# ucb-bar/Accelerated-TinyMPC

Hardware: AMD Instinct MI355X
Metric: MPC solves/sec (batched quadrotor nx=12,nu=4,N=30) (higher is better)
Workload: dtype f32; 1 GPU; quadrotor_tracking batched 65536 instances per GPU, cold-start tiny_solve, early_exit (tol 1e-3, max_iter 100); nx=12, nu=4, N=30, instances_per_gpu=65536, instances_total=65536, parallelism=batch-shard x1, world_size_seen=1, backend=none (single process), kernel=tile16<12,4,30,exact>, max_iters=85

## Files before the change

accelerated-tinympc_amd/csrc/admm_tile16.hip:

```cpp
#include "rowlane_math.h"
#include <cstdlib>

namespace tinympc
{

typedef float f32x16 __attribute__((ext_vector_type(16)));
#ifndef TINY_T16_ABLATE
#define TINY_T16_ABLATE 0
#endif
#ifndef TINY_T16_CQ
#define TINY_T16_CQ 1
#endif
#ifndef TINY_T16_BADDR
#define TINY_T16_BADDR 1
#endif
#ifndef TINY_T16_PADTAB
#define TINY_T16_PADTAB 1
#endif
#ifndef TINY_T16_XPOSE
#define TINY_T16_XPOSE 1
#endif
#ifndef TINY_T16_SCHED
#define TINY_T16_SCHED 1
#endif
// ... 307 lines not shown
{
#pragma unroll
    for (int k = 0; k < 4; k++)
    {
        lo8[k] = __int_as_float(__builtin_amdgcn_update_dpp(__float_as_int(e[k]), __float_as_int(o[k]), 0x128, 0xf, 0xc, false));
        hi8[k] = __int_as_float(__builtin_amdgcn_update_dpp(__float_as_int(o[k]), __float_as_int(e[k]), 0x128, 0xf, 0x3, false));
    }
}

#if TINY_T16_STAMP && !defined(TINY_T16_PI_UNIT)
constexpr int T16_STAMP_TILES = 32;
__device__ unsigned long long *t16_stamp_buf;
__device__ int t16_stamp_slots;
__device__ __forceinline__ void t16_stamp(int wslot, int k, int field, unsigned long long v)
{
    unsigned long long *const buf = t16_stamp_buf;
    if (buf && wslot < t16_stamp_slots && k < T16_STAMP_TILES && (threadIdx.x & 63) == 0) buf[((size_t)wslot * T16_STAMP_TILES + k) * 4 + field] = v;
}
#define T16_STAMP(k, field, v) t16_stamp((int)blockIdx.x * TILE16_WAVES + (int)(threadIdx.x >> 6), (k), (field), (v))
#else
#define T16_STAMP(k, field, v) ((void)0)
#endif

__device__ __forceinline__ void t16_dma_row(unsigned on, const float *sbase, unsigned voff, unsigned lds_dst, float after)
{
    asm volatile("s_cmp_eq_u32 %0, 0\n\ts_cbranch_scc1 1f\n\ts_mov_b32 m0, %3\n\ts_nop 0\n\tglobal_load_lds_dwordx4 %1, %2\n1:"
                 : : "s"(on), "v"(voff), "s"(sbase), "s"(lds_dst), "v"(after) : "memory", "scc");
}
__device__ __forceinline__ void t16_dma_row2(unsigned on, const float *sbase, unsigned voff, unsigned lds_dst, float after0, float after1)
{
    asm volatile("s_cmp_eq_u32 %0, 0\n\ts_cbranch_scc1 1f\n\ts_mov_b32 m0, %3\n\ts_nop 0\n\tglobal_load_lds_dwordx4 %1, %2\n\t"
                 "s_add_u32 m0, m0, 0x3f0\n\ts_nop 0\n\tglobal_load_lds_dwordx4 %1, %2 offset:16\n1:"
                 : : "s"(on), "v"(voff), "s"(sbase), "s"(lds_dst), "v"(after0), "v"(after1) : "memory", "scc");
}
__device__ __forceinline__ void t16_dma_img2(unsigned on, const float *sbase, unsigned voff, unsigned lds_dst, float after0, float after1)
{
    asm volatile("s_cmp_eq_u32 %0, 0\n\ts_cbranch_scc1 1f\n\ts_mov_b32 m0, %3\n\ts_nop 0\n\tglobal_load_lds_dwordx4 %1, %2\n\t"
                 "global_load_lds_dwordx4 %1, %2 offset:1024\n1:"
                 : : "s"(on), "v"(voff), "s"(sbase), "s"(lds_dst), "v"(after0), "v"(after1) : "memory", "scc");
}
__device__ __forceinline__ void t16_wait_vm(int k)
{
    if (k == 0) asm volatile("s_waitcnt vmcnt(0)" ::: "memory");
    else if (k == 1) asm volatile("s_waitcnt vmcnt(1)" ::: "memory");
    else if (k == 2) asm volatile("s_waitcnt vmcnt(2)" ::: "memory");
    else if (k == 3) asm volatile("s_waitcnt vmcnt(3)" ::: "memory");
    else if (k == 4) asm volatile("s_waitcnt vmcnt(4)" ::: "memory");
    else if (k == 5) asm volatile("s_waitcnt vmcnt(5)" ::: "memory");
    else if (k == 6) asm volatile("s_waitcnt vmcnt(6)" ::: "memory");
    else if (k == 7) asm volatile("s_waitcnt vmcnt(7)" ::: "memory");
    else asm volatile("s_waitcnt vmcnt(8)" ::: "memory");
}
constexpr int t16_ring_b(bool XR) { return XR ? 3 : 4; }
constexpr int t16_ring_x(bool BR) { return BR ? 4 : 6; }
constexpr int T16_RING_B = 2048, T16_RING_X = 1024;

template <int N, bool EXACT, bool COLD, bool MPC = false, bool BR = false, bool XR = false>
__global__ __launch_bounds__(WAVE * TILE16_WAVES, 1) void admm_tile16_kernel(const RowParams P)
{
    static_assert(!(MPC && (BR || XR)), "the closed loop on chip is instantiated for batch-shared bounds and a shared / windowed reference");
    constexpr int NX = 12, NU = 4;
    const int lane = threadIdx.x & 63, wv = threadIdx.x >> 6, g = lane >> 4, c = lane & 15;
    const int ntiles = (P.batch + 15) >> 4;
    const float rho = P.rho;
    const f32x4 rho4 = {rho, rho, rho, rho};

    extern __shared__ __attribute__((aligned(16))) float4 lds4_base[];
    float4 *const lds4 = lds4_base;
    float4 *const sn0 = lds4 + wv * (N * WAVE) + lane;
    constexpr int DB = t16_ring_b(XR), DX = t16_ring_x(BR);
    const unsigned ringsB = (P.pi_flags & 1u) ? DB : 2, ringsX = (P.pi_flags & 2u) ? DX : 1;
    const unsigned bnd_f4 = BR ? TILE16_WAVES * ringsB * (T16_RING_B / 16) : 2 * N * 4;
    float4 *const blo = lds4 + TILE16_WAVES * N * WAVE, *const bhi = blo + N * 4, *const tab0 = blo + bnd_f4;
    float4 *const tab = tab0;
    const int tab_rows = P.xref_mode == 1 ? P.table_rows : N;
    const float *tab_src = P.xref_mode == 1 ? P.xref_table : P.xref;
    unsigned dmaB = 0, dmaX = 0;
    if constexpr (BR)
    {
        const unsigned ring = (unsigned)(size_t)(lds_float4 *)blo + wv * (ringsB * T16_RING_B);
        dmaB = __builtin_amdgcn_readfirstlane(ring);
    }
    else
    {
        for (int e = threadIdx.x; e < N * 16; e += WAVE * TILE16_WAVES)
        {
            const float2 lh = reinterpret_cast<const float2 *>(P.bounds)[e];
            const int i = e >> 4, r = e & 15;
            reinterpret_cast<float *>(&blo[i * 4 + (r & 3)])[r >> 2] = lh.x;
            reinterpret_cast<float *>(&bhi[i * 4 + (r & 3)])[r >> 2] = lh.y;
        }
    }
    if constexpr (XR)
    {
        const unsigned ring = (unsigned)(size_t)(lds_float4 *)tab0 + wv * (ringsX * T16_RING_X);
        dmaX = __builtin_amdgcn_readfirstlane(ring);
    }
    else
    {
        for (int e = threadIdx.x; e < (tab_rows + N - 1) * 16; e += WAVE * TILE16_WAVES)
        {
            const int er = (e >> 4) < tab_rows ? (e >> 4) : tab_rows - 1;
            float val = tab_src[er * 16 + (e & 15)];
            if (TINY_T16_CQ) val = -(val * ((e & 15) < NX ? P.mats[(2 * NX + 2 * NU) * 16 + (e & 15)] : 1.f));
            reinterpret_cast<float *>(&tab[(e >> 4) * 4 + (e & 3)])[(e & 15) >> 2] = val;
        }
    }
    if constexpr (!BR || !XR) __syncthreads();

    TileMath<EXACT> M;
    M.load(P.mats, g, c);
    f32x4 qv;
#pragma unroll
    for (int v = 0; v < 3; v++) qv[v] = P.mats[(2 * NX + 2 * NU) * 16 + 4 * v + g];
    qv[3] = 1.f;
    constexpr bool CQ = TINY_T16_CQ && !XR;
    auto cost_of = [&](const f32x4 &xr) { return CQ ? xr : -(xr * qv); };

    constexpr bool DQ = COLD && !MPC;
    int qinc = 1;
    if constexpr (DQ)
    {
        const unsigned tail_stride = (P.pi_flags >> 8) & 0xffu;
        if (tail_stride && (((unsigned)blockIdx.x * TILE16_WAVES + (unsigned)wv) % tail_stride) == 0u) qinc = 0x10000;
        qinc = __builtin_amdgcn_readfirstlane(qinc);
    }
#if TINY_T16_STAMP
    int stamp_k = 0;
#else
    constexpr int stamp_k = 0;
#endif
    for (;;)
    {
    int slot = 0;
    if (lane == 0) slot = atomicAdd(P.n_unsolved + 1, qinc);
    slot = __builtin_amdgcn_readfirstlane(slot);
    T16_STAMP(stamp_k, 0, __builtin_amdgcn_s_memrealtime());
    T16_STAMP(stamp_k, 3, ~0ull);
    if (DQ && ntiles <= 32768)
    {
        const int qh = slot & 0xffff, qt = (int)((unsigned)slot >> 16);
        if (qh + qt >= ntiles) break;
        slot = qinc == 1 ? qh : ntiles - 1 - qt;
    }
    else if (slot >= ntiles) break;
    int ozt;
    asm volatile("s_mov_b32 %0, 0" : "=s"(ozt));
    float4 *const sn = sn0 + ozt;
    float4 *const lds4 = lds4_base + ozt;
    int tile = slot;
    if (P.order) tile = P.order[slot];
    const bool tile_ok = tile >= 0 && tile < ntiles;
    T16_STAMP(stamp_k, 3, (unsigned long long)(unsigned)tile);
    const int inst = tile * 16 + c;
    const bool valid = tile_ok && inst < P.batch;
    const int inst_a = valid ? inst : P.batch - 1;

    float a[N][4];
    float dr[N], bo[N][4], pl[N][3];
    auto dual4 = [&](int i) { return f32x4{a[i][0], a[i][1], a[i][2], a[i][3]}; };
    const int ebase = (inst_a * N) * 16 + g;
    int wstart = 0;
    if (P.xref_mode == 1) wstart = P.xref_start[inst_a];
    const bool zdual = COLD || (P.duals_zero != 0);

    if constexpr (COLD)
    {
        const float4 z4 = make_float4(0.f, 0.f, 0.f, 0.f);
#pragma unroll
        for (int i = 0; i < N; i++)
        {
            a[i][0] = a[i][1] = a[i][2] = a[i][3] = 0.f;
#pragma unroll
            for (int v = 0; v < 4; v++) acc_init(bo[i][v], 0.f);
            sn[i * WAVE] = z4;
            acc_init(pl[i][0], 0.f); acc_init(pl[i][1], 0.f); acc_init(pl[i][2], 0.f);
            dr[i] = 0.f;
        }
    }
    else
    {
#pragma unroll
        for (int i = 0; i < N; i++)
        {
            float vzl[4], pdv[4];
#pragma unroll
            for (int v = 0; v < 4; v++)
            {
                const int o = ebase + i * 16 + 4 * v;
                vzl[v] = P.vz[o]; pdv[v] = P.pd[o];
                const float gyv = P.gy[o];
                a[i][v] = zdual ? 0.f : gyv;
                acc_init(bo[i][v], vzl[v]);
            }
            sn[i * WAVE] = make_float4(vzl[0], vzl[1], vzl[2], vzl[3]);
            acc_init(pl[i][0], pdv[0]); acc_init(pl[i][1], pdv[1]); acc_init(pl[i][2], pdv[2]);
            dr[i] = pdv[3];
        }
    }
    float x0[3];
#pragma unroll
    for (int v = 0; v < 3; v++) x0[v] = P.xu[ebase + 4 * v];

    const unsigned onB = BR ? (P.pi_flags & 1u) : 0u, onX = XR ? (P.pi_flags & 2u) : 0u;
    struct PiAddr { unsigned rdB, rdX, voffB, voffX; };
    auto pi_addr = [&](unsigned lane16) {
        const unsigned c16 = lane16 & 0xf0u, gg = lane16 >> 8, cc = c16 >> 4;
        const int ins = tile * 16 + (int)cc;
        const unsigned ia = (unsigned)((tile_ok && ins < P.batch) ? ins : P.batch - 1);
        PiAddr A;
        A.rdB = dmaB + 1024u * (gg >> 1) + c16 + 8u * (gg & 1u);
        A.rdX = dmaX + c16 + 4u * gg;
        A.voffB = ia * P.bounds_inst_stride * 8u + 32u * gg;
        A.voffX = ia * P.xref_inst_stride * 4u + 16u * gg;
        return A;
    };
    const float *const xsrc = P.xref;
    auto load_xref = [&](const float4 *tb, int ws, int i, int gsel = -1) {
        if constexpr (XR)
        {
            unsigned ll = lane;
            asm volatile("" : "+v"(ll));
            const unsigned cc = ll & 15u, gg = ll >> 4;
            if (onX)
            {
                const float *rp = xsrc + ((size_t)((tile_ok ? tile : 0) * N + i) * 64 + cc) * 4 + gg;
                return f32x4{rp[0], rp[64], rp[128], 0.f};
            }
            const int ins = tile * 16 + (int)cc;
            const float *rp = xsrc + (size_t)((tile_ok && ins < P.batch) ? ins : P.batch - 1) * P.xref_inst_stride + i * 16 + gg;
            return f32x4{rp[0], rp[4], rp[8], 0.f};
        }
        else
        {
        int row;
        if constexpr (TINY_T16_PADTAB && !(EXACT && COLD && !MPC && !BR && !XR)) row = (ws < tab_rows - 1 ? ws : tab_rows - 1) + i;
        else { row = ws + i; row = row < tab_rows ? row : tab_rows - 1; }
        const float4 t4 = tb[row * 4 + (gsel >= 0 ? gsel : g)];
        return f32x4{t4.x, t4.y, t4.z, t4.w};
        }
    };
    PiAddr A0 = {0u, 0u, 0u, 0u};
    if constexpr (BR || XR)
    {
        A0 = pi_addr(16u * lane);
        if constexpr (BR) { t16_dma_row2(onB ^ 1u, P.bounds, A0.voffB, dmaB, 0.f, 0.f); t16_dma_row2(onB ^ 1u, P.bounds, A0.voffB + (N - 1) * 128u, dmaB + T16_RING_B, 0.f, 0.f); }
        if constexpr (XR) t16_dma_row((onX >> 1) ^ 1u, xsrc, A0.voffX, dmaX, 0.f);
        asm volatile("s_waitcnt vmcnt(0)" ::: "memory");
    }
    auto load_xref_raw = [&](const float4 *tb, int ws, int i) {
        if constexpr (CQ)
        {
            int row = ws + i;
            row = row < tab_rows ? row : tab_rows - 1;
            const float *rp = tab_src + row * 16 + g;
            return f32x4{rp[0], rp[4], rp[8], 0.f};
        }
        else return load_xref(tb, ws, i);
    };
    float pterm[3];
    {
        const f32x4 xrN4 = load_xref_raw(tab, wstart, N - 1);
        const float xrN[3] = {xrN4[0], xrN4[1], xrN4[2]};
        M.terminal(xrN, pterm);
    }

    int st = TINY_STATUS_UNSOLVED_, itn = 1;
    float r_ps = 0.f, r_pi = 0.f, r_ds = 0.f, r_di = 0.f;
    if (valid && !COLD)
    {
        r_ps = P.res[4 * inst + 0]; r_pi = P.res[4 * inst + 1];
        r_ds = P.res[4 * inst + 2]; r_di = P.res[4 * inst + 3];
    }
    float pN[3] = {0.f, 0.f, 0.f};

    auto backward_sweep = [&](unsigned long long amask, const float4 *snI, const float4 *tabI, int wsI) {
        float p[3] = {pN[0], pN[1], pN[2]};
        auto load_lin = [&](int i, float4 &sl, f32x4 &xr) {
            sl = snI[i * WAVE];
            xr = load_xref(tabI, wsI, i);
        };
        auto make_lin = [&](int i, const float4 &sl, const f32x4 &xr) {
            const f32x4 sni = {sl.x, sl.y, sl.z, sl.w};
            return lin_cost4<EXACT>(cost_of(xr), rho4, sni - dual4(i));
        };
        float4 sl0; f32x4 xr0;
        load_lin(N - 2, sl0, xr0);
        f32x4 lin = make_lin(N - 2, sl0, xr0);
#pragma unroll
        for (int i = N - 2; i >= 0; i--)
        {
            float4 sl_n = make_float4(0.f, 0.f, 0.f, 0.f); f32x4 xr_n = {0.f, 0.f, 0.f, 0.f};
            if (EXACT && i > 0) load_lin(i - 1, sl_n, xr_n);
            typename TileMath<EXACT>::InFlight F;
            M.riccati_issue(p, lin, F);
            if (!EXACT && i > 0) load_lin(i - 1, sl_n, xr_n);
#if TINY_T16_SCHED
            if constexpr (EXACT) __builtin_amdgcn_sched_barrier(0);
#endif
            f32x4 lin_n = lin;
            if (i > 0) lin_n = make_lin(i - 1, sl_n, xr_n);
#if TINY_T16_SCHED
            if constexpr (EXACT) __builtin_amdgcn_sched_barrier(0);
#endif
            float pn[3], dd;
            M.riccati_finish(F, lin, pn, dd);
            masked_backward_update(amask, pl[i], dr[i], pn, dd);
            p[0] = pn[0]; p[1] = pn[1]; p[2] = pn[2];
// ... 68 lines not shown
            const f32x4 dp = sv - t, dd_ = old - t;
            pri_x = fmaxf(fmaxf(fmaxf(pri_x, fabsf(dp[0])), fabsf(dp[1])), fabsf(dp[2]));
            dua_x = fmaxf(fmaxf(fmaxf(dua_x, fabsf(dd_[0])), fabsf(dd_[1])), fabsf(dd_[2]));
            pri_u = fmaxf(pri_u, fabsf(dp[3]));
            dua_u = fmaxf(dua_u, fabsf(dd_[3]));
            if (i == N - 1)
            {
                const f32x4 an = tp - t;
#pragma unroll
                for (int v = 0; v < 3; v++)
                {
                    const float pn_ = lin_cost<EXACT>(pterm[v], rho, t[v] - an[v]);
                    pN[v] = active ? pn_ : pN[v];
                }
            }
            masked_forward_update(amask, a[i], tp, bo[i], old, sn_addr + i * (WAVE * 16), t);
        };
        f32x4 sv_p = {0.f, 0.f, 0.f, 0.f};
        float4 lo_p = make_float4(0.f, 0.f, 0.f, 0.f), hi_p = lo_p, ol_p = lo_p;
#pragma unroll
        for (int i = 0; i < N; i++)
        {
            float4 lo, hi;
            if constexpr (BR)
            {
                if (i + DB - 1 < N) dma_b(i + DB - 1, lo_p.x, hi_p.w);
                t16_wait_vm(2 * ((N - 1 - i) < (DB - 1) ? (N - 1 - i) : (DB - 1)));
                ring_bounds(i, lo, hi);
            }
            else if constexpr (TINY_T16_BADDR && (COLD || !XR)) { lo = bloG[i * 4]; hi = bhiG[i * 4]; }
            else { lo = bloI[i * 4 + g]; hi = bhiI[i * 4 + g]; }
            const float4 ol = snI[i * WAVE];
            typename TileMath<EXACT>::InFlight F;
            if (i < N - 1) M.lqr_issue(s, F);
#if TINY_T16_SCHED
            if constexpr (EXACT) __builtin_amdgcn_sched_barrier(0);
#endif
            if (i > 0) elementwise(i - 1, sv_p, lo_p, hi_p, ol_p);
            float un = 0.f, xn[3] = {0.f, 0.f, 0.f};
            if (i < N - 1) M.lqr_finish(F, dr[i], un, xn);
            sv_p = f32x4{s[0], s[1], s[2], un};
            lo_p = lo; hi_p = hi; ol_p = ol;
            s[0] = xn[0]; s[1] = xn[1]; s[2] = xn[2];
        }
        elementwise(N - 1, sv_p, lo_p, hi_p, ol_p);
        pri_x = tile_inst_max(pri_x); dua_x = tile_inst_max(dua_x);
        pri_u = tile_inst_max(pri_u); dua_u = tile_inst_max(dua_u);
        bool conv = false;
        if (active)
        {
            itn = it + 1;
            if ((it + 1) % P.check_termination == 0)
            {
                r_ps = pri_x; r_ds = dua_x * rho; r_pi = pri_u; r_di = dua_u * rho;
                conv = (r_ps < P.abs_pri_tol) && (r_pi < P.abs_pri_tol) && (r_ds < P.abs_dua_tol) && (r_di < P.abs_dua_tol);
            }
            if (conv) st = TINY_STATUS_SOLVED_;
        }
        active = active && !conv;
        if (!__any(active)) break;
        if (it == P.max_iter - 1) break;
        {
            float p[3] = {pN[0], pN[1], pN[2]};
            const unsigned long long amask = __ballot(active);
            auto load_lin = [&](int i, float4 &sl, f32x4 &xr) {
                sl = snI[i * WAVE];
                if constexpr (XR) xr = ring_xref(i);
                else xr = load_xref(tabI, wsI, i, TINY_T16_BADDR ? (int)gI : -1);
            };
            auto make_lin = [&](int i, const float4 &sl, const f32x4 &xr) {
                const f32x4 sni = {sl.x, sl.y, sl.z, sl.w};
                return lin_cost4<EXACT>(cost_of(xr), rho4, sni - dual4(i));
            };
            float4 sl0; f32x4 xr0;
            if constexpr (XR) t16_wait_vm(0);
            load_lin(N - 2, sl0, xr0);
            f32x4 lin = make_lin(N - 2, sl0, xr0);
#pragma unroll
            for (int i = N - 2; i >= 0; i--)
            {
                float4 sl_n = make_float4(0.f, 0.f, 0.f, 0.f); f32x4 xr_n = {0.f, 0.f, 0.f, 0.f};
                if constexpr (XR)
                {
                    if (i >= DX) dma_x(i - DX, lin[0]);
                    if (i > 0)
                    {
                        const int hi_j = (i - 2) < (N - 2 - DX) ? (i - 2) : (N - 2 - DX), lo_j = (i - DX) > 0 ? (i - DX) : 0;
                        t16_wait_vm(hi_j >= lo_j ? hi_j - lo_j + 1 : 0);
                    }
                }
                if (EXACT && i > 0) load_lin(i - 1, sl_n, xr_n);
                typename TileMath<EXACT>::InFlight F;
                M.riccati_issue(p, lin, F);
                if (!EXACT && i > 0) load_lin(i - 1, sl_n, xr_n);
#if TINY_T16_SCHED
                if constexpr (EXACT) __builtin_amdgcn_sched_barrier(0);
#endif
                f32x4 lin_n = lin;
                if (i > 0) lin_n = make_lin(i - 1, sl_n, xr_n);
#if TINY_T16_SCHED
                if constexpr (EXACT) __builtin_amdgcn_sched_barrier(0);
#endif
                float pn[3], dd;
                M.riccati_finish(F, lin, pn, dd);
                masked_backward_update(amask, pl[i], dr[i], pn, dd);
                p[0] = pn[0]; p[1] = pn[1]; p[2] = pn[2];
                lin = lin_n;
            }
        }
    }
    if (!MPC || ms + 1 >= P.mpc_steps) break;
    if constexpr (MPC)
    {
        int oz;
        asm volatile("s_mov_b32 %0, 0" : "=s"(oz));
        float4 *const snA = sn + oz;
        const unsigned sn_addr = (unsigned)(size_t)(lds_float4 *)snA;
        const bool solved = st == TINY_STATUS_SOLVED_;
        float un, xn_[3];
        M.lqr(x0, dr[0], un, xn_);
        if (P.u0_traj && valid) P.u0_traj[((long long)ms * P.batch + inst) * NU + g] = un;
        {
            const f32x16 p0 = TINY_MFMA1(M.A1[0], x0[0], M.negz), p1 = TINY_MFMA1(M.A1[1], x0[1], M.negz), p2 = TINY_MFMA1(M.A1[2], x0[2], M.negz);
            const f32x16 pb = TINY_MFMA1(M.A2, un, M.negz);
            f32x4 t[12], t2[4];
            gather12v(t, p0, p1, p2);
            gather4v(t2, pb);
            f32x4 z = {0.f, 0.f, 0.f, 0.f};
            asm volatile("" : "+v"(z));
            f32x4 acc = z + t[0];
#pragma unroll
            for (int k = 1; k < 12; k++) acc = acc + t[k];
            const f32x4 x1 = acc + reduce4<PLAN_SEQ>(t2);
            x0[0] = x1[0]; x0[1] = x1[1]; x0[2] = x1[2];
        }
        const unsigned long long umask = __ballot(valid && !solved);
        if (umask != 0ull) backward_sweep(umask, snA, tab + oz, wstart + oz);
        const unsigned long long smask = __ballot(valid && solved);
#pragma unroll
        for (int i = 0; i < N; i++) masked_restore_slack(smask, bo[i], sn_addr + i * (WAVE * 16));
        if (P.xref_mode == 1)
        {
            wstart += P.window_advance;
            const f32x4 xrN4 = load_xref_raw(tab + oz, wstart, N - 1);
            const float xrN[3] = {xrN4[0], xrN4[1], xrN4[2]};
            M.terminal(xrN, pterm);
        }
#pragma unroll
        for (int i = 0; i < N; i++) a[i][0] = a[i][1] = a[i][2] = a[i][3] = 0.f;
    }
    }
    T16_STAMP(stamp_k, 1, __builtin_amdgcn_s_memrealtime());

    if (P.max_iter <= 0)
    {
        if (valid && g == 0)
        {
            P.status[inst] = TINY_STATUS_UNSOLVED_;
            P.iter[inst] = 1;
            atomicAdd(P.n_unsolved, 1);
        }
        T16_STAMP(stamp_k, 2, __builtin_amdgcn_s_memrealtime());
#if TINY_T16_STAMP
        ++stamp_k;
#endif
        continue;
    }

    {
        const bool solved = st == TINY_STATUS_SOLVED_;
        const int c2 = lane >> 2, q2 = lane & 3;
        const int inst2 = tile * 16 + c2;
        const bool valid2 = tile_ok && inst2 < P.batch;
        const int obase2 = ((valid2 ? inst2 : 0) * N) * 16 + 4 * q2;
        typedef float float_ma __attribute__((may_alias));
        typedef f32x4 f32x4_ma __attribute__((may_alias));
        float_ma *const stage_w = reinterpret_cast<float_ma *>(lds4 + wv * (N * WAVE));
        const int rd_off = (c2 * 4 + q2);
        const int obase4 = ebase + 3 * g;
        constexpr bool XPOSE = TINY_T16_XPOSE && !(EXACT && !COLD && !MPC);
        auto put = [&](float *dst, int i, const f32x4 &val) {
            if constexpr (XPOSE)
            {
                const f32x4 o = t16_transpose4(val);
                if (valid) *reinterpret_cast<f32x4 *>(dst + obase4 + i * 16) = o;
                return;
            }
            float_ma *slot = stage_w + i * (WAVE * 4);
            reinterpret_cast<f32x4_ma *>(slot)[lane] = val;
            asm volatile("" ::: "memory");
            f32x4 o;
            o[0] = slot[rd_off]; o[1] = slot[rd_off + 64]; o[2] = slot[rd_off + 128]; o[3] = slot[rd_off + 192];
            asm volatile("" ::: "memory");
            if (valid2) *reinterpret_cast<f32x4 *>(dst + obase2 + i * 16) = o;
        };
        float s[3] = {x0[0], x0[1], x0[2]};
        if constexpr (XPOSE && TINY_T16_LINES && COLD && !MPC && !BR && !XR)
        {
            auto slack_of = [&](int i) { return reinterpret_cast<const f32x4_ma *>(stage_w + i * (WAVE * 4))[lane]; };
            auto lin_of = [&](int i, const f32x4 &sni) {
                const f32x4 xr = load_xref(tab, wstart, i);
                f32x4 lin = lin_cost4<EXACT>(cost_of(xr), rho4, sni - dual4(i));
                if (i == N - 1) lin[3] = 0.f;
                return lin;
            };
            auto pd_of = [&](int i) { return i == N - 1 ? f32x4{pN[0], pN[1], pN[2], 0.f} : f32x4{acc_get(pl[i][0]), acc_get(pl[i][1]), acc_get(pl[i][2]), dr[i]}; };
            auto vz_of = [&](int i, const f32x4 &sni) {
                f32x4 vzv;
    #pragma unroll
                for (int v = 0; v < 4; v++)
                {
                    const float bov = acc_get(bo[i][v]);
                    vzv[v] = solved ? bov : sni[v];
                }
                return vzv;
            };
            const int instL = tile * 16 + (c & 7);
            const bool validL = tile_ok && instL < P.batch, validH = tile_ok && instL + 8 < P.batch;
            const int obaseL = (validL ? instL : 0) * (N * 16) + ((c >> 3) << 4) + 4 * g, offH = 8 * N * 16;
            auto put2 = [&](float *dst, int i, const f32x4 &ve, const f32x4 &vo) {
                f32x4 lo8, hi8;
                t16_pair_lines(t16_transpose4(ve), t16_transpose4(vo), lo8, hi8);
                if (validL) *reinterpret_cast<f32x4 *>(dst + obaseL + i * 16) = lo8;
                if (validH) *reinterpret_cast<f32x4 *>(dst + obaseL + offH + i * 16) = hi8;
            };
#pragma unroll
            for (int i = 0; i + 1 < N; i += 2)
            {
                const f32x4 sne = slack_of(i), sno = slack_of(i + 1);
                put2(P.gy, i, dual4(i), dual4(i + 1));
                put2(P.vzn, i, sne, sno);
                put2(P.vz, i, vz_of(i, sne), vz_of(i + 1, sno));
                put2(P.pd, i, pd_of(i), pd_of(i + 1));
                put2(P.qr, i, lin_of(i, sne), lin_of(i + 1, sno));
                float ue = 0.f, xe[3];
                M.lqr(s, dr[i], ue, xe);
                const f32x4 sve = {s[0], s[1], s[2], ue};
                float uo = 0.f, xo[3] = {0.f, 0.f, 0.f};
                if (i + 1 < N - 1) M.lqr(xe, dr[i + 1], uo, xo);
                put2(P.xu, i, sve, f32x4{xe[0], xe[1], xe[2], uo});
                s[0] = xo[0]; s[1] = xo[1]; s[2] = xo[2];
            }
            if constexpr (N % 2 == 1)
            {
                const f32x4 sni = slack_of(N - 1);
                put(P.xu, N - 1, f32x4{s[0], s[1], s[2], 0.f});
                put(P.qr, N - 1, lin_of(N - 1, sni));
                put(P.pd, N - 1, pd_of(N - 1));
                put(P.vz, N - 1, vz_of(N - 1, sni));
                put(P.vzn, N - 1, sni);
                put(P.gy, N - 1, dual4(N - 1));
            }
        }
        else
        {
#pragma unroll
        for (int i = 0; i < N; i++)
        {
            float un = 0.f, xn[3] = {0.f, 0.f, 0.f};
            if (i < N - 1) M.lqr(s, dr[i], un, xn);
            const f32x4 sv = {s[0], s[1], s[2], un};
            const f32x4 sni = reinterpret_cast<const f32x4_ma *>(stage_w + i * (WAVE * 4))[lane];
            const f32x4 xr = load_xref(tab, wstart, i);
            f32x4 lin = lin_cost4<EXACT>(cost_of(xr), rho4, sni - dual4(i));
            if (i == N - 1) lin[3] = 0.f;
            f32x4 pdv = {acc_get(pl[i][0]), acc_get(pl[i][1]), acc_get(pl[i][2]), dr[i]};
            if (i == N - 1) pdv = f32x4{pN[0], pN[1], pN[2], 0.f};
            f32x4 vzv;
#pragma unroll
            for (int v = 0; v < 4; v++)
            {
                const float bov = acc_get(bo[i][v]);
                vzv[v] = solved ? bov : sni[v];
            }
            put(P.xu, i, sv);
            put(P.qr, i, lin);
            put(P.pd, i, pdv);
            put(P.vz, i, vzv);
            put(P.vzn, i, sni);
            put(P.gy, i, dual4(i));
            if constexpr (!XPOSE) reinterpret_cast<f32x4_ma *>(stage_w + i * (WAVE * 4))[lane] = sni;
            s[0] = xn[0]; s[1] = xn[1]; s[2] = xn[2];
        }
        }
        const unsigned long long umask = __ballot(valid && !solved);
        if (umask != 0ull)
        {
            const bool unsolved2 = valid2 && ((umask >> c2) & 1ull);
            float p[3] = {pN[0], pN[1], pN[2]};
#pragma unroll
            for (int i = N - 2; i >= 0; i--)
            {
                const f32x4 sni = reinterpret_cast<const f32x4_ma *>(stage_w + i * (WAVE * 4))[lane];
                const f32x4 xr = load_xref(tab, wstart, i);
                const f32x4 lin = lin_cost4<EXACT>(cost_of(xr), rho4, sni - dual4(i));
                float pn[3], dd;
                M.riccati(p, lin, pn, dd);
                if constexpr (XPOSE)
                {
                    const f32x4 o = t16_transpose4(f32x4{pn[0], pn[1], pn[2], dd});
                    if (valid && !solved) *reinterpret_cast<f32x4 *>(P.pd + obase4 + i * 16) = o;
                }
                else
                {
                float_ma *slot = stage_w + i * (WAVE * 4);
                reinterpret_cast<f32x4_ma *>(slot)[lane] = f32x4{pn[0], pn[1], pn[2], dd};
                asm volatile("" ::: "memory");
                f32x4 o;
                o[0] = slot[rd_off]; o[1] = slot[rd_off + 64]; o[2] = slot[rd_off + 128]; o[3] = slot[rd_off + 192];
                asm volatile("" ::: "memory");
                if (unsolved2) *reinterpret_cast<f32x4 *>(P.pd + obase2 + i * 16) = o;
                }
                p[0] = pn[0]; p[1] = pn[1]; p[2] = pn[2];
            }
        }
        if (valid && g == 0)
        {
            P.res[4 * inst + 0] = r_ps; P.res[4 * inst + 1] = r_pi;
            P.res[4 * inst + 2] = r_ds; P.res[4 * inst + 3] = r_di;
            P.status[inst] = st;
            P.iter[inst] = itn;
            if (!solved) atomicAdd(P.n_unsolved, 1);
        }
        if (MPC && valid)
        {
#pragma unroll
            for (int v = 0; v < 3; v++) P.x0buf[inst * NX + 4 * v + g] = x0[v];
            if (g == 0 && P.xref_mode == 1) P.xref_start[inst] = wstart;
        }
    }
    T16_STAMP(stamp_k, 2, __builtin_amdgcn_s_memrealtime());
#if TINY_T16_STAMP
    ++stamp_k;
#endif
    }
}

#ifdef TINY_T16_ONLY30
#define TINY_FOR_EACH_TILE16(X) X(30)
#else
#define TINY_FOR_EACH_TILE16(X) X(30) X(25) X(20) X(10)
#endif

static inline unsigned t16_tail_stride(const RowParams &P, int ntiles, int nblocks, int asked)
{
    static const int env = [] { const char *e = getenv("TINYMPC_T16_TAIL"); return e ? atoi(e) : -1; }();
    const int forced = asked >= 0 ? asked : env;
    if (ntiles > 32768) return 0u;
    if (forced >= 0) return (P.cold_start && P.mpc_steps <= 1) ? (unsigned)(forced > 255 ? 255 : forced) : 0u;
    if (!P.order || P.mpc_steps > 1 || !P.cold_start) return 0u;
    const int slots = nblocks * TILE16_WAVES;
    if (ntiles < 3 * slots) return 0u;
    return (ntiles >= 4 * slots && ntiles < 8 * slots) ? 4u : 8u;
}

#ifdef TINY_T16_PI_UNIT
size_t tile16_pi_lds_bytes(int N, bool bounds_ring, bool xref_ring, unsigned pi_flags, int table_rows)
{
    const size_t bnd = bounds_ring ? (size_t)TILE16_WAVES * ((pi_flags & 1u) ? t16_ring_b(xref_ring) : 2) * T16_RING_B : (size_t)2 * N * 4 * sizeof(float4);
    const size_t ref = xref_ring ? (size_t)TILE16_WAVES * ((pi_flags & 2u) ? t16_ring_x(bounds_ring) : 1) * T16_RING_X : (size_t)(table_rows + N - 1) * 4 * sizeof(float4);
    return (size_t)TILE16_WAVES * N * WAVE * sizeof(float4) + bnd + ref;
}

hipError_t launch_admm_tile16_pi(int N, bool exact, bool bounds_ring, bool xref_ring, const RowParams &P, hipStream_t stream, int n_cu, int tail)
{
    const int ntiles = (P.batch + 15) / 16;
    if (n_cu <= 0) n_cu = 256;
    const int want = (ntiles + TILE16_WAVES - 1) / TILE16_WAVES, nblocks = want < n_cu ? want : n_cu;
    if (P.mpc_steps > 1 || (!bounds_ring && !xref_ring)) return hipErrorInvalidValue;
    if (P.xref_mode == 1 && P.table_rows < 1) return hipErrorInvalidValue;
    if (!bounds_ring && P.bounds_inst_stride != 0) return hipErrorInvalidValue;
    if (!xref_ring && P.xref_mode != 1 && P.xref_inst_stride != 0) return hipErrorInvalidValue;
    if (xref_ring && P.xref_mode == 1) return hipErrorInvalidValue;
    const size_t lds = tile16_pi_lds_bytes(N, bounds_ring, xref_ring, P.pi_flags, P.xref_mode == 1 ? P.table_rows : N);
    if (lds > 160 * 1024) return hipErrorInvalidValue;
    RowParams Q = P;
    Q.pi_flags = (Q.pi_flags & 0xffu) | (t16_tail_stride(P, ntiles, nblocks, tail) << 8);
#define TINY_TILE16_PI_LAUNCH3(NN, EX, BRR, XRR)                                                                           \
    {                                                                                                                      \
        auto kern = P.cold_start ? admm_tile16_kernel<NN, EX, true, false, BRR, XRR> : admm_tile16_kernel<NN, EX, false, false, BRR, XRR>; \
        hipError_t e = hipFuncSetAttribute((const void *)kern, hipFuncAttributeMaxDynamicSharedMemorySize, (int)lds);      \
        if (e != hipSuccess) return e;                                                                                     \
        hipLaunchKernelGGL(kern, dim3(nblocks), dim3(WAVE * TILE16_WAVES), lds, stream, Q);                                \
        return hipGetLastError();                                                                                          \
    }
#define TINY_TILE16_PI_LAUNCH(NN, EX)                                             \
    {                                                                             \
        if (bounds_ring && xref_ring) TINY_TILE16_PI_LAUNCH3(NN, EX, true, true)  \
        else if (bounds_ring) TINY_TILE16_PI_LAUNCH3(NN, EX, true, false)         \
        else TINY_TILE16_PI_LAUNCH3(NN, EX, false, true)                          \
    }
#define TINY_TILE16_PI_DISPATCH(NN)                  \
    if (N == NN)                                     \
    {                                                \
        if (exact) TINY_TILE16_PI_LAUNCH(NN, true)   \
        else TINY_TILE16_PI_LAUNCH(NN, false)        \
    }
    TINY_FOR_EACH_TILE16(TINY_TILE16_PI_DISPATCH)
    return hipErrorInvalidValue;
}
#else
bool tile16_supported(int nx, int nu, int N)
{
    if (nx != 12 || nu != 4) return false;
#define TINY_TILE16_CHECK(NN) \
    if (N == NN) return true;
    TINY_FOR_EACH_TILE16(TINY_TILE16_CHECK)
    return false;
}

int tile16_max_table_rows() { return TILE16_MAX_TABLE_ROWS; }

#if TINY_T16_STAMP
static int t16_stamp_nslots = 0;
extern "C" int tiny_t16_stamp_begin()
{
    static unsigned long long *buf = nullptr;
    int dev = 0, ncu = 0;
    if (hipGetDevice(&dev) != hipSuccess || hipDeviceGetAttribute(&ncu, hipDeviceAttributeMultiprocessorCount, dev) != hipSuccess || ncu <= 0) return 1;
    const int nslots = ncu * TILE16_WAVES;
    const size_t bytes = (size_t)nslots * T16_STAMP_TILES * 4 * sizeof(unsigned long long);
    if (buf) (void)hipFree(buf);
    buf = nullptr;
    if (hipMalloc(&buf, bytes) != hipSuccess || hipMemset(buf, 0, bytes) != hipSuccess) return 1;
    if (hipMemcpyToSymbol(HIP_SYMBOL(t16_stamp_slots), &nslots, sizeof(nslots)) != hipSuccess) return 1;
    if (hipMemcpyToSymbol(HIP_SYMBOL(t16_stamp_buf), &buf, sizeof(buf)) != hipSuccess || hipDeviceSynchronize() != hipSuccess) return 1;
    t16_stamp_nslots = nslots;
    return 0;
}
extern "C" int tiny_t16_stamp_slots() { return t16_stamp_nslots; }
extern "C" int tiny_t16_stamp_read(unsigned long long *host, int nslots)
{
    if (nslots > t16_stamp_nslots) return 1;
    unsigned long long *buf = nullptr;
    if (hipMemcpyFromSymbol(&buf, HIP_SYMBOL(t16_stamp_buf), sizeof(buf)) != hipSuccess || !buf) return 1;
    return hipMemcpy(host, buf, (size_t)nslots * T16_STAMP_TILES * 4 * sizeof(unsigned long long), hipMemcpyDeviceToHost) != hipSuccess;
}
extern "C" int tiny_t16_stamp_tiles() { return T16_STAMP_TILES; }
#endif

hipError_t launch_admm_tile16(int N, bool exact, const RowParams &P, hipStream_t stream, int n_cu, int tail)
{
    const int ntiles = (P.batch + 15) / 16;
    if (n_cu <= 0) n_cu = 256;
    const int want = (ntiles + TILE16_WAVES - 1) / TILE16_WAVES, nblocks = want < n_cu ? want : n_cu;
    const int rows = P.xref_mode == 1 ? P.table_rows : N;
    if (rows > TILE16_MAX_TABLE_ROWS) return hipErrorInvalidValue;
    const size_t lds = (size_t)(TILE16_WAVES * N * WAVE + 2 * N * 4 + (rows + N - 1) * 4) * sizeof(float4);
    RowParams Q = P;
    Q.pi_flags = (Q.pi_flags & 0xffu) | (t16_tail_stride(P, ntiles, nblocks, tail) << 8);
#define TINY_TILE16_LAUNCH(NN, EX)                                                                                         \
    {                                                                                                                      \
        auto kern = P.mpc_steps > 1 ? (P.cold_start ? admm_tile16_kernel<NN, EX, true, true> : admm_tile16_kernel<NN, EX, false, true>) \
                                    : (P.cold_start ? admm_tile16_kernel<NN, EX, true> : admm_tile16_kernel<NN, EX, false>); \
        hipError_t e = hipFuncSetAttribute((const void *)kern, hipFuncAttributeMaxDynamicSharedMemorySize, (int)lds);      \
        if (e != hipSuccess) return e;                                                                                     \
        hipLaunchKernelGGL(kern, dim3(nblocks), dim3(WAVE * TILE16_WAVES), lds, stream, Q);                                \
        return hipGetLastError();                                                                                          \
    }
#define TINY_TILE16_DISPATCH(NN)                  \
    if (N == NN)                                  \
    {                                             \
        if (exact) TINY_TILE16_LAUNCH(NN, true)   \
        else TINY_TILE16_LAUNCH(NN, false)        \
    }
    TINY_FOR_EACH_TILE16(TINY_TILE16_DISPATCH)
    return hipErrorInvalidValue;
}
#endif

}
```

accelerated-tinympc_amd/csrc/dispatch_order.hip:

```cpp
#include "rowlane_math.h"

namespace tinympc
{

constexpr int kPredictorSteps = 4;

template <int NX, int NU, bool H16, bool TILES = false>
__global__ __launch_bounds__(TILES ? 4 * WAVE : WAVE) void dispatch_key_kernel(const RowParams P, float *__restrict__ key)
{
    const int lane = threadIdx.x & (WAVE - 1), r16 = lane & 15;
    const int grp = TILES ? (int)blockIdx.x * 4 + (int)(threadIdx.x >> 6) : (int)blockIdx.x;
    const int inst = grp * 4 + (lane >> 4);
    const bool valid = inst < P.batch;
    const int inst_a = valid ? inst : P.batch - 1;
    const bool is_x = r16 < NX, is_u = (r16 >= NX) && (r16 < NX + NU);
    const int N = P.N;
    const int rowbase = (inst_a * N) * 16 + r16;
    const bool cold = P.cold_start != 0, zdual = cold || (P.duals_zero != 0);
    RowGains<NX, NU> G;
    G.load(P.mats, r16);
    float s = ldw<H16>(P.xu, rowbase), pri = 0.f;
    const int steps = N < kPredictorSteps ? N : kPredictorSteps;
    for (int i = 0; i < steps; i++)
    {
        const int o = rowbase + i * 16;
        float sv, xn = 0.f;
        if (i < N - 1) lqr_step<NX, NU, false, H16>(G, is_x, is_u, s, cold ? 0.f : ldw<H16>(P.pd, o), sv, xn);
        else sv = is_x ? s : 0.f;
        const float2 lh = ld_bounds<H16>(P.bounds, inst_a * (int)P.bounds_inst_stride + i * 16 + r16);
        const float a = zdual ? 0.f : ldw<H16>(P.gy, o);
        pri = fmaxf(pri, fabsf(sv - __builtin_amdgcn_fmed3f(sv + a, lh.x, lh.y)));
        s = xn;
    }
    pri = (valid && (is_x || is_u)) ? pri : 0.f;
#pragma unroll
    for (int m = 32; m >= 1; m >>= 1) pri = fmaxf(pri, __shfl_xor(pri, m));
    if constexpr (TILES)
    {
        __shared__ float wk[4];
        if (lane == 0) wk[threadIdx.x >> 6] = pri;
        __syncthreads();
        if (threadIdx.x == 0) key[blockIdx.x] = fmaxf(fmaxf(wk[0], wk[1]), fmaxf(wk[2], wk[3]));
    }
    else if (lane == 0) key[blockIdx.x] = pri;
}

constexpr int NBUCKET = 2048;
template <class BucketOf>
__device__ inline void bucket_sort_descending(BucketOf bucket_of, int *__restrict__ order, int n, int *__restrict__ counters)
{
    __shared__ int cnt[NBUCKET], sa[NBUCKET], sb[NBUCKET];
    const int t = threadIdx.x;
    if (t == 0 && counters) counters[0] = counters[1] = 0;
    for (int b = t; b < NBUCKET; b += 1024) cnt[b] = 0;
    __syncthreads();
    for (int g = t; g < n; g += 1024) atomicAdd(&cnt[bucket_of(g)], 1);
    __syncthreads();
    for (int r = t; r < NBUCKET; r += 1024) sa[r] = cnt[NBUCKET - 1 - r];
    __syncthreads();
    int *src = sa, *dst = sb;
    for (int d = 1; d < NBUCKET; d <<= 1)
    {
        for (int r = t; r < NBUCKET; r += 1024) dst[r] = src[r] + (r >= d ? src[r - d] : 0);
        __syncthreads();
        int *tmp = src; src = dst; dst = tmp;
    }
    for (int b = t; b < NBUCKET; b += 1024)
    {
        const int r = NBUCKET - 1 - b;
        dst[b] = src[r] - cnt[b];
    }
    __syncthreads();
    for (int g = t; g < n; g += 1024) order[atomicAdd(&dst[bucket_of(g)], 1)] = g;
}

__global__ __launch_bounds__(1024) void dispatch_order_kernel(const float *__restrict__ key, int *__restrict__ order, int n, int *__restrict__ counters)
{
    bucket_sort_descending([key](int g) { return (int)((__builtin_bit_cast(unsigned, key[g]) & 0x7fffffffu) >> 20); }, order, n, counters);
}

__global__ __launch_bounds__(1024) void dispatch_order_history_kernel(const int *__restrict__ iter, int unit, int batch, int use_sum, int *__restrict__ order, int n,
                                                                      int *__restrict__ counters)
{
    bucket_sort_descending(
        [=](int g) {
            int m = 0;
            for (int k = 0; k < unit; k++)
            {
                const int i = g * unit + k;
                if (i < batch) m = use_sum ? m + max(iter[i], 0) : max(m, iter[i]);
            }
            return min(max(m, 0), NBUCKET - 1);
        },
        order, n, counters);
}

hipError_t launch_dispatch_order_history(const int *iter, int batch, int unit, int *order, int *counters, hipStream_t stream, int use_sum)
{
    const int n = (batch + unit - 1) / unit;
    hipLaunchKernelGGL(dispatch_order_history_kernel, dim3(1), dim3(1024), 0, stream, iter, unit, batch, use_sum, order, n, counters);
    return hipGetLastError();
}

hipError_t launch_dispatch_order(int nx, int nu, bool h16, const RowParams &P, float *key, int *order, hipStream_t stream, int tile)
{
    const int ngroups = (P.batch + 3) / 4;
    const int ntiles = (P.batch + 15) / 16;
#define TINY_KEY_DISPATCH(NX, NU)                                                                                      \
    if (nx == NX && nu == NU)                                                                                          \
    {                                                                                                                  \
        if (tile)                                                                                                      \
        {                                                                                                              \
            if (h16) return hipErrorInvalidValue;                                                                      \
            hipLaunchKernelGGL((dispatch_key_kernel<NX, NU, false, true>), dim3(ntiles), dim3(4 * WAVE), 0, stream, P, key); \
            hipLaunchKernelGGL(dispatch_order_kernel, dim3(1), dim3(1024), 0, stream, key, order, ntiles, P.n_unsolved); \
            return hipGetLastError();                                                                                  \
        }                                                                                                              \
        if (h16) hipLaunchKernelGGL((dispatch_key_kernel<NX, NU, true>), dim3(ngroups), dim3(WAVE), 0, stream, P, key); \
        else hipLaunchKernelGGL((dispatch_key_kernel<NX, NU, false>), dim3(ngroups), dim3(WAVE), 0, stream, P, key);   \
        hipLaunchKernelGGL(dispatch_order_kernel, dim3(1), dim3(1024), 0, stream, key, order, ngroups, P.n_unsolved);  \
        return hipGetLastError();                                                                                      \
    }
    TINY_FOR_EACH_ROWDIMS(TINY_KEY_DISPATCH)
    return hipErrorInvalidValue;
}

}
```

accelerated-tinympc_amd/csrc/tinympc_batch.hip:

```cpp
#include "../../include/tinympc_batch.h"
#include "eigen_orders.h"
#include "tinympc_internal.h"

#include <cmath>
#include <cstdarg>
#include <cstdio>
#include <cstring>
#include <limits>
#include <map>
#include <mutex>
#include <optional>
#include <string>
#include <vector>

using namespace tinympc;

namespace
{

thread_local std::string g_err;

int fail(int code, const char *fmt, ...)
{
    char buf[512];
// ... 268 lines not shown
    const long long total = (long long)batch * (1 + pm_gen_floats(nx, nu));
    for (long long e = (long long)blockIdx.x * blockDim.x + threadIdx.x; e < total; e += (long long)gridDim.x * blockDim.x)
    {
        long long o = e;
        int k = 0;
        while (o >= (long long)batch * sz[k]) o -= (long long)batch * sz[k++];
        double v = src[k][o];
        if (k == 7) v = v + rho[o / nx];
        dst[e] = (float)v;
    }
}

__global__ void bounds_table_kernel(const float *__restrict__ xmin, const float *__restrict__ xmax, const float *__restrict__ umin,
                                    const float *__restrict__ umax, int sh_x, int sh_u, float *__restrict__ dst, Geo g, int nb,
                                    int en_state, int en_input, int h16)
{
    const long long total = (long long)nb * g.N * g.rw;
    const float inf = __builtin_inff();
    for (long long e = (long long)blockIdx.x * blockDim.x + threadIdx.x; e < total; e += (long long)gridDim.x * blockDim.x)
    {
        const int r = (int)(e % g.rw);
        const long long t = e / g.rw;
        const int i = (int)(t % g.N), b = (int)(t / g.N);
        float lo = -inf, hi = inf;
        if (r < g.nx && en_state)
        {
            const long long o = ((long long)(sh_x ? 0 : b) * g.N + i) * g.nx + r;
            lo = xmin ? xmin[o] : 0.f; hi = xmax ? xmax[o] : 0.f;
        }
        else if (r >= g.nx && r < g.nx + g.nu && i < g.N - 1 && en_input)
        {
            const long long o = ((long long)(sh_u ? 0 : b) * (g.N - 1) + i) * g.nu + (r - g.nx);
            lo = umin ? umin[o] : 0.f; hi = umax ? umax[o] : 0.f;
        }
        lo = lo < hi ? lo : hi;
        if (h16)
        {
            reinterpret_cast<_Float16 *>(dst)[2 * e] = (_Float16)lo;
            reinterpret_cast<_Float16 *>(dst)[2 * e + 1] = (_Float16)hi;
        }
        else { dst[2 * e] = lo; dst[2 * e + 1] = hi; }
    }
}

__global__ void tile16_image_kernel(const float4 *__restrict__ src, float4 *__restrict__ dst, int nb, int N, int pieces, long long inst_stride_f4)
{
    const long long total = (long long)((nb + 15) / 16) * N * pieces * 64;
    for (long long e = (long long)blockIdx.x * blockDim.x + threadIdx.x; e < total; e += (long long)gridDim.x * blockDim.x)
    {
        const int lane = (int)(e & 63), piece = (int)((e >> 6) % pieces);
        const long long t = e / (64 * pieces);
        const int step = (int)(t % N), g = lane >> 4, c = lane & 15;
        long long inst = (t / N) * 16 + c;
        inst = inst < nb ? inst : nb - 1;
        dst[e] = src[inst * inst_stride_f4 + (long long)step * 4 * pieces + pieces * g + piece];
    }
}

__global__ void rows_vary_kernel(const float2 *__restrict__ bounds, const float *__restrict__ xref, int nb, int N, int nx, int nu, int *__restrict__ vary)
{
    const long long total = (long long)nb * 16;
    for (long long e = (long long)blockIdx.x * blockDim.x + threadIdx.x; e < total; e += (long long)gridDim.x * blockDim.x)
    {
        const int r = (int)(e & 15);
        const long long b = e >> 4;
        if (bounds && r < nx + nu)
        {
            const int steps = r < nx ? N : N - 1;
            const unsigned long long *p = reinterpret_cast<const unsigned long long *>(bounds) + (b * N) * 16 + r;
            bool differ = false;
            for (int i = 1; i < steps; i++) differ |= p[(size_t)i * 16] != p[0];
            if (differ) vary[0] = 1;
        }
        if (xref && r < nx)
        {
            const unsigned *p = reinterpret_cast<const unsigned *>(xref) + (b * N) * 16 + r;
            bool differ = false;
            for (int i = 1; i < N; i++) differ |= p[(size_t)i * 16] != p[0];
            if (differ) vary[1] = 1;
        }
    }
}

int grid_for(long long total, int block = 256)
{
    long long gsz = (total + block - 1) / block;
    if (gsz > 8192) gsz = 8192;
    if (gsz < 1) gsz = 1;
    return (int)gsz;
}

const int kPairOf[TINY_ARR_COUNT] = {0, 0, 1, 1, 2, 2, 3, 4, 3, 4, 5, 5};
bool is_xfam(int id)
{
    return id == TINY_ARR_X || id == TINY_ARR_Q || id == TINY_ARR_P || id == TINY_ARR_V || id == TINY_ARR_VNEW ||
           id == TINY_ARR_G;
}

struct InputArr
{
    float *dev = nullptr;
    bool shared = true, set = false;
    std::vector<float> host;
};

}

struct TinyBatch
{
    int nx = 0, nu = 0, N = 0, batch = 0, device = 0;
    int NXC = 0, NUC = 0, ntiles = 0, bpad4 = 0;
    int rw = 16;
    bool row_dims_ok = false, tile_dims_ok = false, rowmath_ok = false, rowloop_ok = false, wave_ok = false, quad_ok = false;
    bool tile16_ok = false;
    bool waveres_ok = false;
    bool tile48_ok = false;
    bool generic_ok = false;
    float *gen_mats = nullptr;
    int *conv_dev = nullptr;
    hipStream_t stream = nullptr;
    hipStream_t own_stream = nullptr;
    hipGraphExec_t graph_exec = nullptr;
    std::string graph_sig;
    bool have_cache = false, have_dyn = false, have_settings = false, gains_dirty = true;
    float rho = 0.f;
    std::vector<float> Kinf, Pinf, Quu_inv, AmBKt, Adyn, Bdyn, Q;
    float abs_pri_tol = 0.f, abs_dua_tol = 0.f;
    int max_iter = 0, check_termination = 1, en_state_bound = 0, en_input_bound = 0;
    int layout = LAYOUT_TILE;
    float *arr[TINY_ARR_COUNT] = {};
    float *pair[6] = {};
    size_t xfam_floats = 0, ufam_floats = 0, pair_floats = 0;
    InputArr in_xref, in_bnd[4];
    bool en_uref = false, en_d2p = false, have_rcost = false;
    std::vector<float> Rcost, coeff_d2p;
    InputArr in_uref;
    float *r_uref = nullptr;
    const int *order_dev = nullptr;
    int dispatch_mode = -1;
    float *u0_stage = nullptr;
    float *key_buf = nullptr;
    int *order_buf = nullptr;
    bool derived_dirty[2] = {true, true};
    float *t_xref = nullptr, *t_bnd[4] = {};
    float *r_xref = nullptr, *r_bounds = nullptr;
    float *r_bounds_img = nullptr, *r_xref_img = nullptr;
    size_t r_bounds_img_n = 0, r_xref_img_n = 0;
    int *rows_vary_dev = nullptr;
    unsigned rows_vary = 3u;
    size_t r_xref_n = 0, r_bounds_n = 0, r_uref_n = 0;
    int graph_captures = 0;
    int n_cu = 256;
    int tile_queue = -1;
    float *tab_tile = nullptr, *tab_row = nullptr;
    float *tab_row_h = nullptr;
    int table_rows = 0;
    int *xref_start = nullptr;
    int xref_mode = 0;
    float *res = nullptr;
    int *status = nullptr, *iter = nullptr, *n_unsolved = nullptr;
    float *opnd = nullptr, *qvec = nullptr;
    float *mats_exact = nullptr, *mats_fast = nullptr;
    float *dA = nullptr, *dB = nullptr;
    float *x0buf = nullptr;
    float *staging = nullptr;
    size_t staging_floats = 0;
    bool duals_zero_pending = false;
    bool cold_pending = false;
    bool x0_zero_pending = false;
    int variant = VAR_AUTO;
    std::optional<Kernel> row_family_forced;
    int last_dispatch = 0;
    bool iter_history = false;
    bool pm = false;
    float *pm_src = nullptr, *pm_rho = nullptr, *pm_row[2] = {};
    bool pm_row_dirty[2] = {true, true};
    bool h16 = false;
    bool dual32 = false;
    bool dual32_pref = false;
    bool dual32_forced = false;
    bool timing = false;
    hipEvent_t ev0 = nullptr, ev1 = nullptr;
    bool ev_valid = false;
    std::string name_buf[2];
};

namespace
{

struct KernelTraits
{
    const char *name;
    bool name_has_N;
    bool name_has_storage;
    int layout;
    bool fp32_duals;
    int order_unit_solve;
    int order_unit_run;
    bool onchip_mpc;
    int row_kernel_number;
    bool TinyBatch::*has;
};
constexpr KernelTraits kKernelTraits[] = {
     {"rowlane", true, true, LAYOUT_ROW, true, 4, 4, true, 1, &TinyBatch::row_dims_ok},
     {"rowloop", false, true, LAYOUT_ROW, false, 4, 0, false, 2, &TinyBatch::rowloop_ok},
     {"rowstream", false, true, LAYOUT_ROW, false, 0, 0, false, 3, &TinyBatch::rowmath_ok},
     {"wavestream", false, false, LAYOUT_ROW, false, 0, 0, false, 6, &TinyBatch::wave_ok},
     {"quadlane", true, true, LAYOUT_ROW, true, 0, 0, true, 4, &TinyBatch::quad_ok},
     {"tile16", true, false, LAYOUT_ROW, false, 16, 16, true, 5, &TinyBatch::tile16_ok},
     {"waveres", false, false, LAYOUT_ROW, false, 0, 0, false, 7, &TinyBatch::waveres_ok},
     {"tile48", true, false, LAYOUT_ROW, false, 0, 0, false, 8, &TinyBatch::tile48_ok},
     {"stream", false, false, LAYOUT_TILE, false, 0, 0, false, 0, &TinyBatch::tile_dims_ok},
     {"generic", false, false, LAYOUT_TILE, false, 0, 0, false, 0, &TinyBatch::generic_ok},
};
constexpr const KernelTraits &traits(Kernel k) { return kKernelTraits[(int)k]; }

Geo geo(const TinyBatch *tb) { return Geo{tb->nx, tb->nu, tb->N, tb->NXC, tb->NUC, tb->rw}; }

void invalidate_graph(TinyBatch *tb)
{
    if (tb->graph_exec)
    {
        (void)hipSetDevice(tb->device);
        (void)hipStreamSynchronize(tb->stream);
        (void)hipGraphExecDestroy(tb->graph_exec);
        tb->graph_exec = nullptr;
    }
    tb->graph_sig.clear();
}

int set_device(TinyBatch *tb)
{
    HIP_TRY(hipSetDevice(tb->device));
    return 0;
}

int dev_alloc_zero(float **p, size_t nfloats)
{
    HIP_TRY(guarded_malloc((void **)p, nfloats * sizeof(float)));
    HIP_TRY(hipMemset(*p, 0, nfloats * sizeof(float)));
    HIP_TRY(hipStreamSynchronize(nullptr));
    return 0;
}

int sized_buffer(float **p, size_t *have, size_t nfloats)
{
    if (*p && *have == nfloats) return 0;
    if (*p) { (void)guarded_free(*p); *p = nullptr; }
    *have = 0;
    TRY(dev_alloc_zero(p, nfloats));
    *have = nfloats;
    return 0;
}

float *work_ptr(TinyBatch *tb, int id) { return tb->layout == LAYOUT_ROW ? tb->pair[kPairOf[id]] : tb->arr[id]; }
int h16_of(const TinyBatch *tb, int layout) { return (tb->h16 && layout == LAYOUT_ROW) ? 1 : 0; }
int h16_at(const TinyBatch *tb, int layout, const float *arr) { return (h16_of(tb, layout) && !(tb->dual32 && arr == tb->pair[5])) ? 1 : 0; }

int alloc_layout(TinyBatch *tb, int layout)
{
    if (layout == LAYOUT_ROW)
    {
        for (int p = 0; p < 6; p++)
            if (!tb->pair[p]) TRY(dev_alloc_zero(&tb->pair[p], (tb->h16 && !(tb->dual32 && p == 5)) ? (tb->pair_floats + 1) / 2 : tb->pair_floats));
    }
    else
    {
        for (int id = 0; id < TINY_ARR_COUNT; id++)
            if (!tb->arr[id]) TRY(dev_alloc_zero(&tb->arr[id], is_xfam(id) ? tb->xfam_floats : tb->ufam_floats));
    }
    return 0;
}

void free_layout(TinyBatch *tb, int layout)
{
    if (layout == LAYOUT_ROW)
        for (int p = 0; p < 6; p++) { (void)guarded_free(tb->pair[p]); tb->pair[p] = nullptr; }
    else
        for (int id = 0; id < TINY_ARR_COUNT; id++) { (void)guarded_free(tb->arr[id]); tb->arr[id] = nullptr; }
}

int launch_pack(TinyBatch *tb, const float *src, float *dst, int layout, int fam, int nb, bool shared, int step0, int nsteps, float *mirror = nullptr)
{
    const long long total = (long long)nb * nsteps * (fam ? tb->nu : tb->nx);
    hipLaunchKernelGGL(pack_kernel, dim3(grid_for(total)), dim3(256), 0, tb->stream, src, dst, layout, geo(tb), fam, nb,
                       shared ? 1 : 0, step0, nsteps, h16_at(tb, layout, dst), mirror);
    HIP_TRY(hipGetLastError());
    return 0;
}
int launch_unpack(TinyBatch *tb, const float *src, float *dst, int layout, int fam, int nb, int step0, int nsteps)
{
    const long long total = (long long)nb * nsteps * (fam ? tb->nu : tb->nx);
    hipLaunchKernelGGL(unpack_kernel, dim3(grid_for(total)), dim3(256), 0, tb->stream, src, dst, layout, geo(tb), fam, nb,
                       step0, nsteps, h16_at(tb, layout, src));
    HIP_TRY(hipGetLastError());
    return 0;
}
int launch_zero(TinyBatch *tb, float *dst, int layout, int fam, int step0, int nsteps)
{
    const long long total = (long long)tb->batch * nsteps * (fam ? tb->nu : tb->nx);
    hipLaunchKernelGGL(zero_kernel, dim3(grid_for(total)), dim3(256), 0, tb->stream, dst, layout, geo(tb), fam, tb->batch,
                       step0, nsteps, h16_at(tb, layout, dst));
    HIP_TRY(hipGetLastError());
    return 0;
}

// ... 417 lines not shown
};

Kernel row_kernel_for(const TinyBatch *tb, bool closed_loop)
{
    const std::optional<Kernel> forced = tb->row_family_forced;
    if (tb->wave_ok)
    {
        if (forced == Kernel::Wavestream) return Kernel::Wavestream;
        if (tb->tile48_ok && !tb->h16 && (forced == Kernel::Tile48 || (!forced && tile48_pays(tb->batch, tb->n_cu)))) return Kernel::Tile48;
        return tb->waveres_ok ? Kernel::Waveres : Kernel::Wavestream;
    }
    const bool optional_terms = tb->en_uref || tb->en_d2p;
    if (optional_terms && tb->row_dims_ok && !tb->h16 && bounds_all_shared(tb) && !closed_loop && (!forced || forced == Kernel::Rowlane))
        return Kernel::Rowlane;
    if (!bounds_all_shared(tb))
    {
        if (optional_terms) return Kernel::Rowstream;
        if (tile16_applies(tb, closed_loop) && (forced == Kernel::Tile16 || (!forced && tile16_pi_auto(tb)))) return Kernel::Tile16;
        const std::optional<Kernel> ff = forced == Kernel::Tile16 ? std::nullopt : forced;
        if (tb->row_dims_ok && !tb->h16 && (!ff || ff == Kernel::Rowlane)) return Kernel::Rowlane;
        if (tb->rowloop_ok && (!ff || ff == Kernel::Rowloop)) return Kernel::Rowloop;
        return Kernel::Rowstream;
    }
    if (optional_terms) return Kernel::Rowstream;
    if (forced == Kernel::Tile16)
        return tile16_applies(tb, closed_loop) ? Kernel::Tile16 : (tb->row_dims_ok ? Kernel::Rowlane : (tb->rowloop_ok ? Kernel::Rowloop : Kernel::Rowstream));
    if (forced) return *forced;
    if (tb->quad_ok) return Kernel::Quadlane;
    if (tile16_applies(tb, closed_loop) && !tb->order_dev && (closed_loop ? tile16_closed_loop_size(tb) : tile16_auto_size(tb))) return Kernel::Tile16;
    if (tb->row_dims_ok) return Kernel::Rowlane;
    if (tb->rowloop_ok) return Kernel::Rowloop;
    return Kernel::Rowstream;
}

int plan_of(const TinyBatch *tb, int v, Kernel row, KernelPlan *out)
{
    out->kernel = v == VAR_STREAM ? Kernel::Stream : (v == VAR_GENERIC ? Kernel::Generic : row);
    out->exact = v == VAR_ROW_EXACT || v == VAR_GENERIC;
    out->pm = tb->pm;
    out->pi = out->kernel == Kernel::Tile16 && tile16_per_instance(tb);
    if (out->pi) out->pi_tables = tile16_pi_plan(tb);
    return 0;
}

int resolve_plan(const TinyBatch *tb, bool closed_loop, KernelPlan *out)
{
    int v = tb->variant;
    if (tb->pm)
    {
        if (tb->h16)
            return fail(TINY_BATCH_EUNSUPPORTED, "per-instance models (tiny_batch_set_models) are implemented for fp32 storage only: tiny_batch_set_storage(tb, 32) or tiny_batch_clear_models()");
        if (tb->en_uref || tb->en_d2p)
            return fail(TINY_BATCH_EUNSUPPORTED, "the optional Uref / coeff_d2p terms are not implemented with per-instance models (tiny_batch_set_optional_terms(tb, 0, 0) or tiny_batch_clear_models())");
        if (v == VAR_STREAM)
            return fail(TINY_BATCH_EUNSUPPORTED, "the streaming MFMA kernel (variant 1) holds one gain matrix for the whole launch and cannot serve per-instance models");
        if (v == VAR_AUTO)
        {
            if (!tb->row_dims_ok && !tb->generic_ok)
                return fail(TINY_BATCH_EUNSUPPORTED, "per-instance models need the unrolled 16-lane kernel (an instantiated nx, nu, N) or the run-time-dimension exact kernel "
                                                     "(nx, nu each <= 4 or a multiple of 4); nx=%d nu=%d N=%d has neither", tb->nx, tb->nu, tb->N);
            v = tb->row_dims_ok ? VAR_ROW_EXACT : VAR_GENERIC;
        }
        if (v == VAR_ROW_EXACT || v == VAR_ROW_FAST)
        {
            if (!tb->row_dims_ok)
                return fail(TINY_BATCH_EUNSUPPORTED, "with per-instance models the row variants run on the unrolled 16-lane kernel only, which has no instantiation for nx=%d nu=%d N=%d "
                                                     "(variant 4, the run-time-dimension exact kernel, serves it)", tb->nx, tb->nu, tb->N);
            if (tb->row_family_forced && tb->row_family_forced != Kernel::Rowlane)
                return fail(TINY_BATCH_EUNSUPPORTED, "the forced row kernel (tiny_batch_set_row_kernel) keeps one gain table for the whole launch and cannot serve per-instance models "
                                                     "(tile16: its MFMA A operand is one gain matrix for all 16 columns); only the 16-lane kernel (1) or auto (0) can");
        }
        if (v == VAR_GENERIC && !tb->generic_ok)
            return fail(TINY_BATCH_EUNSUPPORTED, "the run-time-dimension exact kernel (variant 4) needs nx, nu each <= 4 or a multiple of 4 (nx=%d nu=%d)", tb->nx, tb->nu);
        return plan_of(tb, v, Kernel::Rowlane, out);
    }
    const bool row_ok = tb->row_dims_ok || tb->rowmath_ok || tb->wave_ok;
    const Kernel row = row_kernel_for(tb, closed_loop);
    if (v == VAR_ROW_FAST && tb->wave_ok && row != Kernel::Waveres && row != Kernel::Tile48)
        return fail(TINY_BATCH_EUNSUPPORTED, "fma arithmetic for 16 < nx + nu <= 64 needs the state-on-chip wave kernel (N <= 50); beyond that it is the streaming MFMA kernel (variant 1)");
    if (v == VAR_AUTO)
    {
        if (!row_ok && !tb->generic_ok)
            return fail(TINY_BATCH_EUNSUPPORTED, "nx=%d nu=%d has no exact-arithmetic kernel (the reference's own summation order depends on column alignment "
                                                 "unless nx and nu are each <= 4 or a multiple of 4); tiny_batch_select_kernel(tb, 1) opts into fma arithmetic "
                                                 "on the MFMA streaming kernel", tb->nx, tb->nu);
        v = row_ok ? VAR_ROW_EXACT : VAR_GENERIC;
    }
    if (v == VAR_GENERIC && (!tb->generic_ok || tb->h16 || tb->en_uref || tb->en_d2p))
        return fail(TINY_BATCH_EUNSUPPORTED, "the run-time-dimension exact kernel (variant 4) needs nx, nu each <= 4 or a multiple of 4 (nx <= 64, nu <= 32), "
                                             "fp32 storage and no optional terms (nx=%d nu=%d)", tb->nx, tb->nu);
    const bool row_variant = v == VAR_ROW_EXACT || v == VAR_ROW_FAST;
    if ((tb->en_uref || tb->en_d2p) && (!tb->rowmath_ok || !row_variant))
        return fail(TINY_BATCH_EUNSUPPORTED, "the optional Uref / coeff_d2p terms (tiny_batch_set_optional_terms) are implemented by the row "
                                             "kernels for nx + nu <= 16 only (nx=%d nu=%d, variant %d)", tb->nx, tb->nu, v);
    if (row_variant && !row_ok)
        return fail(TINY_BATCH_EUNSUPPORTED, "no row kernel instantiation for nx=%d nu=%d (needs nx + nu <= 16)", tb->nx, tb->nu);
    if (v == VAR_STREAM && !tb->tile_dims_ok)
        return fail(TINY_BATCH_EUNSUPPORTED, "no streaming kernel instantiation for nx=%d nu=%d", tb->nx, tb->nu);
    if (v == VAR_STREAM && tb->h16)
        return fail(TINY_BATCH_EUNSUPPORTED, "fp16 storage is implemented by the row kernels only (nx + nu <= 16)");
    return plan_of(tb, v, row, out);
}

std::string kernel_name(const TinyBatch *tb, const KernelPlan &pl)
{
    const KernelTraits &t = traits(pl.kernel);
    char nm[96];
    if (pl.kernel == Kernel::Stream)
    {
        snprintf(nm, sizeof nm, "stream<%d,%d>", tb->NXC, tb->NUC);
        return nm;
    }
    int n = snprintf(nm, sizeof nm, "%s<%d,%d", t.name, tb->nx, tb->nu);
    if (t.name_has_N) n += snprintf(nm + n, sizeof nm - n, ",%d", tb->N);
    const bool d32 = tb->dual32_forced ? tb->dual32 : (tb->dual32_pref && t.fp32_duals);
    const char *suffix = pl.pm ? ",pm" : pl.pi ? ",pi" : (t.name_has_storage && tb->h16) ? (d32 ? ",h16d" : ",h16") : "";
    snprintf(nm + n, sizeof nm - n, ",%s%s>", pl.exact ? "exact" : "fast", suffix);
    return nm;
}

const char *plan_name(TinyBatch *tb, bool closed_loop)
{
    std::string &name = tb->name_buf[closed_loop ? 1 : 0];
    const std::string keep = g_err;
    KernelPlan pl;
    name = resolve_plan(tb, closed_loop, &pl) ? "unsupported" : kernel_name(tb, pl);
    g_err = keep;
    return name.c_str();
}

void fill_row_params(TinyBatch *tb, RowParams &P, bool exact)
{
    P.nx = tb->nx; P.nu = tb->nu; P.N = tb->N; P.batch = tb->batch;
    P.rho = tb->rho; P.abs_pri_tol = tb->abs_pri_tol; P.abs_dua_tol = tb->abs_dua_tol;
    P.max_iter = tb->max_iter; P.check_termination = tb->check_termination;
    P.duals_zero = tb->duals_zero_pending ? 1 : 0;
    P.cold_start = tb->cold_pending ? 1 : 0;
    P.xref_mode = tb->xref_mode;
    P.xu = tb->pair[0]; P.qr = tb->pair[1]; P.pd = tb->pair[2]; P.vz = tb->pair[3]; P.vzn = tb->pair[4]; P.gy = tb->pair[5];
    P.xref = tb->r_xref;
    P.xref_inst_stride = (tb->in_xref.set && !tb->in_xref.shared) ? (unsigned)(tb->N * tb->rw) : 0u;
    P.pi_flags = 0u;
    P.xref_table = tb->h16 ? tb->tab_row_h : tb->tab_row; P.xref_start = tb->xref_start; P.table_rows = tb->table_rows;
    P.bounds = tb->r_bounds;
    P.bounds_inst_stride = bounds_all_shared(tb) ? 0u : (unsigned)(tb->N * tb->rw);
    P.mats = exact ? tb->mats_exact : tb->mats_fast;
    P.uref = tb->en_uref ? tb->r_uref : nullptr;
    P.uref_inst_stride = (tb->in_uref.set && !tb->in_uref.shared) ? (unsigned)(tb->N * tb->rw) : 0u;
    P.en_d2p = tb->en_d2p ? 1 : 0;
    P.order = tb->order_dev;
    P.res = tb->res; P.status = tb->status; P.iter = tb->iter; P.n_unsolved = tb->n_unsolved;
    P.mpc_steps = 1; P.window_advance = 0; P.u0_traj = nullptr; P.x0buf = tb->x0buf;
    P.dual32 = (tb->h16 && tb->dual32) ? 1 : 0;
}

int check_optional_terms(const TinyBatch *tb)
{
    if (tb->en_uref && (!tb->have_rcost || !tb->in_uref.set))
        return fail(TINY_BATCH_ENOTREADY, "the Uref term is enabled: tiny_batch_set_input_cost and tiny_batch_set_uref must be called first");
    if (tb->en_d2p && tb->coeff_d2p.empty())
        return fail(TINY_BATCH_ENOTREADY, "the coeff_d2p term is enabled: tiny_batch_set_coeff_d2p must be called first");
    return 0;
}

int run_step(TinyBatch *tb, int fn, int *converged_host, int *n_true)
{
    if (tb->pm)
        return fail(TINY_BATCH_EUNSUPPORTED, "the six single-function step kernels read one shared model: not available with per-instance models (tiny_batch_clear_models())");
    if (!tb->have_cache || !tb->have_dyn || !tb->have_settings)
        return fail(TINY_BATCH_ENOTREADY, "set_cache, set_dynamics and set_settings must be called first");
    if (!tb->rowmath_ok)
        return fail(TINY_BATCH_EUNSUPPORTED, "the single-function kernels need nx + nu <= 16 and an entry in TINY_FOR_EACH_ROWDIMS (nx=%d nu=%d)", tb->nx, tb->nu);
    if (tb->dual32_forced) return fail(TINY_BATCH_EUNSUPPORTED, "the single-function kernels do not implement fp16 storage with fp32 duals (tiny_batch_set_storage_ex(tb, 16, 32))");
    TRY(check_optional_terms(tb));
    TRY(set_device(tb));
    if (tb->gains_dirty) TRY(pack_gains(tb));
    TRY(ensure_layout(tb, LAYOUT_ROW));
    TRY(settle_dual_width(tb, false));
    TRY(prepare_inputs(tb, LAYOUT_ROW));
    TRY(flush_pending(tb));
    if (!tb->conv_dev) TRY(dev_alloc_zero((float **)&tb->conv_dev, tb->batch));
    RowParams P;
    fill_row_params(tb, P, tb->variant != VAR_ROW_FAST);
    HIP_TRY(hipMemsetAsync(tb->n_unsolved, 0, 2 * sizeof(int), tb->stream));
    hipError_t e = launch_admm_step(tb->nx, tb->nu, tb->variant != VAR_ROW_FAST, tb->h16, fn, P, tb->conv_dev, tb->stream);
    if (e != hipSuccess) return fail(TINY_BATCH_EHIP, "kernel launch failed: %s", hipGetErrorString(e));
    if (fn == STEP_TERMINATION_CONDITION)
    {
        int n_false = 0;
        HIP_TRY(hipMemcpyAsync(&n_false, tb->n_unsolved, sizeof(int), hipMemcpyDeviceToHost, tb->stream));
        if (converged_host)
            HIP_TRY(hipMemcpyAsync(converged_host, tb->conv_dev, (size_t)tb->batch * sizeof(int), hipMemcpyDeviceToHost, tb->stream));
        HIP_TRY(hipStreamSynchronize(tb->stream));
        if (n_true) *n_true = tb->batch - n_false;
    }
    return 0;
}

int pack_models(TinyBatch *tb, const KernelPlan &pl)
{
    if (pl.kernel != Kernel::Rowlane) return 0;
    const int f = pl.exact ? 0 : 1;
    if (!tb->pm_row_dirty[f]) return 0;
    const long long n = (long long)tb->batch * pm_row_floats(tb->nx, tb->nu);
    if (!tb->pm_row[f]) HIP_TRY(guarded_malloc((void **)&tb->pm_row[f], (size_t)n * sizeof(float)));
    hipLaunchKernelGGL(models_pack_row_kernel, dim3(grid_for(n)), dim3(256), 0, tb->stream, tb->pm_src, tb->pm_row[f], tb->batch, tb->nx, tb->nu, f);
    HIP_TRY(hipGetLastError());
    tb->pm_row_dirty[f] = false;
    return 0;
}

ModelParams model_params(const TinyBatch *tb, const KernelPlan &pl)
{
    ModelParams M;
    M.rho = tb->pm_rho;
    if (pl.kernel == Kernel::Generic) { M.mats = tb->pm_src; M.mats_stride = (unsigned)pm_gen_floats(tb->nx, tb->nu); }
    else { M.mats = tb->pm_row[pl.exact ? 0 : 1]; M.mats_stride = (unsigned)pm_row_floats(tb->nx, tb->nu); }
    return M;
}

int prepare_solve(TinyBatch *tb, bool closed_loop, KernelPlan *plan)
{
    if (!(tb->pm || (tb->have_cache && tb->have_dyn)) || !tb->have_settings)
        return fail(TINY_BATCH_ENOTREADY, "tiny_batch_solve: set_cache, set_dynamics (or set_models) and set_settings must be called first");
    for (int k = 0; k < 4; k += 2)
    {
        const InputArr &lo = tb->in_bnd[k], &hi = tb->in_bnd[k + 1];
        const bool lo_inst = lo.set && !lo.shared, hi_inst = hi.set && !hi.shared;
        if (lo_inst != hi_inst && (lo.set || hi.set))
            return fail(TINY_BATCH_EINVAL, "min and max bounds must both be shared or both be per-instance");
    }
    TRY(check_optional_terms(tb));
    TRY(set_device(tb));
    KernelPlan pl;
    TRY(resolve_plan(tb, closed_loop, &pl));
    if (tb->pm) TRY(pack_models(tb, pl));
    else if (tb->gains_dirty) TRY(pack_gains(tb));
    if (!tb->order_buf && tb->bpad4 / 4 >= kDispatchMinGroups)
    {
        TRY(dev_alloc_zero(&tb->key_buf, (size_t)tb->bpad4 / 4 + (size_t)tb->bpad4 / 16 + 16));
        TRY(dev_alloc_zero((float **)&tb->order_buf, (size_t)tb->bpad4 / 4));
    }
    const int layout = traits(pl.kernel).layout;
    const bool inputs_rebuilt = tb->derived_dirty[layout];
    TRY(ensure_layout(tb, layout));
    TRY(settle_dual_width(tb, traits(pl.kernel).fp32_duals));
    TRY(prepare_inputs(tb, layout));
    TRY(flush_x0_zero(tb));
    if (tb->max_iter <= 0) TRY(flush_pending(tb));
    if (inputs_rebuilt) return resolve_plan(tb, closed_loop, plan);
    *plan = pl;
    return 0;
}

void fill_solve_params(const TinyBatch *tb, SolveParams &P)
{
    P.nx = tb->nx; P.nu = tb->nu; P.N = tb->N; P.batch = tb->batch; P.ntiles = tb->ntiles;
    P.rho = tb->rho; P.abs_pri_tol = tb->abs_pri_tol; P.abs_dua_tol = tb->abs_dua_tol;
    P.max_iter = tb->max_iter; P.check_termination = tb->check_termination;
    P.en_state_bound = tb->en_state_bound; P.en_input_bound = tb->en_input_bound;
    P.duals_zero = tb->duals_zero_pending ? 1 : 0;
    P.cold_start = tb->cold_pending ? 1 : 0;
    P.xref_mode = tb->xref_mode;
    P.x = tb->arr[TINY_ARR_X]; P.q = tb->arr[TINY_ARR_Q]; P.p = tb->arr[TINY_ARR_P];
    P.v = tb->arr[TINY_ARR_V]; P.vnew = tb->arr[TINY_ARR_VNEW]; P.g = tb->arr[TINY_ARR_G];
    P.u = tb->arr[TINY_ARR_U]; P.r = tb->arr[TINY_ARR_R]; P.d = tb->arr[TINY_ARR_D];
    P.z = tb->arr[TINY_ARR_Z]; P.znew = tb->arr[TINY_ARR_ZNEW]; P.y = tb->arr[TINY_ARR_Y];
    P.xmin = tb->t_bnd[0]; P.xmax = tb->t_bnd[1]; P.umin = tb->t_bnd[2]; P.umax = tb->t_bnd[3]; P.xref = tb->t_xref;
    const long long xt = (long long)tb->N * WAVE * tb->NXC, ut = (long long)(tb->N - 1) * WAVE * tb->NUC;
    P.xb_tile_stride = (tb->in_bnd[0].set && !tb->in_bnd[0].shared) ? xt : 0;
    P.ub_tile_stride = (tb->in_bnd[2].set && !tb->in_bnd[2].shared) ? ut : 0;
    P.xref_tile_stride = (tb->in_xref.set && !tb->in_xref.shared) ? xt : 0;
    P.xref_table = tb->tab_tile; P.xref_start = tb->xref_start; P.table_rows = tb->table_rows;
    P.res = tb->res; P.status = tb->status; P.iter = tb->iter; P.n_unsolved = tb->n_unsolved;
    P.opnd = tb->opnd; P.qvec = tb->qvec;
}

int enqueue_dispatch_order(TinyBatch *tb, const KernelPlan &pl, int run_steps, bool from_reset, RowParams &P)
{
    const bool run = run_steps > 1;
    const int unit = run ? traits(pl.kernel).order_unit_run : traits(pl.kernel).order_unit_solve;
    const bool eligible = unit && !tb->order_dev && tb->bpad4 / 4 >= kDispatchMinGroups && tb->order_buf;
    const bool history = eligible && dispatch_effective(tb) == 2 && (run || tb->max_iter > 1);
    const bool want_predicted = run ? (tb->dispatch_mode == 1 || (tb->dispatch_mode == -1 && from_reset)) : dispatch_effective(tb) == 1;
    const bool predicted = eligible && want_predicted && !history && !pl.pm && !tb->dual32 && tb->max_iter > 1;
    if (traits(pl.kernel).order_unit_solve == 16) P.order = nullptr;
    hipError_t e = hipSuccess;
    if (history) e = launch_dispatch_order_history(tb->iter, tb->batch, unit, tb->order_buf, tb->n_unsolved, tb->stream, run && unit == 16);
    else if (predicted)
    {
        RowParams K;
        fill_row_params(tb, K, false);
        e = launch_dispatch_order(tb->nx, tb->nu, tb->h16, K, tb->key_buf, tb->order_buf, tb->stream, unit == 16);
    }
    else HIP_TRY(hipMemsetAsync(tb->n_unsolved, 0, 2 * sizeof(int), tb->stream));
    if (e != hipSuccess) return fail(TINY_BATCH_EHIP, "kernel launch failed: %s", hipGetErrorString(e));
    if (history || predicted) P.order = tb->order_buf;
    return history ? 3 : predicted ? 1 : (P.order ? 2 : 0);
}

hipError_t launch_kernel(const TinyBatch *tb, const KernelPlan &pl, RowParams &P)
{
    const int nx = tb->nx, nu = tb->nu, N = tb->N;
    switch (pl.kernel)
    {
    case Kernel::Rowlane:
        return pl.pm ? launch_admm_rowlane_pm(nx, nu, N, pl.exact, P, model_params(tb, pl), tb->stream) : launch_admm_rowlane(nx, nu, N, pl.exact, tb->h16, P, tb->stream);
    case Kernel::Rowloop: return launch_admm_rowloop(nx, nu, pl.exact, tb->h16, P, tb->stream);
    case Kernel::Rowstream: return launch_admm_rowstream(nx, nu, pl.exact, tb->h16, P, tb->stream);
    case Kernel::Wavestream: return launch_admm_wavestream(nx, nu, P, tb->stream);
    case Kernel::Quadlane: return launch_admm_quadlane(N, pl.exact, tb->h16, P, tb->stream);
    case Kernel::Waveres: return launch_admm_waveres(nx, nu, pl.exact, P, tb->stream);
    case Kernel::Tile48: return launch_admm_tile48(N, pl.exact, P, tb->stream);
    case Kernel::Tile16:
    {
        if (!pl.pi) return launch_admm_tile16(N, pl.exact, P, tb->stream, tb->n_cu, tb->tile_queue);
        const Tile16Pi &t = pl.pi_tables;
        P.pi_flags = t.flags;
        if (t.bounds_ring && (t.flags & 1u))
        {
            if (!tb->r_bounds_img) return hipErrorInvalidValue;
            P.bounds = tb->r_bounds_img;
        }
        if (t.xref_ring && (t.flags & 2u))
        {
            if (!tb->r_xref_img) return hipErrorInvalidValue;
            P.xref = tb->r_xref_img;
        }
        return launch_admm_tile16_pi(N, pl.exact, t.bounds_ring, t.xref_ring, P, tb->stream, tb->n_cu, tb->tile_queue);
    }
    case Kernel::Stream:
    case Kernel::Generic:
    {
        SolveParams S;
        fill_solve_params(tb, S);
        if (pl.kernel == Kernel::Stream) return launch_admm_stream(tb->NXC, tb->NUC, S, tb->stream);
        return pl.pm ? launch_admm_generic_pm(S, model_params(tb, pl), tb->NXC, tb->NUC, tb->stream) : launch_admm_generic(S, tb->gen_mats, tb->NXC, tb->NUC, tb->stream);
    }
    }
    return hipErrorInvalidValue;
}

int enqueue_solve(TinyBatch *tb, const KernelPlan &pl, bool record_events)
{
    const KernelTraits &t = traits(pl.kernel);
    RowParams P;
    if (t.layout == LAYOUT_ROW)
    {
        fill_row_params(tb, P, pl.exact);
        const int applied = enqueue_dispatch_order(tb, pl, 1, false, P);
        if (applied < 0) return applied;
        tb->last_dispatch = applied;
    }
    else HIP_TRY(hipMemsetAsync(tb->n_unsolved, 0, 2 * sizeof(int), tb->stream));
    if (record_events) HIP_TRY(hipEventRecord(tb->ev0, tb->stream));
    if (t.layout == LAYOUT_ROW && P.dual32 && !t.fp32_duals)
        return fail(TINY_BATCH_EUNSUPPORTED, "fp16 storage with fp32 duals runs on the register-resident 16-lane and quad kernels only "
                                             "(batch-shared bounds, no optional terms, no forced row kernel)");
    const hipError_t e = launch_kernel(tb, pl, P);
    if (e != hipSuccess) return fail(TINY_BATCH_EHIP, "kernel launch failed: %s", hipGetErrorString(e));
    if (record_events)
    {
        HIP_TRY(hipEventRecord(tb->ev1, tb->stream));
        tb->ev_valid = true;
    }
    if (tb->max_iter > 0) tb->duals_zero_pending = tb->cold_pending = false;
    if (tb->max_iter > 0) tb->iter_history = true;
    return 0;
}

int enqueue_plant_step(TinyBatch *tb, int window_advance)
{
    if (tb->pm)
    {
        hipLaunchKernelGGL(plant_step_pm_kernel, dim3((tb->batch + 127) / 128), dim3(128), 0, tb->stream, tb->x0buf, work_ptr(tb, TINY_ARR_X), work_ptr(tb, TINY_ARR_U),
                           tb->pm_src, tb->xref_mode == 1 ? tb->xref_start : nullptr, window_advance, tb->batch, tb->layout, geo(tb), h16_of(tb, tb->layout));
        HIP_TRY(hipGetLastError());
        return 0;
    }
    hipLaunchKernelGGL(plant_step_kernel, dim3((tb->batch + 127) / 128), dim3(128), 0, tb->stream, tb->x0buf,
                       work_ptr(tb, TINY_ARR_X), work_ptr(tb, TINY_ARR_U), tb->dA, tb->dB,
                       tb->xref_mode == 1 ? tb->xref_start : nullptr, window_advance, tb->batch, tb->layout, geo(tb),
                       h16_of(tb, tb->layout));
    HIP_TRY(hipGetLastError());
    return 0;
}

int set_bound(TinyBatch *tb, const float *src, int shared, int which)
{
    CHECK_TB(tb);
    CHECK_PTR(src);
    TRY(set_device(tb));
    const bool xf = which < 2;
    return store_input(tb, tb->in_bnd[which], src, shared != 0, xf ? tb->N : tb->N - 1, xf ? tb->nx : tb->nu);
}

bool stream_dims_supported(int nxc, int nuc, int *pxc, int *puc)
{
    int best = 1 << 30;
    bool found = false;
#define TINY_CHECK_DIMS(NXC, NUC)                                        \
    if (nxc <= NXC && nuc <= NUC && (NXC + NUC) * 64 + NXC < best)       \
    {                                                                    \
        best = (NXC + NUC) * 64 + NXC; *pxc = NXC; *puc = NUC; found = true; \
    }
    TINY_FOR_EACH_DIMS(TINY_CHECK_DIMS)
    return found;
}

}

extern "C"
{

const char *tiny_batch_last_error(void) { return g_err.c_str(); }

int tiny_batch_create(TinyBatch **out, int nx, int nu, int N, int batch, int device)
{
    CHECK_PTR(out);
    *out = nullptr;
    if (nx < 1 || nu < 1 || N < 2 || batch < 1)
        return fail(TINY_BATCH_EINVAL, "tiny_batch_create: need nx>=1, nu>=1, N>=2, batch>=1 (got %d,%d,%d,%d)", nx, nu, N, batch);
    int nxc = (nx + 3) / 4, nuc = (nu + 3) / 4;
    const bool tile_ok = stream_dims_supported(nxc, nuc, &nxc, &nuc),
               row_ok = rowlane_supported(nx, nu, N) && ((long long)(batch + 3) * N * 16 < (1ll << 30));
    const bool wave_ok = !rowdims_supported(nx, nu) && wavedims_supported(nx, nu) && ((long long)(batch + 3) * N * 64 < (1ll << 30));
    if (!tile_ok && !row_ok && !rowdims_supported(nx, nu) && !wave_ok)
        return fail(TINY_BATCH_EUNSUPPORTED,
                    "no kernel for nx=%d nu=%d N=%d: exact arithmetic needs a compiled class (TINY_FOR_EACH_ROWDIMS / _WAVEDIMS), fma arithmetic nx <= 64 and nu <= 32",
                    nx, nu, N);
    int ndev = 0;
    HIP_TRY(hipGetDeviceCount(&ndev));
    if (device < 0 || device >= ndev) return fail(TINY_BATCH_EINVAL, "device %d out of range (have %d)", device, ndev);
    TinyBatch *tb = new TinyBatch();
    tb->nx = nx; tb->nu = nu; tb->N = N; tb->batch = batch; tb->device = device;
    tb->NXC = nxc; tb->NUC = nuc; tb->ntiles = (batch + TILE - 1) / TILE; tb->bpad4 = (batch + 3) / 4 * 4;
    tb->tile_dims_ok = tile_ok; tb->row_dims_ok = row_ok;
    tb->rowmath_ok = rowdims_supported(nx, nu) && ((long long)(batch + 3) * N * 16 < (1ll << 30));
    tb->rowloop_ok = tb->rowmath_ok && rowloop_supported(nx, nu, N);
    tb->wave_ok = wave_ok;
    tb->quad_ok = tb->rowmath_ok && quadlane_supported(nx, nu, N);
    tb->tile16_ok = tb->rowmath_ok && tile16_supported(nx, nu, N);
    tb->waveres_ok = wave_ok && waveres_supported(nx, nu, N);
    tb->tile48_ok = wave_ok && tile48_supported(nx, nu, N);
    tb->generic_ok = tile_ok && generic_exact_supported(nx, nu);
    tb->rw = wave_ok ? 64 : 16;
    tb->xfam_floats = (size_t)tb->ntiles * N * WAVE * nxc;
    tb->ufam_floats = (size_t)tb->ntiles * (N - 1) * WAVE * nuc;
    tb->pair_floats = (size_t)tb->bpad4 * N * tb->rw;
    tb->layout = (row_ok || wave_ok || !tile_ok) ? LAYOUT_ROW : LAYOUT_TILE;
    auto cleanup = [&](int rc) { tiny_batch_destroy(tb); return rc; };
    if (hipSetDevice(device) != hipSuccess) return cleanup(fail(TINY_BATCH_EHIP, "hipSetDevice(%d) failed", device));
    {
        int ncu = 0;
        if (hipDeviceGetAttribute(&ncu, hipDeviceAttributeMultiprocessorCount, device) == hipSuccess && ncu > 0) tb->n_cu = ncu;
    }
    if (int rc = alloc_layout(tb, tb->layout)) return cleanup(rc);
    if (int rc = dev_alloc_zero(&tb->res, (size_t)batch * 4)) return cleanup(rc);
    if (int rc = dev_alloc_zero((float **)&tb->status, batch)) return cleanup(rc);
    if (int rc = dev_alloc_zero((float **)&tb->iter, batch)) return cleanup(rc);
    if (int rc = dev_alloc_zero((float **)&tb->n_unsolved, 2)) return cleanup(rc);
    if (int rc = dev_alloc_zero((float **)&tb->xref_start, batch)) return cleanup(rc);
    if (int rc = dev_alloc_zero(&tb->x0buf, (size_t)batch * nx)) return cleanup(rc);
    tb->staging_floats = (size_t)batch * N * (nx > nu ? nx : nu);
    if (int rc = dev_alloc_zero(&tb->staging, tb->staging_floats)) return cleanup(rc);
    if (hipEventCreate(&tb->ev0) != hipSuccess || hipEventCreate(&tb->ev1) != hipSuccess)
        return cleanup(fail(TINY_BATCH_EHIP, "hipEventCreate failed"));
    tb->cold_pending = true;
    *out = tb;
    return TINY_BATCH_OK;
}

void tiny_batch_destroy(TinyBatch *tb)
{
    if (!tb) return;
    (void)hipSetDevice(tb->device);
    free_layout(tb, LAYOUT_TILE);
    free_layout(tb, LAYOUT_ROW);
    (void)guarded_free(tb->in_xref.dev);
    (void)guarded_free(tb->in_uref.dev); (void)guarded_free(tb->r_uref);
    (void)guarded_free(tb->key_buf); (void)guarded_free(tb->order_buf); (void)guarded_free(tb->u0_stage);
    for (int k = 0; k < 4; k++) { (void)guarded_free(tb->in_bnd[k].dev); (void)guarded_free(tb->t_bnd[k]); }
    (void)guarded_free(tb->t_xref); (void)guarded_free(tb->r_xref); (void)guarded_free(tb->r_bounds); (void)guarded_free((float *)tb->rows_vary_dev);
    (void)guarded_free(tb->r_bounds_img); (void)guarded_free(tb->r_xref_img);
    (void)guarded_free(tb->tab_tile); (void)guarded_free(tb->tab_row); (void)guarded_free(tb->tab_row_h); (void)guarded_free(tb->xref_start);
    (void)guarded_free(tb->res); (void)guarded_free(tb->status); (void)guarded_free(tb->iter); (void)guarded_free(tb->n_unsolved);
    (void)guarded_free(tb->opnd); (void)guarded_free(tb->qvec); (void)guarded_free(tb->gen_mats); (void)guarded_free(tb->mats_exact); (void)guarded_free(tb->mats_fast);
    (void)guarded_free(tb->pm_src); (void)guarded_free(tb->pm_rho); (void)guarded_free(tb->pm_row[0]); (void)guarded_free(tb->pm_row[1]);
    (void)guarded_free(tb->dA); (void)guarded_free(tb->dB); (void)guarded_free(tb->x0buf); (void)guarded_free(tb->staging); (void)guarded_free(tb->conv_dev);
    if (tb->graph_exec) (void)hipGraphExecDestroy(tb->graph_exec);
    if (tb->own_stream) (void)hipStreamDestroy(tb->own_stream);
    if (tb->ev0) (void)hipEventDestroy(tb->ev0);
    if (tb->ev1) (void)hipEventDestroy(tb->ev1);
    delete tb;
}

int tiny_batch_set_stream(TinyBatch *tb, void *hip_stream)
{
    CHECK_TB(tb);
    invalidate_graph(tb);
    tb->stream = (hipStream_t)hip_stream;
    return 0;
}

int tiny_batch_synchronize(TinyBatch *tb)
{
    CHECK_TB(tb);
    TRY(set_device(tb));
    HIP_TRY(hipStreamSynchronize(tb->stream));
    return 0;
}

int tiny_batch_set_cache(TinyBatch *tb, float rho, const float *Kinf, const float *Pinf, const float *Quu_inv,
                         const float *AmBKt)
{
    CHECK_TB(tb); CHECK_PTR(Kinf); CHECK_PTR(Pinf); CHECK_PTR(Quu_inv); CHECK_PTR(AmBKt);
    const int nx = tb->nx, nu = tb->nu;
    tb->rho = rho;
    tb->Kinf.assign(Kinf, Kinf + (size_t)nu * nx);
    tb->Pinf.assign(Pinf, Pinf + (size_t)nx * nx);
    tb->Quu_inv.assign(Quu_inv, Quu_inv + (size_t)nu * nu);
    tb->AmBKt.assign(AmBKt, AmBKt + (size_t)nx * nx);
    tb->have_cache = true;
    tb->gains_dirty = true;
    invalidate_graph(tb);
    return 0;
}

int tiny_batch_set_dynamics(TinyBatch *tb, const float *Adyn, const float *Bdyn, const float *Q)
{
    CHECK_TB(tb); CHECK_PTR(Adyn); CHECK_PTR(Bdyn); CHECK_PTR(Q);
    const int nx = tb->nx, nu = tb->nu;
    tb->Adyn.assign(Adyn, Adyn + (size_t)nx * nx);
    tb->Bdyn.assign(Bdyn, Bdyn + (size_t)nx * nu);
    tb->Q.assign(Q, Q + nx);
    tb->have_dyn = true;
    tb->gains_dirty = true;
    invalidate_graph(tb);
    return 0;
}

int tiny_batch_set_models_device(TinyBatch *tb, const float *d_rho, const float *d_Kinf, const float *d_Pinf, const float *d_Quu_inv,
                                 const float *d_AmBKt, const float *d_Adyn, const float *d_Bdyn, const float *d_Q)
{
    CHECK_TB(tb); CHECK_PTR(d_rho); CHECK_PTR(d_Kinf); CHECK_PTR(d_Pinf); CHECK_PTR(d_Quu_inv); CHECK_PTR(d_AmBKt); CHECK_PTR(d_Adyn); CHECK_PTR(d_Bdyn); CHECK_PTR(d_Q);
    TRY(set_device(tb));
    invalidate_graph(tb);
    const long long n = (long long)tb->batch * pm_gen_floats(tb->nx, tb->nu);
    if (!tb->pm_src) HIP_TRY(guarded_malloc((void **)&tb->pm_src, (size_t)n * sizeof(float)));
    if (!tb->pm_rho) HIP_TRY(guarded_malloc((void **)&tb->pm_rho, (size_t)tb->batch * sizeof(float)));
    hipLaunchKernelGGL(models_gather_kernel, dim3(grid_for(n)), dim3(256), 0, tb->stream, d_rho, d_Kinf, d_Pinf, d_Quu_inv, d_AmBKt, d_Adyn, d_Bdyn, d_Q,
                       tb->pm_src, tb->pm_rho, tb->batch, tb->nx, tb->nu);
    HIP_TRY(hipGetLastError());
    tb->pm = true;
    tb->pm_row_dirty[0] = tb->pm_row_dirty[1] = true;
    return 0;
}

namespace
{
int set_models_packed(TinyBatch *tb, const float *d)
{
    const size_t B = tb->batch, nx = tb->nx, nu = tb->nu;
    const float *p = d;
    const float *rho = p; p += B;
    const float *K = p; p += B * nu * nx;
    const float *Pf = p; p += B * nx * nx;
    const float *Qi = p; p += B * nu * nu;
    const float *Am = p; p += B * nx * nx;
    const float *A = p; p += B * nx * nx;
    const float *Bm = p; p += B * nx * nu;
    return tiny_batch_set_models_device(tb, rho, K, Pf, Qi, Am, A, Bm, p);
}
}

int tiny_batch_set_models(TinyBatch *tb, const float *rho, const float *Kinf, const float *Pinf, const float *Quu_inv, const float *AmBKt,
                          const float *Adyn, const float *Bdyn, const float *Q)
{
    CHECK_TB(tb); CHECK_PTR(rho); CHECK_PTR(Kinf); CHECK_PTR(Pinf); CHECK_PTR(Quu_inv); CHECK_PTR(AmBKt); CHECK_PTR(Adyn); CHECK_PTR(Bdyn); CHECK_PTR(Q);
    TRY(set_device(tb));
    const size_t B = tb->batch, nx = tb->nx, nu = tb->nu;
    const float *src[8] = {rho, Kinf, Pinf, Quu_inv, AmBKt, Adyn, Bdyn, Q};
    const size_t sz[8] = {B, B * nu * nx, B * nx * nx, B * nu * nu, B * nx * nx, B * nx * nx, B * nx * nu, B * nx};
    size_t total = 0;
    for (size_t z : sz) total += z;
    float *d = nullptr;
    HIP_TRY(guarded_malloc((void **)&d, total * sizeof(float)));
    int rc = 0;
    size_t o = 0;
    for (int k = 0; k < 8 && rc == 0; k++)
    {
        if (hipMemcpyAsync(d + o, src[k], sz[k] * sizeof(float), hipMemcpyHostToDevice, tb->stream) != hipSuccess) rc = fail(TINY_BATCH_EHIP, "hipMemcpyAsync failed");
        o += sz[k];
    }
    if (rc == 0) rc = set_models_packed(tb, d);
    if (hipStreamSynchronize(tb->stream) != hipSuccess && rc == 0) rc = fail(TINY_BATCH_EHIP, "hipStreamSynchronize failed");
    (void)guarded_free(d);
    return rc;
}

int tiny_batch_clear_models(TinyBatch *tb)
{
    CHECK_TB(tb);
    if (!tb->pm) return 0;
    TRY(set_device(tb));
    invalidate_graph(tb);
    HIP_TRY(hipStreamSynchronize(tb->stream));
    for (float **p : {&tb->pm_src, &tb->pm_rho, &tb->pm_row[0], &tb->pm_row[1]})
    {
        (void)guarded_free(*p);
        *p = nullptr;
    }
    tb->pm_row_dirty[0] = tb->pm_row_dirty[1] = true;
    tb->pm = false;
    return 0;
}

int tiny_batch_models_per_instance(TinyBatch *tb)
{
    CHECK_TB(tb);
    return tb->pm ? 1 : 0;
}

int tiny_batch_riccati_device(int nx, int nu, int count, const double *d_A, const double *d_B, const double *d_Q, const double *d_R, const double *d_rho,
                              double *d_Kinf, double *d_Pinf, double *d_Quu_inv, double *d_AmBKt, double *d_coeff_d2p, int *d_iters, void *hip_stream)
{
    if (nx < 1 || nx > 64 || nu < 1 || nu > 32) return fail(TINY_BATCH_EINVAL, "tiny_batch_riccati_device: need 1 <= nx <= 64 and 1 <= nu <= 32 (got %d, %d)", nx, nu);
    if (count < 1) return fail(TINY_BATCH_EINVAL, "tiny_batch_riccati_device: count must be >= 1 (got %d)", count);
    CHECK_PTR(d_A); CHECK_PTR(d_B); CHECK_PTR(d_Q); CHECK_PTR(d_R); CHECK_PTR(d_rho); CHECK_PTR(d_Kinf); CHECK_PTR(d_Pinf); CHECK_PTR(d_Quu_inv);
    CHECK_PTR(d_AmBKt); CHECK_PTR(d_iters);
    hipStream_t st = (hipStream_t)hip_stream;
    const size_t per = (size_t)riccati_batch_doubles(nx, nu) * sizeof(double);
    long long chunk = (long long)((1ull << 30) / per) / 64 * 64;
    if (chunk < 64) chunk = 64;
    if (chunk > (long long)(count + 63) / 64 * 64) chunk = (long long)(count + 63) / 64 * 64;
    double *scratch = nullptr;
    int *nfail = nullptr;
    HIP_TRY(guarded_malloc((void **)&scratch, (size_t)chunk * per));
    int rc = 0;
    if (guarded_malloc((void **)&nfail, sizeof(int)) != hipSuccess || hipMemsetAsync(nfail, 0, sizeof(int), st) != hipSuccess)
        rc = fail(TINY_BATCH_EHIP, "tiny_batch_riccati_device: allocation failed");
    for (long long s0 = 0; s0 < count && rc == 0; s0 += chunk)
    {
        hipError_t e = launch_riccati_batch(nx, nu, (int)s0, (int)chunk, count, d_A, d_B, d_Q, d_R, d_rho, d_Kinf, d_Pinf, d_Quu_inv, d_AmBKt, d_coeff_d2p, d_iters,
                                            scratch, nfail, st);
        if (e != hipSuccess) rc = fail(TINY_BATCH_EHIP, "kernel launch failed: %s", hipGetErrorString(e));
    }
    int h = 0;
    if (rc == 0 && hipMemcpyAsync(&h, nfail, sizeof(int), hipMemcpyDeviceToHost, st) != hipSuccess) rc = fail(TINY_BATCH_EHIP, "hipMemcpyAsync failed");
    if (hipStreamSynchronize(st) != hipSuccess && rc == 0) rc = fail(TINY_BATCH_EHIP, "hipStreamSynchronize failed");
    (void)guarded_free(scratch);
    (void)guarded_free(nfail);
    return rc ? rc : h;
}

int tiny_batch_set_systems(TinyBatch *tb, const double *A, const double *B, const double *Q, const double *R, const double *rho, int *iters)
{
    CHECK_TB(tb); CHECK_PTR(A); CHECK_PTR(B); CHECK_PTR(Q); CHECK_PTR(R); CHECK_PTR(rho);
    TRY(set_device(tb));
    const size_t Bn = tb->batch, nx = tb->nx, nu = tb->nu;
    const size_t in_sz[5] = {Bn * nx * nx, Bn * nx * nu, Bn * nx, Bn * nu, Bn};
    const size_t out_sz[4] = {Bn * nu * nx, Bn * nx * nx, Bn * nu * nu, Bn * nx * nx};
    const double *in[5] = {A, B, Q, R, rho};
    size_t nd = 0;
    for (size_t z : in_sz) nd += z;
    for (size_t z : out_sz) nd += z;
    const size_t nf = Bn * (1 + pm_gen_floats(tb->nx, tb->nu));
    double *d = nullptr;
    float *f = nullptr;
    int *it = nullptr;
    int rc = 0;
    if (guarded_malloc((void **)&d, nd * sizeof(double)) != hipSuccess || guarded_malloc((void **)&f, nf * sizeof(float)) != hipSuccess ||
        guarded_malloc((void **)&it, Bn * sizeof(int)) != hipSuccess)
        rc = fail(TINY_BATCH_EHIP, "tiny_batch_set_systems: allocation failed");
    double *dp[9];
    size_t o = 0;
    for (int k = 0; k < 5; k++) { dp[k] = d + o; o += in_sz[k]; }
    for (int k = 0; k < 4; k++) { dp[5 + k] = d + o; o += out_sz[k]; }
    for (int k = 0; k < 5 && rc == 0; k++)
        if (hipMemcpyAsync(dp[k], in[k], in_sz[k] * sizeof(double), hipMemcpyHostToDevice, tb->stream) != hipSuccess) rc = fail(TINY_BATCH_EHIP, "hipMemcpyAsync failed");
    int nfail = 0;
    if (rc == 0)
    {
        nfail = tiny_batch_riccati_device(tb->nx, tb->nu, tb->batch, dp[0], dp[1], dp[2], dp[3], dp[4], dp[5], dp[6], dp[7], dp[8], nullptr, it, tb->stream);
        if (nfail < 0) rc = nfail;
    }
    if (rc == 0 && iters && hipMemcpy(iters, it, Bn * sizeof(int), hipMemcpyDeviceToHost) != hipSuccess) rc = fail(TINY_BATCH_EHIP, "hipMemcpy failed");
    if (rc == 0 && nfail > 0) rc = fail(TINY_BATCH_EINVAL, "tiny_batch_set_systems: the Riccati recursion is singular for %d of %zu systems (iters = -1); models unchanged", nfail, Bn);
    if (rc == 0)
    {
        hipLaunchKernelGGL(systems_to_models_kernel, dim3(grid_for((long long)nf)), dim3(256), 0, tb->stream, dp[4], dp[5], dp[6], dp[7], dp[8], dp[0], dp[1], dp[2], f,
                           tb->batch, tb->nx, tb->nu);
        if (hipGetLastError() != hipSuccess) rc = fail(TINY_BATCH_EHIP, "kernel launch failed");
    }
    if (rc == 0) rc = set_models_packed(tb, f);
    if (hipStreamSynchronize(tb->stream) != hipSuccess && rc == 0) rc = fail(TINY_BATCH_EHIP, "hipStreamSynchronize failed");
    (void)guarded_free(d); (void)guarded_free(f); (void)guarded_free(it);
    return rc;
}

int tiny_batch_set_optional_terms(TinyBatch *tb, int en_uref, int en_coeff_d2p)
{
    CHECK_TB(tb);
    tb->en_uref = en_uref != 0;
    tb->en_d2p = en_coeff_d2p != 0;
    invalidate_graph(tb);
    return 0;
}

int tiny_batch_set_input_cost(TinyBatch *tb, const float *R)
{
    CHECK_TB(tb); CHECK_PTR(R);
    tb->Rcost.assign(R, R + tb->nu);
    tb->have_rcost = true;
    tb->gains_dirty = true;
    invalidate_graph(tb);
    return 0;
}

int tiny_batch_set_coeff_d2p(TinyBatch *tb, const float *coeff_d2p)
{
    CHECK_TB(tb); CHECK_PTR(coeff_d2p);
    tb->coeff_d2p.assign(coeff_d2p, coeff_d2p + (size_t)tb->nx * tb->nu);
    tb->gains_dirty = true;
    invalidate_graph(tb);
    return 0;
}

int tiny_batch_set_uref(TinyBatch *tb, const float *uref, int shared)
{
    CHECK_TB(tb); CHECK_PTR(uref);
    TRY(set_device(tb));
    TRY(store_input(tb, tb->in_uref, uref, shared != 0, tb->N - 1, tb->nu));
    return 0;
}

int tiny_batch_set_dispatch(TinyBatch *tb, int mode)
{
    CHECK_TB(tb);
    if (mode < -1 || mode > 2) return fail(TINY_BATCH_EINVAL, "tiny_batch_set_dispatch: mode must be 0 (index order), 1 (longest first, predicted), 2 (longest first by the previous solve's iteration counts) or -1 (automatic)");
    tb->dispatch_mode = mode;
    invalidate_graph(tb);
    return 0;
}

int tiny_batch_set_tile_queue(TinyBatch *tb, int stride)
{
    CHECK_TB(tb);
    if (stride < -1 || stride > 255) return fail(TINY_BATCH_EINVAL, "tiny_batch_set_tile_queue: stride must be -1 (automatic), 0 (one counter) or 1 .. 255");
    tb->tile_queue = stride;
    invalidate_graph(tb);
    return TINY_BATCH_OK;
}

int tiny_batch_dispatch_applied(TinyBatch *tb)
{
    CHECK_TB(tb);
    return tb->last_dispatch;
}

int tiny_batch_set_dispatch_order_device(TinyBatch *tb, const int *d_order)
{
    CHECK_TB(tb);
    tb->order_dev = d_order;
    invalidate_graph(tb);
    return 0;
}

int tiny_batch_set_settings(TinyBatch *tb, float abs_pri_tol, float abs_dua_tol, int max_iter, int check_termination,
                            int en_state_bound, int en_input_bound)
{
    CHECK_TB(tb);
    if (check_termination < 1)
        return fail(TINY_BATCH_EINVAL, "check_termination must be >= 1 (the reference computes iter %% check_termination, admm.cpp:93)");
    if (tb->en_state_bound != en_state_bound || tb->en_input_bound != en_input_bound) tb->derived_dirty[LAYOUT_ROW] = true;
    tb->abs_pri_tol = abs_pri_tol; tb->abs_dua_tol = abs_dua_tol;
    tb->max_iter = max_iter; tb->check_termination = check_termination;
    tb->en_state_bound = en_state_bound; tb->en_input_bound = en_input_bound;
    tb->have_settings = true;
    return 0;
}

int tiny_batch_set_x0(TinyBatch *tb, const float *x0)
{
    CHECK_TB(tb); CHECK_PTR(x0);
    TRY(set_device(tb));
    tb->x0_zero_pending = false;
    HIP_TRY(hipMemcpyAsync(tb->x0buf, x0, (size_t)tb->batch * tb->nx * sizeof(float), hipMemcpyHostToDevice, tb->stream));
    return upload_work(tb, x0, TINY_ARR_X, 0, 1);
}

int tiny_batch_set_x0_device(TinyBatch *tb, const float *d_x0)
{
    CHECK_TB(tb); CHECK_PTR(d_x0);
    TRY(set_device(tb));
    tb->x0_zero_pending = false;
    return launch_pack(tb, d_x0, work_ptr(tb, TINY_ARR_X), tb->layout, 0, tb->batch, false, 0, 1, tb->x0buf);
}

int tiny_batch_set_xref(TinyBatch *tb, const float *xref, int shared)
{
    CHECK_TB(tb); CHECK_PTR(xref);
    TRY(set_device(tb));
    TRY(store_input(tb, tb->in_xref, xref, shared != 0, tb->N, tb->nx));
    tb->xref_mode = 0;
    return 0;
}

int tiny_batch_set_xref_window(TinyBatch *tb, const float *table, int rows, const int *start)
{
    CHECK_TB(tb); CHECK_PTR(table); CHECK_PTR(start);
    if (rows < tb->N) return fail(TINY_BATCH_EINVAL, "trajectory table has %d rows, need at least N=%d", rows, tb->N);
    for (int b = 0; b < tb->batch; b++)
        if (start[b] < 0 || start[b] + tb->N > rows)
            return fail(TINY_BATCH_EINVAL, "window start[%d]=%d out of range for %d rows, N=%d", b, start[b], rows, tb->N);
    TRY(set_device(tb));
    std::vector<float> tt((size_t)rows * 4 * tb->NXC, 0.f), tr((size_t)rows * tb->rw, 0.f);
    for (int r = 0; r < rows; r++)
        for (int row = 0; row < tb->nx; row++)
        {
            const float v = table[(size_t)r * tb->nx + row];
            tt[((size_t)r * 4 + (row & 3)) * tb->NXC + (row >> 2)] = v;
            if (row < tb->rw) tr[(size_t)r * tb->rw + row] = v;
        }
    if (tb->table_rows != rows)
    {
        (void)guarded_free(tb->tab_tile); (void)guarded_free(tb->tab_row); (void)guarded_free(tb->tab_row_h);
        tb->tab_tile = tb->tab_row = tb->tab_row_h = nullptr;
    }
    TRY(upload_vec(tb, &tb->tab_tile, tt));
    TRY(upload_vec(tb, &tb->tab_row, tr));
    {
        std::vector<_Float16> th(tr.size());
        for (size_t e = 0; e < tr.size(); e++) th[e] = (_Float16)tr[e];
        std::vector<float> packed(tr.size() / 2);
        std::memcpy(packed.data(), th.data(), packed.size() * sizeof(float));
        TRY(upload_vec(tb, &tb->tab_row_h, packed));
    }
    HIP_TRY(hipMemcpyAsync(tb->xref_start, start, (size_t)tb->batch * sizeof(int), hipMemcpyHostToDevice, tb->stream));
    HIP_TRY(hipStreamSynchronize(tb->stream));
    tb->table_rows = rows;
    tb->xref_mode = 1;
    invalidate_graph(tb);
    return 0;
}

int tiny_batch_set_xmin(TinyBatch *tb, const float *s, int shared) { return set_bound(tb, s, shared, 0); }
int tiny_batch_set_xmax(TinyBatch *tb, const float *s, int shared) { return set_bound(tb, s, shared, 1); }
int tiny_batch_set_umin(TinyBatch *tb, const float *s, int shared) { return set_bound(tb, s, shared, 2); }
int tiny_batch_set_umax(TinyBatch *tb, const float *s, int shared) { return set_bound(tb, s, shared, 3); }

int tiny_batch_reset_dual_variables(TinyBatch *tb)
{
    CHECK_TB(tb);
    tb->duals_zero_pending = true;
    return 0;
}

int tiny_batch_solve_async(TinyBatch *tb)
{
    CHECK_TB(tb);
    KernelPlan pl;
    TRY(prepare_solve(tb, false, &pl));
    return enqueue_solve(tb, pl, tb->timing);
}

int tiny_batch_wait(TinyBatch *tb, int *n_unsolved)
{
    CHECK_TB(tb);
    TRY(set_device(tb));
    int n = 0;
    HIP_TRY(hipMemcpyAsync(&n, tb->n_unsolved, sizeof(int), hipMemcpyDeviceToHost, tb->stream));
    HIP_TRY(hipStreamSynchronize(tb->stream));
    if (n_unsolved) *n_unsolved = n;
    return 0;
}

int tiny_batch_solve(TinyBatch *tb)
{
    TRY(tiny_batch_solve_async(tb));
    int n = 0;
    TRY(tiny_batch_wait(tb, &n));
    return n > 0 ? 1 : 0;
}

int tiny_batch_group_solve(TinyBatch **tbs, int n, int *n_unsolved)
{
    CHECK_PTR(tbs);
    if (n < 1) return fail(TINY_BATCH_EINVAL, "tiny_batch_group_solve: need at least one handle");
    for (int i = 0; i < n; i++)
    {
        CHECK_TB(tbs[i]);
        for (int j = 0; j < i; j++)
            if (tbs[j] == tbs[i]) return fail(TINY_BATCH_EINVAL, "tiny_batch_group_solve: handle %d appears twice", i);
    }
    for (int i = 0; i < n; i++)
    {
        TinyBatch *tb = tbs[i];
        if (!tb->stream)
        {
            TRY(set_device(tb));
            HIP_TRY(hipStreamSynchronize(nullptr));
            if (!tb->own_stream) HIP_TRY(hipStreamCreateWithFlags(&tb->own_stream, hipStreamNonBlocking));
            tb->stream = tb->own_stream;
        }
        TRY(tiny_batch_solve_async(tb));
    }
    int total = 0;
    for (int i = 0; i < n; i++)
    {
        int u = 0;
        TRY(tiny_batch_wait(tbs[i], &u));
        total += u;
    }
    if (n_unsolved) *n_unsolved = total;
    return total > 0 ? 1 : 0;
}

int tiny_batch_group_gather_u0(TinyBatch **tbs, int n, int dst_device, float *d_dst)
{
    CHECK_PTR(tbs); CHECK_PTR(d_dst);
    if (n < 1) return fail(TINY_BATCH_EINVAL, "tiny_batch_group_gather_u0: need at least one handle");
    for (int i = 0; i < n; i++)
    {
        CHECK_TB(tbs[i]);
        if (tbs[i]->nu != tbs[0]->nu) return fail(TINY_BATCH_EINVAL, "tiny_batch_group_gather_u0: handle %d has nu=%d, handle 0 nu=%d", i, tbs[i]->nu, tbs[0]->nu);
    }
    size_t off = 0;
    for (int i = 0; i < n; i++)
    {
        TinyBatch *tb = tbs[i];
        const size_t cnt = (size_t)tb->batch * tb->nu;
        TRY(set_device(tb));
        if (tb->device == dst_device)
            TRY(launch_unpack(tb, work_ptr(tb, TINY_ARR_U), d_dst + off, tb->layout, 1, tb->batch, 0, 1));
        else
        {
            if (!tb->u0_stage) TRY(dev_alloc_zero(&tb->u0_stage, cnt));
            TRY(launch_unpack(tb, work_ptr(tb, TINY_ARR_U), tb->u0_stage, tb->layout, 1, tb->batch, 0, 1));
            HIP_TRY(hipMemcpyPeerAsync(d_dst + off, dst_device, tb->u0_stage, tb->device, cnt * sizeof(float), tb->stream));
        }
        off += cnt;
    }
    for (int i = 0; i < n; i++)
    {
        TRY(set_device(tbs[i]));
        HIP_TRY(hipStreamSynchronize(tbs[i]->stream));
    }
    return 0;
}

int tiny_batch_group_get_u0(TinyBatch **tbs, int n, float *u0_host)
{
    CHECK_PTR(tbs); CHECK_PTR(u0_host);
    if (n < 1) return fail(TINY_BATCH_EINVAL, "tiny_batch_group_get_u0: need at least one handle");
    size_t total = 0;
    for (int i = 0; i < n; i++) { CHECK_TB(tbs[i]); total += (size_t)tbs[i]->batch * tbs[i]->nu; }
    TRY(set_device(tbs[0]));
    float *d = nullptr;
    HIP_TRY(guarded_malloc((void **)&d, total * sizeof(float)));
    int rc = tiny_batch_group_gather_u0(tbs, n, tbs[0]->device, d);
    if (rc == 0)
    {
        (void)hipSetDevice(tbs[0]->device);
        hipError_t e = hipMemcpy(u0_host, d, total * sizeof(float), hipMemcpyDeviceToHost);
        if (e != hipSuccess) rc = fail(TINY_BATCH_EHIP, "tiny_batch_group_get_u0: %s", hipGetErrorString(e));
    }
    (void)hipSetDevice(tbs[0]->device);
    (void)guarded_free(d);
    return rc;
}

int tiny_batch_forward_pass(TinyBatch *tb) { CHECK_TB(tb); return run_step(tb, STEP_FORWARD_PASS, nullptr, nullptr); }
int tiny_batch_update_slack(TinyBatch *tb) { CHECK_TB(tb); return run_step(tb, STEP_UPDATE_SLACK, nullptr, nullptr); }
int tiny_batch_update_dual(TinyBatch *tb) { CHECK_TB(tb); return run_step(tb, STEP_UPDATE_DUAL, nullptr, nullptr); }
int tiny_batch_update_linear_cost(TinyBatch *tb) { CHECK_TB(tb); return run_step(tb, STEP_UPDATE_LINEAR_COST, nullptr, nullptr); }
int tiny_batch_backward_pass_grad(TinyBatch *tb) { CHECK_TB(tb); return run_step(tb, STEP_BACKWARD_PASS_GRAD, nullptr, nullptr); }
int tiny_batch_termination_condition(TinyBatch *tb, int *converged)
{
    CHECK_TB(tb);
    int n_true = 0;
    TRY(run_step(tb, STEP_TERMINATION_CONDITION, converged, &n_true));
    return n_true;
}

int tiny_batch_get_x(TinyBatch *tb, float *x) { return tiny_batch_get_array(tb, TINY_ARR_X, x); }
int tiny_batch_get_u(TinyBatch *tb, float *u) { return tiny_batch_get_array(tb, TINY_ARR_U, u); }

int tiny_batch_get_status(TinyBatch *tb, int *iter, int *status, float *residuals)
{
    CHECK_TB(tb);
    TRY(set_device(tb));
    TRY(flush_pending(tb));
    if (iter) HIP_TRY(hipMemcpyAsync(iter, tb->iter, (size_t)tb->batch * sizeof(int), hipMemcpyDeviceToHost, tb->stream));
    if (status) HIP_TRY(hipMemcpyAsync(status, tb->status, (size_t)tb->batch * sizeof(int), hipMemcpyDeviceToHost, tb->stream));
    if (residuals) HIP_TRY(hipMemcpyAsync(residuals, tb->res, (size_t)tb->batch * 4 * sizeof(float), hipMemcpyDeviceToHost, tb->stream));
    HIP_TRY(hipStreamSynchronize(tb->stream));
    return 0;
}

int tiny_batch_set_status(TinyBatch *tb, const int *iter, const int *status, const float *residuals)
{
    CHECK_TB(tb);
    TRY(set_device(tb));
    TRY(flush_pending(tb));
    if (iter) { HIP_TRY(hipMemcpyAsync(tb->iter, iter, (size_t)tb->batch * sizeof(int), hipMemcpyHostToDevice, tb->stream)); tb->iter_history = false; }
    if (status) HIP_TRY(hipMemcpyAsync(tb->status, status, (size_t)tb->batch * sizeof(int), hipMemcpyHostToDevice, tb->stream));
    if (residuals) HIP_TRY(hipMemcpyAsync(tb->res, residuals, (size_t)tb->batch * 4 * sizeof(float), hipMemcpyHostToDevice, tb->stream));
    HIP_TRY(hipStreamSynchronize(tb->stream));
    return 0;
}

int tiny_batch_set_array(TinyBatch *tb, int id, const float *src)
{
    CHECK_TB(tb); CHECK_PTR(src);
    if (id < 0 || id >= TINY_ARR_COUNT) return fail(TINY_BATCH_EINVAL, "bad array id %d", id);
    TRY(set_device(tb));
    TRY(flush_pending(tb));
    TRY(upload_work(tb, src, id, 0, is_xfam(id) ? tb->N : tb->N - 1));
    if (id == TINY_ARR_X)
        TRY(launch_unpack(tb, work_ptr(tb, TINY_ARR_X), tb->x0buf, tb->layout, 0, tb->batch, 0, 1));
    return 0;
}

int tiny_batch_get_array(TinyBatch *tb, int id, float *dst)
{
    CHECK_TB(tb); CHECK_PTR(dst);
    if (id < 0 || id >= TINY_ARR_COUNT) return fail(TINY_BATCH_EINVAL, "bad array id %d", id);
    TRY(set_device(tb));
    TRY(flush_pending(tb));
    return download_work(tb, id, dst, 0, is_xfam(id) ? tb->N : tb->N - 1);
}

int tiny_batch_reset_workspace(TinyBatch *tb)
{
    CHECK_TB(tb);
    TRY(set_device(tb));
    tb->x0_zero_pending = true;
    tb->cold_pending = true;
    tb->duals_zero_pending = false;
    tb->iter_history = false;
    return 0;
}

int tiny_batch_set_array_device(TinyBatch *tb, int id, const float *d_src)
{
    CHECK_TB(tb); CHECK_PTR(d_src);
    if (id < 0 || id >= TINY_ARR_COUNT) return fail(TINY_BATCH_EINVAL, "bad array id %d", id);
    TRY(set_device(tb));
    TRY(flush_pending(tb));
    const int fam = is_xfam(id) ? 0 : 1;
    TRY(launch_pack(tb, d_src, work_ptr(tb, id), tb->layout, fam, tb->batch, false, 0, fam ? tb->N - 1 : tb->N));
    if (id == TINY_ARR_X) TRY(launch_unpack(tb, work_ptr(tb, TINY_ARR_X), tb->x0buf, tb->layout, 0, tb->batch, 0, 1));
    return 0;
}

int tiny_batch_get_array_device(TinyBatch *tb, int id, float *d_dst)
{
    CHECK_TB(tb); CHECK_PTR(d_dst);
    if (id < 0 || id >= TINY_ARR_COUNT) return fail(TINY_BATCH_EINVAL, "bad array id %d", id);
    TRY(set_device(tb));
    TRY(flush_pending(tb));
    const int fam = is_xfam(id) ? 0 : 1;
    return launch_unpack(tb, work_ptr(tb, id), d_dst, tb->layout, fam, tb->batch, 0, fam ? tb->N - 1 : tb->N);
}

int tiny_batch_set_xref_device(TinyBatch *tb, const float *d_xref, int shared)
{
    CHECK_TB(tb); CHECK_PTR(d_xref);
    TRY(set_device(tb));
    TRY(store_input(tb, tb->in_xref, d_xref, shared != 0, tb->N, tb->nx, hipMemcpyDeviceToDevice));
    tb->xref_mode = 0;
    return 0;
}

int tiny_batch_get_u0_device(TinyBatch *tb, float *d_u0)
{
    CHECK_TB(tb); CHECK_PTR(d_u0);
    TRY(set_device(tb));
    return launch_unpack(tb, work_ptr(tb, TINY_ARR_U), d_u0, tb->layout, 1, tb->batch, 0, 1);
}

int tiny_batch_mpc_step_async(TinyBatch *tb, int window_advance)
{
    CHECK_TB(tb);
    if (tb->nx > 64) return fail(TINY_BATCH_EUNSUPPORTED, "mpc_step supports nx <= 64");
    if (window_advance < 0) return fail(TINY_BATCH_EINVAL, "tiny_batch_mpc_step_async: window_advance must be >= 0 (got %d): the window gather clamps at the last table row only", window_advance);
    tb->duals_zero_pending = true;
    TRY(tiny_batch_solve_async(tb));
    return enqueue_plant_step(tb, window_advance);
}

int tiny_batch_mpc_run_traj_async(TinyBatch *tb, int steps, int window_advance, float *d_u0_traj)
{
    CHECK_TB(tb);
    if (steps < 1) return fail(TINY_BATCH_EINVAL, "tiny_batch_mpc_run_async: steps must be >= 1");
    if (window_advance < 0) return fail(TINY_BATCH_EINVAL, "tiny_batch_mpc_run_async: window_advance must be >= 0 (got %d): the window gather clamps at the last table row only", window_advance);
    if (tb->nx > 64) return fail(TINY_BATCH_EUNSUPPORTED, "mpc_run supports nx <= 64");
    if (tb->max_iter <= 0) return fail(TINY_BATCH_EINVAL, "tiny_batch_mpc_run_async needs max_iter > 0");
    TRY(set_device(tb));
    const bool from_reset = tb->cold_pending;
    TRY(flush_pending(tb));
    tb->duals_zero_pending = true;
    KernelPlan pl;
    TRY(prepare_solve(tb, steps > 1, &pl));
    const size_t u0n = (size_t)tb->batch * tb->nu;
    if (traits(pl.kernel).onchip_mpc && !tb->h16 && steps > 1 && bounds_all_shared(tb))
    {
        RowParams P;
        fill_row_params(tb, P, pl.exact);
        P.mpc_steps = steps; P.window_advance = window_advance; P.u0_traj = d_u0_traj;
        const int applied = enqueue_dispatch_order(tb, pl, steps, from_reset, P);
        if (applied < 0) return applied;
        tb->last_dispatch = applied;
        const hipError_t e = launch_kernel(tb, pl, P);
        if (e != hipSuccess) return fail(TINY_BATCH_EHIP, "kernel launch failed: %s", hipGetErrorString(e));
        if (d_u0_traj) TRY(launch_unpack(tb, work_ptr(tb, TINY_ARR_U), d_u0_traj + (size_t)(steps - 1) * u0n, tb->layout, 1, tb->batch, 0, 1));
        TRY(enqueue_plant_step(tb, window_advance));
        tb->duals_zero_pending = tb->cold_pending = false;
        tb->iter_history = true;
        tb->ev_valid = false;
        return 0;
    }
    if (!tb->stream)
    {
        HIP_TRY(hipStreamSynchronize(nullptr));
        if (!tb->own_stream) HIP_TRY(hipStreamCreateWithFlags(&tb->own_stream, hipStreamNonBlocking));
        tb->stream = tb->own_stream;
    }
    char sig[560];
    snprintf(sig, sizeof sig, "%p|%p|%p|%d|%d|%d|%s|%d|%d|%g|%g|%d|%d|%p|%p|%p|%d|%p|%p|%p|%p|%d%d|%a|%d%d%d|%d%d|%d|%p|%p|%p", (void *)tb->pm_src, (void *)tb->pm_row[0],
             (void *)tb->pm_row[1], steps, window_advance, tb->variant, kernel_name(tb, pl).c_str(), tb->max_iter,
             tb->check_termination, (double)tb->abs_pri_tol, (double)tb->abs_dua_tol, tb->xref_mode, tb->table_rows, (void *)tb->pair[0],
             (void *)tb->arr[0], (void *)tb->r_bounds, (int)tb->h16, (void *)tb->stream, (void *)d_u0_traj, (void *)tb->r_xref,
             (void *)tb->r_uref, (int)tb->en_uref, (int)tb->en_d2p, (double)tb->rho, (int)bounds_all_shared(tb),
             (int)(tb->in_xref.set && tb->in_xref.shared), (int)(tb->in_uref.set && tb->in_uref.shared), tb->en_state_bound, tb->en_input_bound,
             tb->dispatch_mode, (void *)tb->order_dev, (void *)tb->mats_exact, (void *)tb->xref_start);
    if (!tb->graph_exec || tb->graph_sig != sig)
    {
        if (tb->graph_exec) { (void)hipGraphExecDestroy(tb->graph_exec); tb->graph_exec = nullptr; }
        hipGraph_t graph = nullptr;
        HIP_TRY(hipStreamBeginCapture(tb->stream, hipStreamCaptureModeThreadLocal));
        int rc = 0;
        for (int k = 0; k < steps && rc == 0; k++)
        {
            tb->duals_zero_pending = true;
            rc = enqueue_solve(tb, pl, false);
            if (rc == 0 && d_u0_traj) rc = launch_unpack(tb, work_ptr(tb, TINY_ARR_U), d_u0_traj + (size_t)k * u0n, tb->layout, 1, tb->batch, 0, 1);
            if (rc == 0) rc = enqueue_plant_step(tb, window_advance);
        }
        hipError_t ec = hipStreamEndCapture(tb->stream, &graph);
        if (rc) { if (graph) (void)hipGraphDestroy(graph); return rc; }
        HIP_TRY(ec);
        hipError_t ei = hipGraphInstantiate(&tb->graph_exec, graph, nullptr, nullptr, 0);
        (void)hipGraphDestroy(graph);
        HIP_TRY(ei);
        tb->graph_sig = sig;
        tb->graph_captures++;
    }
    HIP_TRY(hipGraphLaunch(tb->graph_exec, tb->stream));
    tb->duals_zero_pending = tb->cold_pending = false;
    tb->ev_valid = false;
    return 0;
}

int tiny_batch_mpc_run_async(TinyBatch *tb, int steps, int window_advance)
{
    return tiny_batch_mpc_run_traj_async(tb, steps, window_advance, nullptr);
}

int tiny_batch_mpc_run_traj(TinyBatch *tb, int steps, int window_advance, float *u0_traj_host)
{
    CHECK_TB(tb); CHECK_PTR(u0_traj_host);
    if (steps < 1) return fail(TINY_BATCH_EINVAL, "tiny_batch_mpc_run_traj: steps must be >= 1");
    TRY(set_device(tb));
    const size_t n = (size_t)steps * tb->batch * tb->nu;
    float *d = nullptr;
    HIP_TRY(guarded_malloc((void **)&d, n * sizeof(float)));
    int rc = tiny_batch_mpc_run_traj_async(tb, steps, window_advance, d);
    if (rc == 0)
    {
        hipError_t e = hipStreamSynchronize(tb->stream);
        if (e == hipSuccess) e = hipMemcpy(u0_traj_host, d, n * sizeof(float), hipMemcpyDeviceToHost);
        if (e != hipSuccess) rc = fail(TINY_BATCH_EHIP, "tiny_batch_mpc_run_traj: %s", hipGetErrorString(e));
    }
    (void)guarded_free(d);
    return rc;
}

int tiny_batch_get_x0(TinyBatch *tb, float *x0)
{
    CHECK_TB(tb); CHECK_PTR(x0);
    TRY(set_device(tb));
    TRY(flush_x0_zero(tb));
    HIP_TRY(hipMemcpyAsync(x0, tb->x0buf, (size_t)tb->batch * tb->nx * sizeof(float), hipMemcpyDeviceToHost, tb->stream));
    HIP_TRY(hipStreamSynchronize(tb->stream));
    return 0;
}

int tiny_batch_enable_timing(TinyBatch *tb, int on)
{
    CHECK_TB(tb);
    tb->timing = on != 0;
    tb->ev_valid = false;
    return 0;
}

int tiny_batch_last_solve_ms(TinyBatch *tb, float *ms)
{
    CHECK_TB(tb); CHECK_PTR(ms);
    if (!tb->ev_valid) return fail(TINY_BATCH_ENOTREADY, "no timed solve recorded (call tiny_batch_enable_timing first)");
    TRY(set_device(tb));
    HIP_TRY(hipEventSynchronize(tb->ev1));
    HIP_TRY(hipEventElapsedTime(ms, tb->ev0, tb->ev1));
    return 0;
}

const char *tiny_batch_kernel_name(TinyBatch *tb)
{
    if (!tb) return "";
    if (tb->tile16_ok && !tb->h16 && tb->derived_dirty[LAYOUT_ROW] && tile16_per_instance(tb))
    {
        const std::string keep = g_err;
        KernelPlan pl;
        (void)prepare_solve(tb, false, &pl);
        g_err = keep;
    }
    return plan_name(tb, false);
}

int tiny_batch_debug_graph_captures(TinyBatch *tb)
{
    CHECK_TB(tb);
    return tb->graph_captures;
}

int tiny_batch_debug_guards(int on)
{
    std::lock_guard<std::mutex> lk(g_guard_mu);
    g_guards_on = on != 0;
    return 0;
}

long long tiny_batch_debug_check(void)
{
    std::lock_guard<std::mutex> lk(g_guard_mu);
    if (g_guarded.empty()) return 0;
    unsigned long long *bad = nullptr, host = 0;
    if (hipMalloc((void **)&bad, sizeof *bad) != hipSuccess || hipMemset(bad, 0, sizeof *bad) != hipSuccess) return fail(TINY_BATCH_EHIP, "tiny_batch_debug_check: allocation failed");
    if (hipDeviceSynchronize() != hipSuccess) { (void)hipFree(bad); return fail(TINY_BATCH_EHIP, "tiny_batch_debug_check: a kernel faulted: %s", hipGetErrorString(hipGetLastError())); }
    for (const auto &kv : g_guarded)
    {
        char *u = (char *)kv.first;
        hipLaunchKernelGGL(guard_count_kernel, dim3(1), dim3(256), 0, nullptr, (const unsigned *)(u - kGuard * sizeof(float)), kGuard, bad);
        hipLaunchKernelGGL(guard_count_kernel, dim3(1), dim3(256), 0, nullptr, (const unsigned *)(u + kv.second), kGuard, bad);
    }
    hipError_t e = hipMemcpy(&host, bad, sizeof host, hipMemcpyDeviceToHost);
    (void)hipFree(bad);
    if (e != hipSuccess) return fail(TINY_BATCH_EHIP, "tiny_batch_debug_check: %s", hipGetErrorString(e));
    return (long long)host;
}

int tiny_batch_debug_poke(TinyBatch *tb, int which)
{
    CHECK_TB(tb);
    TRY(set_device(tb));
    float *arr = tb->layout == LAYOUT_ROW ? tb->pair[0] : tb->arr[0];
// ... 101 lines not shown
```

accelerated-tinympc_amd/csrc/tinympc_internal.h:

```cpp
#pragma once
#include <hip/hip_runtime.h>
#include <stddef.h>
#include <stdint.h>

namespace tinympc
{

constexpr int TILE = 16;
constexpr int WAVE = 64;
constexpr int TINY_STATUS_SOLVED_ = 1;
constexpr int TINY_STATUS_UNSOLVED_ = 11;

#define TINY_FOR_EACH_DIMS(X) X(3, 1) X(1, 1) X(8, 4) X(2, 1) X(16, 8)

template <int NXC_, int NUC_>
struct Dims
{
    static constexpr int NXC = NXC_;
    static constexpr int NUC = NUC_;
    static constexpr int NCH = NXC_ + NUC_;
    static constexpr int NT = (NCH + 3) / 4;
    static constexpr int NTX = (NXC_ + 3) / 4;
    static constexpr int TU0 = NXC_ / 4;
    static constexpr int NTU = NT - TU0;
    static constexpr int N_A1 = NT * NXC_;
    static constexpr int N_A2 = NTX * NUC_;
    static constexpr int N_A3 = NT * NXC_;
    static constexpr int N_A4 = NTX * NUC_;
    static constexpr int N_A5 = NTU * NUC_;
    static constexpr int N_AP = NTX * NXC_;
    static constexpr int N_OPND = N_A1 + N_A2 + N_A3 + N_A4 + N_A5 + N_AP;
};

struct SolveParams
{
    int nx, nu, N, batch, ntiles;
    float rho, abs_pri_tol, abs_dua_tol;
    int max_iter, check_termination, en_state_bound, en_input_bound;
    int duals_zero;
    int cold_start;
    int xref_mode;
    float *x, *q, *p, *v, *vnew, *g;
    float *u, *r, *d, *z, *znew, *y;
    const float *xmin, *xmax, *umin, *umax, *xref;
    long long xb_tile_stride, ub_tile_stride, xref_tile_stride;
    const float *xref_table;
    const int *xref_start;
    int table_rows;
    float *res;
    int *status;
    int *iter;
    int *n_unsolved;
    const float *opnd;
    const float *qvec;
};

#define TINY_FOR_EACH_ROWLANE(X) X(12, 4, 30) X(12, 4, 25) X(12, 4, 20) X(12, 4, 10) X(4, 1, 10) X(8, 3, 7) X(12, 4, 40) X(12, 4, 50)

struct RowParams
{
    int nx, nu, N, batch;
    float rho, abs_pri_tol, abs_dua_tol;
    int max_iter, check_termination;
    int duals_zero, cold_start;
    int xref_mode;
    float *xu, *qr, *pd, *vz, *vzn, *gy;
    const float *xref;
    unsigned xref_inst_stride;
    unsigned pi_flags;
    const float *xref_table;
    int *xref_start;
    int table_rows;
    const float *bounds;
    unsigned bounds_inst_stride;
    const float *mats;
    const float *uref;
    unsigned uref_inst_stride;
    int en_d2p;
    const int *order;
    float *res;
    int *status, *iter, *n_unsolved;
    int mpc_steps, window_advance;
    float *u0_traj;
    float *x0buf;
    int dual32;
};

struct ModelParams
{
    const float *mats = nullptr;
    unsigned mats_stride = 0;
    const float *rho = nullptr;
};
__host__ __device__ inline int pm_row_floats(int nx, int nu) { return (3 * nx + 2 * nu + 1) * 16; }
__host__ __device__ inline int pm_gen_floats(int nx, int nu) { return nu * nx + nx * nx + nu * nu + nx * nx + nx * nx + nx * nu + nx; }

__host__ __device__ inline int riccati_batch_doubles(int nx, int nu) { return 4 * nx * nx + 3 * nu * nx + nu * (nx > nu ? nx : nu) + 2 * nu * nu; }
hipError_t launch_riccati_batch(int nx, int nu, int s0, int n, int count, const double *A, const double *B, const double *Q, const double *R, const double *rho,
                                double *Kinf, double *Pinf, double *Quu_inv, double *AmBKt, double *coeff_d2p, int *iters, double *scratch, int *nfail,
                                hipStream_t stream);

#define TINY_FOR_EACH_ROWDIMS(X) X(12, 4) X(4, 1) X(8, 3) X(8, 4) X(12, 2) X(4, 2) X(4, 4) X(2, 2)
#define TINY_FOR_EXACT_H16(exact, h16, X, NX, NU)  \
    do                                             \
    {                                              \
        if ((exact) && !(h16)) X(NX, NU, true, false); \
        else if (exact) X(NX, NU, true, true);     \
        else if (!(h16)) X(NX, NU, false, false);  \
        else X(NX, NU, false, true);               \
    } while (0)
enum { STEP_FORWARD_PASS = 0, STEP_UPDATE_SLACK, STEP_UPDATE_DUAL, STEP_UPDATE_LINEAR_COST, STEP_TERMINATION_CONDITION,
       STEP_BACKWARD_PASS_GRAD };

typedef float f32x4 __attribute__((ext_vector_type(4)));

bool rowlane_supported(int nx, int nu, int N);
hipError_t launch_admm_rowlane(int nx, int nu, int N, bool exact, bool h16, const RowParams &P, hipStream_t stream);
hipError_t launch_admm_rowlane_pm(int nx, int nu, int N, bool exact, const RowParams &P, const ModelParams &M, hipStream_t stream);
bool rowdims_supported(int nx, int nu);
hipError_t launch_admm_rowstream(int nx, int nu, bool exact, bool h16, const RowParams &P, hipStream_t stream);
hipError_t launch_admm_step(int nx, int nu, bool exact, bool h16, int fn, const RowParams &P, int *conv_out, hipStream_t stream);

bool rowloop_supported(int nx, int nu, int N);
hipError_t launch_admm_rowloop(int nx, int nu, bool exact, bool h16, const RowParams &P, hipStream_t stream);

bool quadlane_supported(int nx, int nu, int N);
hipError_t launch_admm_quadlane(int N, bool exact, bool h16, const RowParams &P, hipStream_t stream);

bool tile16_supported(int nx, int nu, int N);
hipError_t launch_admm_tile16(int N, bool exact, const RowParams &P, hipStream_t stream, int n_cu, int tail = -1);
hipError_t launch_admm_tile16_pi(int N, bool exact, bool bounds_ring, bool xref_ring, const RowParams &P, hipStream_t stream, int n_cu, int tail = -1);
size_t tile16_pi_lds_bytes(int N, bool bounds_ring, bool xref_ring, unsigned pi_flags, int table_rows);
int tile16_max_table_rows();

#define TINY_FOR_EACH_WAVEDIMS(X) X(32, 16) X(16, 8) X(16, 4) X(20, 8) X(24, 4)
bool wavedims_supported(int nx, int nu);
hipError_t launch_admm_wavestream(int nx, int nu, const RowParams &P, hipStream_t stream);
bool waveres_supported(int nx, int nu, int N);
hipError_t launch_admm_waveres(int nx, int nu, bool exact, const RowParams &P, hipStream_t stream);
bool tile48_supported(int nx, int nu, int N);
hipError_t launch_admm_tile48(int N, bool exact, const RowParams &P, hipStream_t stream);

hipError_t launch_admm_stream(int nxc, int nuc, const SolveParams &P, hipStream_t stream);
bool generic_exact_supported(int nx, int nu);
hipError_t launch_admm_generic(const SolveParams &P, const float *gains, int nxc, int nuc, hipStream_t stream);
hipError_t launch_admm_generic_pm(const SolveParams &P, const ModelParams &M, int nxc, int nuc, hipStream_t stream);

hipError_t launch_dispatch_order(int nx, int nu, bool h16, const RowParams &P, float *key, int *order, hipStream_t stream, int tile = 0);
hipError_t launch_dispatch_order_history(const int *iter, int batch, int unit, int *order, int *counters, hipStream_t stream, int use_sum = 0);

}
```

accelerated-tinympc_amd/solver.py:

```python
from __future__ import annotations

import ctypes as C
from pathlib import Path

import numpy as np

import os

from . import build as _build

PKG = Path(__file__).resolve().parent
LIB_PATH = PKG / "lib" / "libtinympc_hip.so"

ARRAY_IDS = {"x": 0, "u": 1, "q": 2, "r": 3, "p": 4, "d": 5, "v": 6, "vnew": 7, "z": 8, "znew": 9, "g": 10, "y": 11}
X_FAMILY = ("x", "q", "p", "v", "vnew", "g")
TINY_SOLVED, TINY_UNSOLVED = 1, 11

_lib = None


class TinyBatchError(RuntimeError):
    pass


def load_library(build_if_missing: bool = False) -> C.CDLL:
    global _lib
    if _lib is not None:
        return _lib
    if not LIB_PATH.exists():
        if build_if_missing:
            _build.build()
        else:
            raise TinyBatchError(f"{LIB_PATH} is missing: run `python accelerated-tinympc_amd/build.py` "
                                 "(hipcc --offload-arch=gfx950); there is no CPU fallback")
    override = os.environ.get("TINYMPC_HIP_LIB")
    if override:
        import warnings
        warnings.warn(f"TINYMPC_HIP_LIB is set: loading {override} instead of {LIB_PATH}", RuntimeWarning)
    lib = C.CDLL(override or str(LIB_PATH))
    F, I, P = C.POINTER(C.c_float), C.POINTER(C.c_int), C.c_void_p
    D = C.POINTER(C.c_double)
    sig = {
        "tiny_batch_create": [C.POINTER(P), C.c_int, C.c_int, C.c_int, C.c_int, C.c_int],
        "tiny_batch_set_stream": [P, P],
        "tiny_batch_synchronize": [P],
        "tiny_batch_set_cache": [P, C.c_float, F, F, F, F],
        "tiny_batch_set_dynamics": [P, F, F, F],
        "tiny_batch_set_settings": [P, C.c_float, C.c_float, C.c_int, C.c_int, C.c_int, C.c_int],
        "tiny_batch_set_x0": [P, F],
        "tiny_batch_set_xref": [P, F, C.c_int],
        "tiny_batch_set_xref_window": [P, F, C.c_int, I],
        "tiny_batch_set_umin": [P, F, C.c_int], "tiny_batch_set_umax": [P, F, C.c_int],
        "tiny_batch_set_xmin": [P, F, C.c_int], "tiny_batch_set_xmax": [P, F, C.c_int],
        "tiny_batch_reset_dual_variables": [P],
        "tiny_batch_solve": [P], "tiny_batch_solve_async": [P], "tiny_batch_wait": [P, I],
        "tiny_batch_get_x": [P, F], "tiny_batch_get_u": [P, F],
        "tiny_batch_forward_pass": [P], "tiny_batch_update_slack": [P], "tiny_batch_update_dual": [P],
        "tiny_batch_update_linear_cost": [P], "tiny_batch_backward_pass_grad": [P], "tiny_batch_termination_condition": [P, I],
        "tiny_batch_get_status": [P, I, I, F], "tiny_batch_set_status": [P, I, I, F],
        "tiny_batch_set_array": [P, C.c_int, F], "tiny_batch_get_array": [P, C.c_int, F],
        "tiny_batch_reset_workspace": [P],
        "tiny_batch_set_x0_device": [P, P], "tiny_batch_get_u0_device": [P, P],
        "tiny_batch_mpc_step_async": [P, C.c_int], "tiny_batch_get_x0": [P, F],
        "tiny_batch_mpc_run_async": [P, C.c_int, C.c_int], "tiny_batch_mpc_run_traj_async": [P, C.c_int, C.c_int, P], "tiny_batch_mpc_run_traj": [P, C.c_int, C.c_int, F],
        "tiny_batch_enable_timing": [P, C.c_int], "tiny_batch_last_solve_ms": [P, F],
        "tiny_batch_select_kernel": [P, C.c_int], "tiny_batch_arithmetic": [P], "tiny_batch_debug_graph_captures": [P], "tiny_batch_set_storage": [P, C.c_int], "tiny_batch_set_storage_ex": [P, C.c_int, C.c_int],
        "tiny_batch_set_row_kernel": [P, C.c_int],
        "tiny_batch_set_dispatch": [P, C.c_int], "tiny_batch_set_tile_queue": [P, C.c_int], "tiny_batch_set_dispatch_order_device": [P, P], "tiny_batch_dispatch_applied": [P],
        "tiny_batch_set_optional_terms": [P, C.c_int, C.c_int], "tiny_batch_set_input_cost": [P, F],
        "tiny_batch_set_coeff_d2p": [P, F], "tiny_batch_set_uref": [P, F, C.c_int],
        "tiny_batch_group_solve": [C.POINTER(P), C.c_int, I],
        "tiny_batch_group_gather_u0": [C.POINTER(P), C.c_int, C.c_int, P], "tiny_batch_group_get_u0": [C.POINTER(P), C.c_int, F],
        "tiny_batch_set_array_device": [P, C.c_int, P], "tiny_batch_get_array_device": [P, C.c_int, P],
        "tiny_batch_set_xref_device": [P, P, C.c_int],
        "tiny_riccati": [C.c_int, C.c_int, D, D, D, D, C.c_double, D, D, D, D, D, I],
        "tiny_batch_set_models": [P, F, F, F, F, F, F, F, F], "tiny_batch_set_models_device": [P, P, P, P, P, P, P, P, P],
        "tiny_batch_clear_models": [P], "tiny_batch_models_per_instance": [P],
        "tiny_batch_riccati_device": [C.c_int, C.c_int, C.c_int, P, P, P, P, P, P, P, P, P, P, P, P],
        "tiny_batch_set_systems": [P, D, D, D, D, D, I],
    }
    for name, args in sig.items():
        fn = getattr(lib, name)
        fn.argtypes, fn.restype = args, C.c_int
    sig64 = {
        "tiny_batch64_create": [C.POINTER(P), C.c_int, C.c_int, C.c_int, C.c_int, C.c_int],
        "tiny_batch64_set_cache": [P, C.c_double, D, D, D, D], "tiny_batch64_set_dynamics": [P, D, D, D],
        "tiny_batch64_set_settings": [P, C.c_double, C.c_double, C.c_int, C.c_int, C.c_int, C.c_int],
        "tiny_batch64_set_x0": [P, D], "tiny_batch64_set_xref": [P, D, C.c_int],
        "tiny_batch64_set_xmin": [P, D, C.c_int], "tiny_batch64_set_xmax": [P, D, C.c_int],
        "tiny_batch64_set_umin": [P, D, C.c_int], "tiny_batch64_set_umax": [P, D, C.c_int],
        "tiny_batch64_reset_dual_variables": [P], "tiny_batch64_solve": [P],
        "tiny_batch64_set_array": [P, C.c_int, D], "tiny_batch64_get_array": [P, C.c_int, D],
        "tiny_batch64_get_status": [P, I, I, D], "tiny_batch64_set_status": [P, I, I, D],
        "tiny_batch64_select_kernel": [P, C.c_int], "tiny_batch64_mpc_step": [P], "tiny_batch64_get_first_columns": [P, D, D],
        "tiny_batch64_forward_pass": [P], "tiny_batch64_update_slack": [P], "tiny_batch64_update_dual": [P],
        "tiny_batch64_update_linear_cost": [P], "tiny_batch64_backward_pass_grad": [P], "tiny_batch64_termination_condition": [P, I],
    }
    for name, args in sig64.items():
        fn = getattr(lib, name)
        fn.argtypes, fn.restype = args, C.c_int
    lib.tiny_batch64_destroy.argtypes, lib.tiny_batch64_destroy.restype = [P], None
    lib.tiny_batch64_last_error.argtypes, lib.tiny_batch64_last_error.restype = [], C.c_char_p
    lib.tiny_batch64_kernel_name.argtypes, lib.tiny_batch64_kernel_name.restype = [P], C.c_char_p
    lib.tiny_batch_debug_guards.argtypes, lib.tiny_batch_debug_guards.restype = [C.c_int], C.c_int
    lib.tiny_batch_debug_check.argtypes, lib.tiny_batch_debug_check.restype = [], C.c_longlong
    lib.tiny_batch_debug_poke.argtypes, lib.tiny_batch_debug_poke.restype = [P, C.c_int], C.c_int
    lib.tiny_batch_destroy.argtypes, lib.tiny_batch_destroy.restype = [P], None
    lib.tiny_batch_last_error.argtypes, lib.tiny_batch_last_error.restype = [], C.c_char_p
    lib.tiny_batch_kernel_name.argtypes, lib.tiny_batch_kernel_name.restype = [P], C.c_char_p
    lib.tiny_batch_closed_loop_kernel_name.argtypes, lib.tiny_batch_closed_loop_kernel_name.restype = [P], C.c_char_p
    _lib = lib
    return lib


def debug_guards(on: bool):
    load_library().tiny_batch_debug_guards(1 if on else 0)


def debug_check() -> int:
    n = load_library().tiny_batch_debug_check()
    if n < 0:
        raise TinyBatchError(f"tiny_batch_debug_check: {load_library().tiny_batch_last_error().decode()} ({n})")
    return int(n)


def exported_symbols():
    import re
    txt = (PKG.parent / "include" / "tinympc_batch.h").read_text() + (PKG.parent / "include" / "tinympc_batch64.h").read_text()
    return sorted(set(re.findall(r"\b(tiny_(?:batch(?:64)?_[a-z0-9_]+|riccati))\s*\(", txt)))


def _f32(a):
    return np.ascontiguousarray(a, dtype=np.float32)


def _fp(a):
    return a.ctypes.data_as(C.POINTER(C.c_float))


def _colmajor(m):
    return np.ascontiguousarray(np.asarray(m, dtype=np.float32).T).ravel()


def riccati(nx, nu, A, B, Q, R, rho):
    lib = load_library()
    dp = lambda a: a.ctypes.data_as(C.POINTER(C.c_double))
    a = np.ascontiguousarray(np.asarray(A, np.float64).T).ravel()
    b = np.ascontiguousarray(np.asarray(B, np.float64).T).ravel()
    q = np.ascontiguousarray(Q, np.float64).ravel()
    r = np.ascontiguousarray(R, np.float64).ravel()
    K, Pm, Qi, Am, cd = (np.zeros(nu * nx), np.zeros(nx * nx), np.zeros(nu * nu), np.zeros(nx * nx), np.zeros(nx * nu))
    it = C.c_int(0)
    rc = lib.tiny_riccati(nx, nu, dp(a), dp(b), dp(q), dp(r), float(rho), dp(K), dp(Pm), dp(Qi), dp(Am), dp(cd), C.byref(it))
    if rc != 0:
        raise TinyBatchError(f"tiny_riccati failed rc={rc}")
    return dict(Kinf=K.reshape(nx, nu).T.copy(), Pinf=Pm.reshape(nx, nx).T.copy(), Quu_inv=Qi.reshape(nu, nu).T.copy(),
                AmBKt=Am.reshape(nx, nx).T.copy(), coeff_d2p=cd.reshape(nu, nx).T.copy(), iters=it.value)


def _colmajor_batch(m, dtype=np.float32):
    a = np.asarray(m, dtype=dtype)
    return np.ascontiguousarray(np.swapaxes(a, 1, 2)).reshape(a.shape[0], -1)


def _hip():
    hip = C.CDLL(os.path.join(os.environ.get("ROCM_PATH", "/opt/rocm"), "lib", "libamdhip64.so"))
    hip.hipMalloc.argtypes, hip.hipMalloc.restype = [C.POINTER(C.c_void_p), C.c_size_t], C.c_int
    hip.hipFree.argtypes, hip.hipFree.restype = [C.c_void_p], C.c_int
    hip.hipMemcpy.argtypes, hip.hipMemcpy.restype = [C.c_void_p, C.c_void_p, C.c_size_t, C.c_int], C.c_int
    return hip


def riccati_batch(nx, nu, A, B, Q, R, rho, coeff_d2p: bool = True) -> dict:
    lib, hip = load_library(), _hip()
    S = int(np.asarray(rho).shape[0])
    ins = [_colmajor_batch(A, np.float64), _colmajor_batch(B, np.float64), np.asarray(Q, np.float64).reshape(S, nx),
           np.asarray(R, np.float64).reshape(S, nu), np.asarray(rho, np.float64).reshape(S)]
    shp = {"Kinf": (nx, nu), "Pinf": (nx, nx), "Quu_inv": (nu, nu), "AmBKt": (nx, nx), "coeff_d2p": (nu, nx)}
    if not coeff_d2p:
        del shp["coeff_d2p"]
    outs = {k: np.full((S, a * b), np.nan) for k, (a, b) in shp.items()}
    it = np.zeros(S, np.int32)
    host = [np.ascontiguousarray(a) for a in ins] + list(outs.values()) + [it]
    dev = []
    try:
        for a in host:
            p = C.c_void_p()
            if hip.hipMalloc(C.byref(p), a.nbytes) != 0:
                raise TinyBatchError("hipMalloc failed")
            dev.append(p)
            if hip.hipMemcpy(p, a.ctypes.data, a.nbytes, 1) != 0:
                raise TinyBatchError("hipMemcpy failed")
        rc = lib.tiny_batch_riccati_device(nx, nu, S, *(dev if coeff_d2p else dev[:9] + [None] + dev[9:]), None)
        if rc < 0:
            raise TinyBatchError(f"rc={rc}: {lib.tiny_batch_last_error().decode()}")
        for a, p in zip(host[5:], dev[5:]):
            if hip.hipMemcpy(a.ctypes.data, p, a.nbytes, 2) != 0:
                raise TinyBatchError("hipMemcpy failed")
    finally:
        for p in dev:
            hip.hipFree(p)
    res = {k: np.swapaxes(v.reshape(S, *shp[k]), 1, 2).copy() for k, v in outs.items()}
    res["iters"] = it
    return res


def solve_group(solvers) -> int:
    lib = load_library()
    hs = (C.c_void_p * len(solvers))(*[s._h for s in solvers])
    n = C.c_int(0)
    rc = lib.tiny_batch_group_solve(hs, len(solvers), C.byref(n))
    if rc < 0:
        raise TinyBatchError(f"rc={rc}: {lib.tiny_batch_last_error().decode()}")
    return n.value


class TinyBatchSolver:

    def __init__(self, prob: dict, batch: int, device: int = 0, settings: dict | None = None):
        self.lib = load_library()
        self.nx, self.nu, self.N, self.B = int(prob["nx"]), int(prob["nu"]), int(prob["N"]), int(batch)
# ... 76 lines not shown
            assert a.shape == (self.B, steps, dim), (a.shape, (self.B, steps, dim))
            shared = 0
        self._check(fn(self._h, _fp(a), shared))

    def set_xref(self, xref):
        self._set_steps(self.lib.tiny_batch_set_xref, xref, self.N, self.nx)

    def set_optional_terms(self, en_uref=False, en_coeff_d2p=False):
        self._check(self.lib.tiny_batch_set_optional_terms(self._h, int(bool(en_uref)), int(bool(en_coeff_d2p))))

    def set_input_cost(self, R):
        a = _f32(np.asarray(R).ravel()); assert a.shape == (self.nu,), a.shape
        self._check(self.lib.tiny_batch_set_input_cost(self._h, _fp(a)))

    def set_coeff_d2p(self, coeff_d2p):
        assert np.asarray(coeff_d2p).shape == (self.nx, self.nu)
        a = _colmajor(coeff_d2p)
        self._check(self.lib.tiny_batch_set_coeff_d2p(self._h, _fp(a)))

    def set_uref(self, uref):
        self._set_steps(self.lib.tiny_batch_set_uref, uref, self.N - 1, self.nu)

    def set_xref_window(self, table, start):
        t = _f32(table); s = np.ascontiguousarray(start, dtype=np.int32)
        assert t.ndim == 2 and t.shape[1] == self.nx and s.shape == (self.B,)
        self._check(self.lib.tiny_batch_set_xref_window(self._h, _fp(t), t.shape[0], s.ctypes.data_as(C.POINTER(C.c_int))))

    def set_umin(self, a): self._set_steps(self.lib.tiny_batch_set_umin, a, self.N - 1, self.nu)
    def set_umax(self, a): self._set_steps(self.lib.tiny_batch_set_umax, a, self.N - 1, self.nu)
    def set_xmin(self, a): self._set_steps(self.lib.tiny_batch_set_xmin, a, self.N, self.nx)
    def set_xmax(self, a): self._set_steps(self.lib.tiny_batch_set_xmax, a, self.N, self.nx)

    def set_bounds(self, x_min, x_max, u_min, u_max):
        self.set_xmin(x_min); self.set_xmax(x_max); self.set_umin(u_min); self.set_umax(u_max)

    def reset_dual_variables(self):
        self._check(self.lib.tiny_batch_reset_dual_variables(self._h))

    def solve(self) -> int:
        return self._check(self.lib.tiny_batch_solve(self._h))

    call_tiny_solve = solve

    def solve_async(self):
        self._check(self.lib.tiny_batch_solve_async(self._h))

    def wait(self) -> int:
        n = C.c_int(0)
        self._check(self.lib.tiny_batch_wait(self._h, C.byref(n)))
        return n.value

    def forward_pass(self): self._check(self.lib.tiny_batch_forward_pass(self._h))
    def update_slack(self): self._check(self.lib.tiny_batch_update_slack(self._h))
    def update_dual(self): self._check(self.lib.tiny_batch_update_dual(self._h))
    def update_linear_cost(self): self._check(self.lib.tiny_batch_update_linear_cost(self._h))
    def backward_pass_grad(self): self._check(self.lib.tiny_batch_backward_pass_grad(self._h))

    def termination_condition(self):
        conv = np.zeros(self.B, np.int32)
        self._check(self.lib.tiny_batch_termination_condition(self._h, conv.ctypes.data_as(C.POINTER(C.c_int))))
        return conv.astype(bool)

    def get_x(self): return self.get_array("x")
    def get_u(self): return self.get_array("u")

    def get_status(self):
        it = np.zeros(self.B, np.int32); st = np.zeros(self.B, np.int32); res = np.zeros((self.B, 4), np.float32)
        ip = lambda a: a.ctypes.data_as(C.POINTER(C.c_int))
        self._check(self.lib.tiny_batch_get_status(self._h, ip(it), ip(st), _fp(res)))
        return it, st, res

    def set_status(self, iter=None, status=None, residuals=None):
        ip = lambda a: None if a is None else np.ascontiguousarray(a, np.int32).ctypes.data_as(C.POINTER(C.c_int))
        keep = [None if a is None else np.ascontiguousarray(a, np.int32) for a in (iter, status)]
        r = None if residuals is None else _f32(residuals)
        self._check(self.lib.tiny_batch_set_status(
            self._h, None if keep[0] is None else keep[0].ctypes.data_as(C.POINTER(C.c_int)),
            None if keep[1] is None else keep[1].ctypes.data_as(C.POINTER(C.c_int)), None if r is None else _fp(r)))

    def get_array(self, name):
        out = np.empty(self._xshape(name), np.float32)
        self._check(self.lib.tiny_batch_get_array(self._h, ARRAY_IDS[name], _fp(out)))
        return out

    def set_array(self, name, arr):
        a = _f32(arr); assert a.shape == self._xshape(name), (name, a.shape)
        self._check(self.lib.tiny_batch_set_array(self._h, ARRAY_IDS[name], _fp(a)))

    def get_state(self) -> dict:
        st = {k: self.get_array(k) for k in ARRAY_IDS}
        st["iter"], st["status"], st["residuals"] = self.get_status()
        return st

    def set_state(self, st: dict):
        for k in ARRAY_IDS:
            if k in st:
                self.set_array(k, st[k])
        self.set_status(st.get("iter"), st.get("status"), st.get("residuals"))

    def reset_workspace(self):
        self._check(self.lib.tiny_batch_reset_workspace(self._h))

    def mpc_step_async(self, window_advance: int = 0):
        self._check(self.lib.tiny_batch_mpc_step_async(self._h, window_advance))

    def mpc_run_async(self, steps: int, window_advance: int = 0):
        self._check(self.lib.tiny_batch_mpc_run_async(self._h, steps, window_advance))

    def mpc_run_traj(self, steps: int, window_advance: int = 0) -> np.ndarray:
        out = np.zeros((steps, self.B, self.nu), np.float32)
        self._check(self.lib.tiny_batch_mpc_run_traj(self._h, steps, window_advance, _fp(out)))
        return out

    def get_x0(self):
        out = np.empty((self.B, self.nx), np.float32)
        self._check(self.lib.tiny_batch_get_x0(self._h, _fp(out)))
        return out

    def synchronize(self):
        self._check(self.lib.tiny_batch_synchronize(self._h))

    def enable_timing(self, on=True):
        self._check(self.lib.tiny_batch_enable_timing(self._h, 1 if on else 0))

    def last_solve_ms(self) -> float:
        ms = C.c_float(0)
        self._check(self.lib.tiny_batch_last_solve_ms(self._h, C.byref(ms)))
        return ms.value

    def kernel_name(self) -> str:
        return self.lib.tiny_batch_kernel_name(self._h).decode()

    def closed_loop_kernel_name(self) -> str:
        return self.lib.tiny_batch_closed_loop_kernel_name(self._h).decode()

    def arithmetic(self) -> str:
        rc = self.lib.tiny_batch_arithmetic(self._h)
        if rc < 0:
            self._check(rc)
        return "exact" if rc == 0 else "fma"

    def select_kernel(self, variant: int):
        self._check(self.lib.tiny_batch_select_kernel(self._h, variant))

    def set_row_kernel(self, family: int):
        self._check(self.lib.tiny_batch_set_row_kernel(self._h, family))

    def set_dispatch(self, mode: int):
        self._check(self.lib.tiny_batch_set_dispatch(self._h, mode))

    def set_tile_queue(self, stride: int):
        self._check(self.lib.tiny_batch_set_tile_queue(self._h, stride))

    def dispatch_applied(self) -> int:
        return self._check(self.lib.tiny_batch_dispatch_applied(self._h))

    def set_dispatch_order_device(self, d_order_ptr):
        self._check(self.lib.tiny_batch_set_dispatch_order_device(self._h, C.c_void_p(d_order_ptr)))

    def set_storage(self, bits: int, dual_bits: int | None = None):
        if dual_bits is None:
            self._check(self.lib.tiny_batch_set_storage(self._h, bits))
        else:
            self._check(self.lib.tiny_batch_set_storage_ex(self._h, bits, dual_bits))

    def set_stream(self, stream_ptr: int):
        self._check(self.lib.tiny_batch_set_stream(self._h, C.c_void_p(stream_ptr)))


class TinyBatchSolver64:

    def __init__(self, prob: dict, batch: int, device: int = 0, settings: dict | None = None):
        self.lib = load_library()
        self.nx, self.nu, self.N, self.B = int(prob["nx"]), int(prob["nu"]), int(prob["N"]), int(batch)
        self._h = C.c_void_p()
        self._check(self.lib.tiny_batch64_create(C.byref(self._h), self.nx, self.nu, self.N, self.B, int(device)))
        cm = lambda m: np.ascontiguousarray(np.asarray(m, np.float64).T).ravel()
        dp = lambda a: a.ctypes.data_as(C.POINTER(C.c_double))
        k, p, qi, am = (cm(prob[n]) for n in ("Kinf", "Pinf", "Quu_inv", "AmBKt"))
        self._check(self.lib.tiny_batch64_set_cache(self._h, float(prob["rho"]), dp(k), dp(p), dp(qi), dp(am)))
        a, b, q = cm(prob["Adyn"]), cm(prob["Bdyn"]), np.ascontiguousarray(np.asarray(prob["Q"], np.float64).ravel())
        self._check(self.lib.tiny_batch64_set_dynamics(self._h, dp(a), dp(b), dp(q)))
        s = dict(abs_pri_tol=1e-3, abs_dua_tol=1e-3, max_iter=100, check_termination=1, en_state_bound=1, en_input_bound=1)
        if settings:
            s.update(settings)
        self.set_settings(**s)

    def _check(self, rc):
        if rc < 0:
            raise TinyBatchError(f"rc={rc}: {self.lib.tiny_batch64_last_error().decode()}")
        return rc

    def close(self):
        if getattr(self, "_h", None) and self._h.value:
            self.lib.tiny_batch64_destroy(self._h)
            self._h = C.c_void_p()

    def __del__(self):
        try:
            self.close()
        except Exception:
            pass

    @staticmethod
    def _dp(a):
        return a.ctypes.data_as(C.POINTER(C.c_double))

    def _xshape(self, name):
        return (self.B, self.N, self.nx) if name in X_FAMILY else (self.B, self.N - 1, self.nu)

    def set_settings(self, abs_pri_tol, abs_dua_tol, max_iter, check_termination, en_state_bound, en_input_bound):
        self.settings = dict(abs_pri_tol=abs_pri_tol, abs_dua_tol=abs_dua_tol, max_iter=max_iter, check_termination=check_termination,
                             en_state_bound=en_state_bound, en_input_bound=en_input_bound)
        self._check(self.lib.tiny_batch64_set_settings(self._h, abs_pri_tol, abs_dua_tol, max_iter, check_termination, en_state_bound, en_input_bound))

    def set_x0(self, x0):
        a = np.ascontiguousarray(x0, np.float64); assert a.shape == (self.B, self.nx), a.shape
        self._check(self.lib.tiny_batch64_set_x0(self._h, self._dp(a)))

    def _set_steps(self, fn, arr, steps, dim):
        a = np.ascontiguousarray(arr, np.float64)
        shared = 1 if a.shape == (steps, dim) else 0
        assert shared or a.shape == (self.B, steps, dim), a.shape
        self._check(fn(self._h, self._dp(a), shared))

    def set_xref(self, xref): self._set_steps(self.lib.tiny_batch64_set_xref, xref, self.N, self.nx)

    def set_bounds(self, x_min, x_max, u_min, u_max):
        self._set_steps(self.lib.tiny_batch64_set_xmin, x_min, self.N, self.nx)
        self._set_steps(self.lib.tiny_batch64_set_xmax, x_max, self.N, self.nx)
        self._set_steps(self.lib.tiny_batch64_set_umin, u_min, self.N - 1, self.nu)
        self._set_steps(self.lib.tiny_batch64_set_umax, u_max, self.N - 1, self.nu)

    def reset_dual_variables(self): self._check(self.lib.tiny_batch64_reset_dual_variables(self._h))

    def select_kernel(self, which: int):
        self._check(self.lib.tiny_batch64_select_kernel(self._h, which))

    def kernel_name(self) -> str: return self.lib.tiny_batch64_kernel_name(self._h).decode()

    def forward_pass(self): self._check(self.lib.tiny_batch64_forward_pass(self._h))
    def update_slack(self): self._check(self.lib.tiny_batch64_update_slack(self._h))
    def update_dual(self): self._check(self.lib.tiny_batch64_update_dual(self._h))
    def update_linear_cost(self): self._check(self.lib.tiny_batch64_update_linear_cost(self._h))
    def backward_pass_grad(self): self._check(self.lib.tiny_batch64_backward_pass_grad(self._h))

    def termination_condition(self):
        conv = np.zeros(self.B, np.int32)
        self._check(self.lib.tiny_batch64_termination_condition(self._h, conv.ctypes.data_as(C.POINTER(C.c_int))))
        return conv.astype(bool)

    def mpc_step(self) -> int:
        return self._check(self.lib.tiny_batch64_mpc_step(self._h))

    def first_columns(self):
        x0, u0 = np.empty((self.B, self.nx)), np.empty((self.B, self.nu))
        self._check(self.lib.tiny_batch64_get_first_columns(self._h, self._dp(x0), self._dp(u0)))
        return x0, u0

    def solve(self) -> int: return self._check(self.lib.tiny_batch64_solve(self._h))

    def get_array(self, name):
        out = np.empty(self._xshape(name), np.float64)
        self._check(self.lib.tiny_batch64_get_array(self._h, ARRAY_IDS[name], self._dp(out)))
        return out

    def set_array(self, name, arr):
        a = np.ascontiguousarray(arr, np.float64); assert a.shape == self._xshape(name), (name, a.shape)
        self._check(self.lib.tiny_batch64_set_array(self._h, ARRAY_IDS[name], self._dp(a)))

    def get_u(self): return self.get_array("u")

    def get_status(self):
        it = np.zeros(self.B, np.int32); st = np.zeros(self.B, np.int32); res = np.zeros((self.B, 4), np.float64)
        ip = lambda a: a.ctypes.data_as(C.POINTER(C.c_int))
        self._check(self.lib.tiny_batch64_get_status(self._h, ip(it), ip(st), self._dp(res)))
        return it, st, res

    def get_state(self) -> dict:
        st = {k: self.get_array(k) for k in ARRAY_IDS}
        st["iter"], st["status"], st["residuals"] = self.get_status()
        return st

    def set_state(self, st: dict):
        for k in ARRAY_IDS:
            if k in st:
                self.set_array(k, st[k])
        ip = lambda a: np.ascontiguousarray(a, np.int32)
        it, sta, res = ip(st["iter"]), ip(st["status"]), np.ascontiguousarray(st["residuals"], np.float64)
        self._check(self.lib.tiny_batch64_set_status(self._h, it.ctypes.data_as(C.POINTER(C.c_int)), sta.ctypes.data_as(C.POINTER(C.c_int)), self._dp(res)))
```

include/tinympc_batch.h:

```cpp
#ifndef TINYMPC_BATCH_H
#define TINYMPC_BATCH_H

#ifdef __cplusplus
extern "C"
{
#endif

    typedef struct TinyBatch TinyBatch;

    typedef enum
    {
        TINY_BATCH_OK = 0,
        TINY_BATCH_EINVAL = -1,
        TINY_BATCH_EHIP = -2,
        TINY_BATCH_EUNSUPPORTED = -3,
        TINY_BATCH_ENOTREADY = -4
    } TinyBatchError;

#define TINY_STATUS_SOLVED 1
#define TINY_STATUS_UNSOLVED 11

    typedef enum
    {
        TINY_ARR_X = 0, TINY_ARR_U = 1, TINY_ARR_Q = 2, TINY_ARR_R = 3, TINY_ARR_P = 4, TINY_ARR_D = 5,
        TINY_ARR_V = 6, TINY_ARR_VNEW = 7, TINY_ARR_Z = 8, TINY_ARR_ZNEW = 9, TINY_ARR_G = 10, TINY_ARR_Y = 11,
        TINY_ARR_COUNT = 12
    } TinyBatchArray;

    const char *tiny_batch_last_error(void);

    int tiny_batch_create(TinyBatch **out, int nx, int nu, int N, int batch, int device);
    void tiny_batch_destroy(TinyBatch *tb);
    int tiny_batch_set_stream(TinyBatch *tb, void *hip_stream);
    int tiny_batch_synchronize(TinyBatch *tb);

    int tiny_batch_set_cache(TinyBatch *tb, float rho, const float *Kinf , const float *Pinf ,
                             const float *Quu_inv , const float *AmBKt );
    int tiny_batch_set_dynamics(TinyBatch *tb, const float *Adyn , const float *Bdyn ,
                                const float *Q );
    int tiny_batch_set_settings(TinyBatch *tb, float abs_pri_tol, float abs_dua_tol, int max_iter,
                                int check_termination, int en_state_bound, int en_input_bound);

    int tiny_batch_set_x0(TinyBatch *tb, const float *x0 );
    int tiny_batch_set_xref(TinyBatch *tb, const float *xref , int shared);
    int tiny_batch_set_xref_window(TinyBatch *tb, const float *table , int rows,
                                   const int *start );
    int tiny_batch_set_umin(TinyBatch *tb, const float *umin , int shared);
    int tiny_batch_set_umax(TinyBatch *tb, const float *umax, int shared);
    int tiny_batch_set_xmin(TinyBatch *tb, const float *xmin , int shared);
    int tiny_batch_set_xmax(TinyBatch *tb, const float *xmax, int shared);
    int tiny_batch_reset_dual_variables(TinyBatch *tb);
    int tiny_batch_solve(TinyBatch *tb);
    int tiny_batch_get_x(TinyBatch *tb, float *x );
    int tiny_batch_get_u(TinyBatch *tb, float *u );
    int tiny_batch_get_status(TinyBatch *tb, int *iter , int *status , float *residuals );

    int tiny_batch_forward_pass(TinyBatch *tb);
    int tiny_batch_update_slack(TinyBatch *tb);
    int tiny_batch_update_dual(TinyBatch *tb);
    int tiny_batch_update_linear_cost(TinyBatch *tb);
    int tiny_batch_backward_pass_grad(TinyBatch *tb);
    int tiny_batch_termination_condition(TinyBatch *tb, int *converged );

    int tiny_batch_solve_async(TinyBatch *tb);
    int tiny_batch_wait(TinyBatch *tb, int *n_unsolved);

    int tiny_batch_group_solve(TinyBatch **tbs, int n, int *n_unsolved);
    int tiny_batch_group_gather_u0(TinyBatch **tbs, int n, int dst_device, float *d_dst);
    int tiny_batch_group_get_u0(TinyBatch **tbs, int n, float *u0_host);

    int tiny_batch_set_array(TinyBatch *tb, int array_id, const float *src);
    int tiny_batch_get_array(TinyBatch *tb, int array_id, float *dst);
    int tiny_batch_set_status(TinyBatch *tb, const int *iter, const int *status, const float *residuals);
    int tiny_batch_reset_workspace(TinyBatch *tb);

    int tiny_batch_set_x0_device(TinyBatch *tb, const float *d_x0 );
    int tiny_batch_get_u0_device(TinyBatch *tb, float *d_u0 );
    int tiny_batch_set_array_device(TinyBatch *tb, int array_id, const float *d_src);
    int tiny_batch_get_array_device(TinyBatch *tb, int array_id, float *d_dst);
    int tiny_batch_set_xref_device(TinyBatch *tb, const float *d_xref , int shared);

    int tiny_batch_mpc_step_async(TinyBatch *tb, int window_advance);
    int tiny_batch_mpc_run_async(TinyBatch *tb, int steps, int window_advance);
    int tiny_batch_mpc_run_traj_async(TinyBatch *tb, int steps, int window_advance, float *d_u0_traj);
    int tiny_batch_mpc_run_traj(TinyBatch *tb, int steps, int window_advance, float *u0_traj_host);
    int tiny_batch_get_x0(TinyBatch *tb, float *x0 );

    int tiny_batch_enable_timing(TinyBatch *tb, int on);
    int tiny_batch_last_solve_ms(TinyBatch *tb, float *ms);
    const char *tiny_batch_kernel_name(TinyBatch *tb);
    const char *tiny_batch_closed_loop_kernel_name(TinyBatch *tb);
    int tiny_batch_debug_guards(int on);
    int tiny_batch_debug_graph_captures(TinyBatch *tb);
    long long tiny_batch_debug_check(void);
    int tiny_batch_debug_poke(TinyBatch *tb, int which);
    enum { TINY_BATCH_ARITH_EXACT = 0, TINY_BATCH_ARITH_FMA = 1 };
    int tiny_batch_arithmetic(TinyBatch *tb);
    int tiny_batch_select_kernel(TinyBatch *tb, int variant);
    int tiny_batch_set_row_kernel(TinyBatch *tb, int family);
    int tiny_batch_set_storage(TinyBatch *tb, int bits);
    int tiny_batch_set_storage_ex(TinyBatch *tb, int bits, int dual_bits);

    int tiny_batch_set_dispatch(TinyBatch *tb, int mode);
    int tiny_batch_set_tile_queue(TinyBatch *tb, int stride);
    int tiny_batch_dispatch_applied(TinyBatch *tb);
    int tiny_batch_set_dispatch_order_device(TinyBatch *tb, const int *d_order);

    int tiny_batch_set_optional_terms(TinyBatch *tb, int en_uref, int en_coeff_d2p);
    int tiny_batch_set_input_cost(TinyBatch *tb, const float *R);
    int tiny_batch_set_coeff_d2p(TinyBatch *tb, const float *coeff_d2p);
    int tiny_batch_set_uref(TinyBatch *tb, const float *uref, int shared);

    int tiny_batch_set_models(TinyBatch *tb, const float *rho , const float *Kinf , const float *Pinf ,
                              const float *Quu_inv , const float *AmBKt , const float *Adyn ,
                              const float *Bdyn , const float *Q );
    int tiny_batch_set_models_device(TinyBatch *tb, const float *d_rho, const float *d_Kinf, const float *d_Pinf, const float *d_Quu_inv,
                                     const float *d_AmBKt, const float *d_Adyn, const float *d_Bdyn, const float *d_Q);
    int tiny_batch_clear_models(TinyBatch *tb);
    int tiny_batch_models_per_instance(TinyBatch *tb);
    int tiny_batch_riccati_device(int nx, int nu, int count, const double *d_A, const double *d_B, const double *d_Q, const double *d_R,
                                  const double *d_rho, double *d_Kinf, double *d_Pinf, double *d_Quu_inv, double *d_AmBKt,
                                  double *d_coeff_d2p, int *d_iters, void *hip_stream);
    int tiny_batch_set_systems(TinyBatch *tb, const double *A, const double *B, const double *Q, const double *R, const double *rho, int *iters);

    int tiny_riccati(int nx, int nu, const double *A, const double *B, const double *Q, const double *R, double rho,
                     double *Kinf, double *Pinf, double *Quu_inv, double *AmBKt, double *coeff_d2p, int *iters);

#ifdef __cplusplus
}
#endif
#endif
```

Baseline: 46.15 million solves/s.

## Group instances into tiles by reference-window start via a device-built instance map

Adds a bucket-sort instance map that permutes instances so each 16-wide tile holds instances with similar xref window start. The cold-start tile16 kernel and the dispatch-order key kernel read instances through this map, which should make iteration counts within a tile more uniform and cut divergence and wasted work. It also changes the two-ended tail-stride heuristic when grouping is on. In exchange it adds scattered, non-contiguous global writes and extra map loads, plus two small kernels whenever the map is rebuilt. The map is cached and only rebuilt when marked dirty.

```diff
diff --git a/accelerated-tinympc_amd/csrc/admm_tile16.hip b/accelerated-tinympc_amd/csrc/admm_tile16.hip
--- a/accelerated-tinympc_amd/csrc/admm_tile16.hip
+++ b/accelerated-tinympc_amd/csrc/admm_tile16.hip
@@ -483,8 +483,12 @@
     if (P.order) tile = P.order[slot];
     const bool tile_ok = tile >= 0 && tile < ntiles;
     T16_STAMP(stamp_k, 3, (unsigned long long)(unsigned)tile);
-    const int inst = tile * 16 + c;
-    const bool valid = tile_ok && inst < P.batch;
+    constexpr bool GM = COLD && !MPC && !BR && !XR;
+    int inst = tile * 16 + c;
+    if constexpr (GM)
+        if (P.inst_map) inst = P.inst_map[(tile_ok ? tile : 0) * 16 + c];
+    auto in_batch = [&](int i) { return GM ? (unsigned)i < (unsigned)P.batch : i < P.batch; };
+    const bool valid = tile_ok && in_batch(inst);
     const int inst_a = valid ? inst : P.batch - 1;
 
     float a[N][4];
@@ -859,12 +863,33 @@
     }
     T16_STAMP(stamp_k, 1, __builtin_amdgcn_s_memrealtime());
 
+    auto inst_of = [&](int col) {
+        if constexpr (GM)
+        {
+            int tl = tile_ok ? tile : 0;
+            asm volatile("" : "+s"(tl));
+            if (P.inst_map) return P.inst_map[tl * 16 + col];
+            return tl * 16 + col;
+        }
+        else return tile * 16 + col;
+    };
+    int inst_e = inst, ebase_e = ebase;
+    bool valid_e = valid;
+    if constexpr (GM)
+    {
+        unsigned ll = lane;
+        asm volatile("" : "+v"(ll));
+        inst_e = inst_of((int)(ll & 15u));
+        valid_e = tile_ok && in_batch(inst_e);
+        ebase_e = ((valid_e ? inst_e : P.batch - 1) * N) * 16 + (int)(ll >> 4);
+    }
+
     if (P.max_iter <= 0)
     {
-        if (valid && g == 0)
-        {
-            P.status[inst] = TINY_STATUS_UNSOLVED_;
-            P.iter[inst] = 1;
+        if (valid_e && g == 0)
+        {
+            P.status[inst_e] = TINY_STATUS_UNSOLVED_;
+            P.iter[inst_e] = 1;
             atomicAdd(P.n_unsolved, 1);
         }
         T16_STAMP(stamp_k, 2, __builtin_amdgcn_s_memrealtime());
@@ -877,20 +902,20 @@
     {
         const bool solved = st == TINY_STATUS_SOLVED_;
         const int c2 = lane >> 2, q2 = lane & 3;
-        const int inst2 = tile * 16 + c2;
-        const bool valid2 = tile_ok && inst2 < P.batch;
+        const int inst2 = inst_of(c2);
+        const bool valid2 = tile_ok && in_batch(inst2);
         const int obase2 = ((valid2 ? inst2 : 0) * N) * 16 + 4 * q2;
         typedef float float_ma __attribute__((may_alias));
         typedef f32x4 f32x4_ma __attribute__((may_alias));
         float_ma *const stage_w = reinterpret_cast<float_ma *>(lds4 + wv * (N * WAVE));
         const int rd_off = (c2 * 4 + q2);
-        const int obase4 = ebase + 3 * g;
+        const int obase4 = ebase_e + 3 * g;
         constexpr bool XPOSE = TINY_T16_XPOSE && !(EXACT && !COLD && !MPC);
         auto put = [&](float *dst, int i, const f32x4 &val) {
             if constexpr (XPOSE)
             {
                 const f32x4 o = t16_transpose4(val);
-                if (valid) *reinterpret_cast<f32x4 *>(dst + obase4 + i * 16) = o;
+                if (valid_e) *reinterpret_cast<f32x4 *>(dst + obase4 + i * 16) = o;
                 return;
             }
             float_ma *slot = stage_w + i * (WAVE * 4);
@@ -922,9 +947,10 @@
                 }
                 return vzv;
             };
-            const int instL = tile * 16 + (c & 7);
-            const bool validL = tile_ok && instL < P.batch, validH = tile_ok && instL + 8 < P.batch;
-            const int obaseL = (validL ? instL : 0) * (N * 16) + ((c >> 3) << 4) + 4 * g, offH = 8 * N * 16;
+            const int instL = inst_of(c & 7), instH = inst_of((c & 7) + 8);
+            const bool validL = tile_ok && in_batch(instL), validH = tile_ok && in_batch(instH);
+            const int obaseL = (validL ? instL : 0) * (N * 16) + ((c >> 3) << 4) + 4 * g;
+            const int offH = ((validH ? instH : 0) - (validL ? instL : 0)) * (N * 16);
             auto put2 = [&](float *dst, int i, const f32x4 &ve, const f32x4 &vo) {
                 f32x4 lo8, hi8;
                 t16_pair_lines(t16_transpose4(ve), t16_transpose4(vo), lo8, hi8);
@@ -990,7 +1016,7 @@
             s[0] = xn[0]; s[1] = xn[1]; s[2] = xn[2];
         }
         }
-        const unsigned long long umask = __ballot(valid && !solved);
+        const unsigned long long umask = __ballot(valid_e && !solved);
         if (umask != 0ull)
         {
             const bool unsolved2 = valid2 && ((umask >> c2) & 1ull);
@@ -1006,7 +1032,7 @@
                 if constexpr (XPOSE)
                 {
                     const f32x4 o = t16_transpose4(f32x4{pn[0], pn[1], pn[2], dd});
-                    if (valid && !solved) *reinterpret_cast<f32x4 *>(P.pd + obase4 + i * 16) = o;
+                    if (valid_e && !solved) *reinterpret_cast<f32x4 *>(P.pd + obase4 + i * 16) = o;
                 }
                 else
                 {
@@ -1021,12 +1047,12 @@
                 p[0] = pn[0]; p[1] = pn[1]; p[2] = pn[2];
             }
         }
-        if (valid && g == 0)
-        {
-            P.res[4 * inst + 0] = r_ps; P.res[4 * inst + 1] = r_pi;
-            P.res[4 * inst + 2] = r_ds; P.res[4 * inst + 3] = r_di;
-            P.status[inst] = st;
-            P.iter[inst] = itn;
+        if (valid_e && g == 0)
+        {
+            P.res[4 * inst_e + 0] = r_ps; P.res[4 * inst_e + 1] = r_pi;
+            P.res[4 * inst_e + 2] = r_ds; P.res[4 * inst_e + 3] = r_di;
+            P.status[inst_e] = st;
+            P.iter[inst_e] = itn;
             if (!solved) atomicAdd(P.n_unsolved, 1);
         }
         if (MPC && valid)
@@ -1049,7 +1075,7 @@
 #define TINY_FOR_EACH_TILE16(X) X(30) X(25) X(20) X(10)
 #endif
 
-static inline unsigned t16_tail_stride(const RowParams &P, int ntiles, int nblocks, int asked)
+static inline unsigned t16_tail_stride(const RowParams &P, int ntiles, int nblocks, int asked, bool grouped)
 {
     static const int env = [] { const char *e = getenv("TINYMPC_T16_TAIL"); return e ? atoi(e) : -1; }();
     const int forced = asked >= 0 ? asked : env;
@@ -1058,6 +1084,7 @@
     if (!P.order || P.mpc_steps > 1 || !P.cold_start) return 0u;
     const int slots = nblocks * TILE16_WAVES;
     if (ntiles < 3 * slots) return 0u;
+    if (grouped) return ntiles < 8 * slots ? 12u : 8u;
     return (ntiles >= 4 * slots && ntiles < 8 * slots) ? 4u : 8u;
 }
 
@@ -1082,7 +1109,8 @@
     const size_t lds = tile16_pi_lds_bytes(N, bounds_ring, xref_ring, P.pi_flags, P.xref_mode == 1 ? P.table_rows : N);
     if (lds > 160 * 1024) return hipErrorInvalidValue;
     RowParams Q = P;
-    Q.pi_flags = (Q.pi_flags & 0xffu) | (t16_tail_stride(P, ntiles, nblocks, tail) << 8);
+    Q.inst_map = nullptr;
+    Q.pi_flags = (Q.pi_flags & 0xffu) | (t16_tail_stride(P, ntiles, nblocks, tail, false) << 8);
 #define TINY_TILE16_PI_LAUNCH3(NN, EX, BRR, XRR)                                                                           \
     {                                                                                                                      \
         auto kern = P.cold_start ? admm_tile16_kernel<NN, EX, true, false, BRR, XRR> : admm_tile16_kernel<NN, EX, false, false, BRR, XRR>; \
@@ -1117,6 +1145,17 @@
 }
 
 int tile16_max_table_rows() { return TILE16_MAX_TABLE_ROWS; }
+
+bool tile16_two_ended(int batch, int n_cu, int tail)
+{
+    RowParams P{};
+    static const int dummy_order = 0;
+    P.batch = batch; P.cold_start = 1; P.mpc_steps = 1; P.order = &dummy_order;
+    const int ntiles = (batch + 15) / 16;
+    if (n_cu <= 0) n_cu = 256;
+    const int want = (ntiles + TILE16_WAVES - 1) / TILE16_WAVES, nblocks = want < n_cu ? want : n_cu;
+    return t16_tail_stride(P, ntiles, nblocks, tail, true) != 0u;
+}
 
 #if TINY_T16_STAMP
 static int t16_stamp_nslots = 0;
@@ -1155,7 +1194,8 @@
     if (rows > TILE16_MAX_TABLE_ROWS) return hipErrorInvalidValue;
     const size_t lds = (size_t)(TILE16_WAVES * N * WAVE + 2 * N * 4 + (rows + N - 1) * 4) * sizeof(float4);
     RowParams Q = P;
-    Q.pi_flags = (Q.pi_flags & 0xffu) | (t16_tail_stride(P, ntiles, nblocks, tail) << 8);
+    if (P.mpc_steps > 1 || !P.cold_start) Q.inst_map = nullptr;
+    Q.pi_flags = (Q.pi_flags & 0xffu) | (t16_tail_stride(P, ntiles, nblocks, tail, Q.inst_map != nullptr) << 8);
 #define TINY_TILE16_LAUNCH(NN, EX)                                                                                         \
     {                                                                                                                      \
         auto kern = P.mpc_steps > 1 ? (P.cold_start ? admm_tile16_kernel<NN, EX, true, true> : admm_tile16_kernel<NN, EX, false, true>) \
diff --git a/accelerated-tinympc_amd/csrc/dispatch_order.hip b/accelerated-tinympc_amd/csrc/dispatch_order.hip
--- a/accelerated-tinympc_amd/csrc/dispatch_order.hip
+++ b/accelerated-tinympc_amd/csrc/dispatch_order.hip
@@ -10,8 +10,10 @@
 {
     const int lane = threadIdx.x & (WAVE - 1), r16 = lane & 15;
     const int grp = TILES ? (int)blockIdx.x * 4 + (int)(threadIdx.x >> 6) : (int)blockIdx.x;
-    const int inst = grp * 4 + (lane >> 4);
-    const bool valid = inst < P.batch;
+    int inst = grp * 4 + (lane >> 4);
+    if constexpr (TILES)
+        if (P.inst_map) inst = P.inst_map[inst];
+    const bool valid = (unsigned)inst < (unsigned)P.batch;
     const int inst_a = valid ? inst : P.batch - 1;
     const bool is_x = r16 < NX, is_u = (r16 >= NX) && (r16 < NX + NU);
     const int N = P.N;
@@ -79,6 +81,63 @@
     bucket_sort_descending([key](int g) { return (int)((__builtin_bit_cast(unsigned, key[g]) & 0x7fffffffu) >> 20); }, order, n, counters);
 }
 
+__device__ inline int start_bucket(int s) { return min(max(s, 0), NBUCKET - 1); }
+
+__global__ __launch_bounds__(1024) void instance_hist_kernel(const int *__restrict__ start, int batch, int *__restrict__ hist)
+{
+    __shared__ int cnt[NBUCKET];
+    const int t = threadIdx.x, i = (int)blockIdx.x * 1024 + t;
+    for (int b = t; b < NBUCKET; b += 1024) cnt[b] = 0;
+    __syncthreads();
+    if (i < batch) atomicAdd(&cnt[start_bucket(start[i])], 1);
+    __syncthreads();
+    for (int b = t; b < NBUCKET; b += 1024)
+        if (cnt[b]) atomicAdd(&hist[b], cnt[b]);
+}
+
+__global__ __launch_bounds__(1024) void instance_map_kernel(const int *__restrict__ start, int batch, const int *__restrict__ hist, int *__restrict__ cursor,
+                                                            int *__restrict__ map)
+{
+    __shared__ int cnt[NBUCKET], sa[NBUCKET], sb[NBUCKET];
+    const int t = threadIdx.x, i = (int)blockIdx.x * 1024 + t;
+    for (int b = t; b < NBUCKET; b += 1024) { cnt[b] = 0; sa[b] = hist[b]; }
+    __syncthreads();
+    int bk = 0, rank = 0;
+    if (i < batch)
+    {
+        bk = start_bucket(start[i]);
+        rank = atomicAdd(&cnt[bk], 1);
+    }
+    int *src = sa, *dst = sb;
+    for (int d = 1; d < NBUCKET; d <<= 1)
+    {
+        __syncthreads();
+        for (int b = t; b < NBUCKET; b += 1024) dst[b] = src[b] + (b >= d ? src[b - d] : 0);
+        int *tmp = src; src = dst; dst = tmp;
+    }
+    __syncthreads();
+    for (int b = t; b < NBUCKET; b += 1024)
+    {
+        const int c = cnt[b];
+        if (c) cnt[b] = src[b] - hist[b] + atomicAdd(&cursor[b], c);
+    }
+    __syncthreads();
+    if (i < batch) map[cnt[bk] + rank] = i;
+    if (blockIdx.x == 0)
+        for (int e = batch + t; e < ((batch + 15) & ~15); e += 1024) map[e] = -1;
+}
+
+hipError_t launch_instance_map(const int *start, int batch, int *map, int *scratch, hipStream_t stream)
+{
+    hipError_t e = hipMemsetAsync(scratch, 0, 2 * NBUCKET * sizeof(int), stream);
+    if (e != hipSuccess) return e;
+    const int nwg = (batch + 1023) / 1024;
+    hipLaunchKernelGGL(instance_hist_kernel, dim3(nwg), dim3(1024), 0, stream, start, batch, scratch);
+    hipLaunchKernelGGL(instance_map_kernel, dim3(nwg), dim3(1024), 0, stream, start, batch, scratch, scratch + NBUCKET, map);
+    return hipGetLastError();
+}
+int instance_map_scratch_ints() { return 2 * NBUCKET; }
+
 __global__ __launch_bounds__(1024) void dispatch_order_history_kernel(const int *__restrict__ iter, int unit, int batch, int use_sum, int *__restrict__ order, int n,
                                                                       int *__restrict__ counters)
 {
diff --git a/accelerated-tinympc_amd/csrc/tinympc_batch.hip b/accelerated-tinympc_amd/csrc/tinympc_batch.hip
--- a/accelerated-tinympc_amd/csrc/tinympc_batch.hip
+++ b/accelerated-tinympc_amd/csrc/tinympc_batch.hip
@@ -444,6 +444,11 @@
     int graph_captures = 0;
     int n_cu = 256;
     int tile_queue = -1;
+    int tile_grouping = -1;
+    int *tile_map = nullptr;
+    bool tile_map_dirty = true;
+    int tile_map_builds = 0;
+    bool last_grouped = false;
     float *tab_tile = nullptr, *tab_row = nullptr;
     float *tab_row_h = nullptr;
     int table_rows = 0;
@@ -1167,6 +1172,7 @@
     P.res = tb->res; P.status = tb->status; P.iter = tb->iter; P.n_unsolved = tb->n_unsolved;
     P.mpc_steps = 1; P.window_advance = 0; P.u0_traj = nullptr; P.x0buf = tb->x0buf;
     P.dual32 = (tb->h16 && tb->dual32) ? 1 : 0;
+    P.inst_map = nullptr;
 }
 
 int check_optional_terms(const TinyBatch *tb)
@@ -1234,6 +1240,28 @@
     return M;
 }
 
+bool tile_grouping_wanted(const TinyBatch *tb, const KernelPlan &pl)
+{
+    static const int env = [] { const char *e = getenv("TINYMPC_T16_GROUP"); return e ? atoi(e) : -1; }();
+    const int mode = tb->tile_grouping >= 0 ? tb->tile_grouping : env;
+    if (mode == 0) return false;
+    if (pl.kernel != Kernel::Tile16 || pl.pi || pl.pm || tb->xref_mode != 1 || tb->order_dev) return false;
+    if (!tb->cold_pending || dispatch_effective(tb) != 1 || tb->max_iter <= 0) return false;
+    return mode >= 1 || tile16_two_ended(tb->batch, tb->n_cu, tb->tile_queue);
+}
+
+int ensure_tile_map(TinyBatch *tb, const KernelPlan &pl)
+{
+    if (!tile_grouping_wanted(tb, pl) || (tb->tile_map && !tb->tile_map_dirty)) return 0;
+    const size_t n = (size_t)((tb->batch + 15) / 16) * 16;
+    if (!tb->tile_map) TRY(dev_alloc_zero((float **)&tb->tile_map, n + (size_t)instance_map_scratch_ints()));
+    const hipError_t e = launch_instance_map(tb->xref_start, tb->batch, tb->tile_map, tb->tile_map + n, tb->stream);
+    if (e != hipSuccess) return fail(TINY_BATCH_EHIP, "kernel launch failed: %s", hipGetErrorString(e));
+    tb->tile_map_dirty = false;
+    ++tb->tile_map_builds;
+    return 0;
+}
+
 int prepare_solve(TinyBatch *tb, bool closed_loop, KernelPlan *plan)
 {
     if (!(tb->pm || (tb->have_cache && tb->have_dyn)) || !tb->have_settings)
@@ -1263,9 +1291,9 @@
     TRY(prepare_inputs(tb, layout));
     TRY(flush_x0_zero(tb));
     if (tb->max_iter <= 0) TRY(flush_pending(tb));
-    if (inputs_rebuilt) return resolve_plan(tb, closed_loop, plan);
-    *plan = pl;
-    return 0;
+    if (inputs_rebuilt) TRY(resolve_plan(tb, closed_loop, plan));
+    else *plan = pl;
+    return closed_loop ? 0 : ensure_tile_map(tb, *plan);
 }
 
 void fill_solve_params(const TinyBatch *tb, SolveParams &P)
@@ -1300,12 +1328,14 @@
     const bool want_predicted = run ? (tb->dispatch_mode == 1 || (tb->dispatch_mode == -1 && from_reset)) : dispatch_effective(tb) == 1;
     const bool predicted = eligible && want_predicted && !history && !pl.pm && !tb->dual32 && tb->max_iter > 1;
     if (traits(pl.kernel).order_unit_solve == 16) P.order = nullptr;
+    P.inst_map = (!run && tb->tile_map && tile_grouping_wanted(tb, pl)) ? tb->tile_map : nullptr;
     hipError_t e = hipSuccess;
     if (history) e = launch_dispatch_order_history(tb->iter, tb->batch, unit, tb->order_buf, tb->n_unsolved, tb->stream, run && unit == 16);
     else if (predicted)
     {
         RowParams K;
         fill_row_params(tb, K, false);
+        K.inst_map = P.inst_map;
         e = launch_dispatch_order(tb->nx, tb->nu, tb->h16, K, tb->key_buf, tb->order_buf, tb->stream, unit == 16);
     }
     else HIP_TRY(hipMemsetAsync(tb->n_unsolved, 0, 2 * sizeof(int), tb->stream));
@@ -1366,8 +1396,13 @@
         const int applied = enqueue_dispatch_order(tb, pl, 1, false, P);
         if (applied < 0) return applied;
         tb->last_dispatch = applied;
-    }
-    else HIP_TRY(hipMemsetAsync(tb->n_unsolved, 0, 2 * sizeof(int), tb->stream));
+        tb->last_grouped = P.inst_map != nullptr;
+    }
+    else
+    {
+        HIP_TRY(hipMemsetAsync(tb->n_unsolved, 0, 2 * sizeof(int), tb->stream));
+        tb->last_grouped = false;
+    }
     if (record_events) HIP_TRY(hipEventRecord(tb->ev0, tb->stream));
     if (t.layout == LAYOUT_ROW && P.dual32 && !t.fp32_duals)
         return fail(TINY_BATCH_EUNSUPPORTED, "fp16 storage with fp32 duals runs on the register-resident 16-lane and quad kernels only "
@@ -1386,6 +1421,7 @@
 
 int enqueue_plant_step(TinyBatch *tb, int window_advance)
 {
+    if (tb->xref_mode == 1 && window_advance) tb->tile_map_dirty = true;
     if (tb->pm)
     {
         hipLaunchKernelGGL(plant_step_pm_kernel, dim3((tb->batch + 127) / 128), dim3(128), 0, tb->stream, tb->x0buf, work_ptr(tb, TINY_ARR_X), work_ptr(tb, TINY_ARR_U),
@@ -1498,7 +1534,7 @@
     for (int k = 0; k < 4; k++) { (void)guarded_free(tb->in_bnd[k].dev); (void)guarded_free(tb->t_bnd[k]); }
     (void)guarded_free(tb->t_xref); (void)guarded_free(tb->r_xref); (void)guarded_free(tb->r_bounds); (void)guarded_free((float *)tb->rows_vary_dev);
     (void)guarded_free(tb->r_bounds_img); (void)guarded_free(tb->r_xref_img);
-    (void)guarded_free(tb->tab_tile); (void)guarded_free(tb->tab_row); (void)guarded_free(tb->tab_row_h); (void)guarded_free(tb->xref_start);
+    (void)guarded_free(tb->tab_tile); (void)guarded_free(tb->tab_row); (void)guarded_free(tb->tab_row_h); (void)guarded_free(tb->xref_start); (void)guarded_free(tb->tile_map);
     (void)guarded_free(tb->res); (void)guarded_free(tb->status); (void)guarded_free(tb->iter); (void)guarded_free(tb->n_unsolved);
     (void)guarded_free(tb->opnd); (void)guarded_free(tb->qvec); (void)guarded_free(tb->gen_mats); (void)guarded_free(tb->mats_exact); (void)guarded_free(tb->mats_fast);
     (void)guarded_free(tb->pm_src); (void)guarded_free(tb->pm_rho); (void)guarded_free(tb->pm_row[0]); (void)guarded_free(tb->pm_row[1]);
@@ -1768,6 +1804,36 @@
     return TINY_BATCH_OK;
 }
 
+int tiny_batch_set_tile_grouping(TinyBatch *tb, int mode)
+{
+    CHECK_TB(tb);
+    if (mode < -1 || mode > 1) return fail(TINY_BATCH_EINVAL, "tiny_batch_set_tile_grouping: mode must be -1 (automatic), 0 (off) or 1 (by window start)");
+    tb->tile_grouping = mode;
+    invalidate_graph(tb);
+    return TINY_BATCH_OK;
+}
+
+int tiny_batch_tile_grouping_applied(TinyBatch *tb)
+{
+    CHECK_TB(tb);
+    return tb->last_grouped ? 1 : 0;
+}
+
+int tiny_batch_get_tile_map(TinyBatch *tb, int *map, int *builds)
+{
+    CHECK_TB(tb);
+    if (builds) *builds = tb->tile_map_builds;
+    if (!tb->tile_map) return 0;
+    const int n = (tb->batch + 15) / 16 * 16;
+    if (map)
+    {
+        TRY(set_device(tb));
+        HIP_TRY(hipMemcpyAsync(map, tb->tile_map, (size_t)n * sizeof(int), hipMemcpyDeviceToHost, tb->stream));
+        HIP_TRY(hipStreamSynchronize(tb->stream));
+    }
+    return n;
+}
+
 int tiny_batch_dispatch_applied(TinyBatch *tb)
 {
     CHECK_TB(tb);
@@ -1856,6 +1922,7 @@
     HIP_TRY(hipStreamSynchronize(tb->stream));
     tb->table_rows = rows;
     tb->xref_mode = 1;
+    tb->tile_map_dirty = true;
     invalidate_graph(tb);
     return 0;
 }
@@ -2114,6 +2181,7 @@
     if (tb->nx > 64) return fail(TINY_BATCH_EUNSUPPORTED, "mpc_run supports nx <= 64");
     if (tb->max_iter <= 0) return fail(TINY_BATCH_EINVAL, "tiny_batch_mpc_run_async needs max_iter > 0");
     TRY(set_device(tb));
+    if (tb->xref_mode == 1 && window_advance) tb->tile_map_dirty = true;
     const bool from_reset = tb->cold_pending;
     TRY(flush_pending(tb));
     tb->duals_zero_pending = true;
@@ -2128,6 +2196,7 @@
         const int applied = enqueue_dispatch_order(tb, pl, steps, from_reset, P);
         if (applied < 0) return applied;
         tb->last_dispatch = applied;
+        tb->last_grouped = false;
         const hipError_t e = launch_kernel(tb, pl, P);
         if (e != hipSuccess) return fail(TINY_BATCH_EHIP, "kernel launch failed: %s", hipGetErrorString(e));
         if (d_u0_traj) TRY(launch_unpack(tb, work_ptr(tb, TINY_ARR_U), d_u0_traj + (size_t)(steps - 1) * u0n, tb->layout, 1, tb->batch, 0, 1));
diff --git a/accelerated-tinympc_amd/csrc/tinympc_internal.h b/accelerated-tinympc_amd/csrc/tinympc_internal.h
--- a/accelerated-tinympc_amd/csrc/tinympc_internal.h
+++ b/accelerated-tinympc_amd/csrc/tinympc_internal.h
@@ -84,6 +84,7 @@
     float *u0_traj;
     float *x0buf;
     int dual32;
+    const int *inst_map;
 };
 
 struct ModelParams
@@ -132,6 +133,7 @@
 hipError_t launch_admm_tile16_pi(int N, bool exact, bool bounds_ring, bool xref_ring, const RowParams &P, hipStream_t stream, int n_cu, int tail = -1);
 size_t tile16_pi_lds_bytes(int N, bool bounds_ring, bool xref_ring, unsigned pi_flags, int table_rows);
 int tile16_max_table_rows();
+bool tile16_two_ended(int batch, int n_cu, int tail);
 
 #define TINY_FOR_EACH_WAVEDIMS(X) X(32, 16) X(16, 8) X(16, 4) X(20, 8) X(24, 4)
 bool wavedims_supported(int nx, int nu);
@@ -148,5 +150,7 @@
 
 hipError_t launch_dispatch_order(int nx, int nu, bool h16, const RowParams &P, float *key, int *order, hipStream_t stream, int tile = 0);
 hipError_t launch_dispatch_order_history(const int *iter, int batch, int unit, int *order, int *counters, hipStream_t stream, int use_sum = 0);
+hipError_t launch_instance_map(const int *start, int batch, int *map, int *scratch, hipStream_t stream);
+int instance_map_scratch_ints();
 
 }
diff --git a/accelerated-tinympc_amd/solver.py b/accelerated-tinympc_amd/solver.py
--- a/accelerated-tinympc_amd/solver.py
+++ b/accelerated-tinympc_amd/solver.py
@@ -66,7 +66,7 @@
         "tiny_batch_enable_timing": [P, C.c_int], "tiny_batch_last_solve_ms": [P, F],
         "tiny_batch_select_kernel": [P, C.c_int], "tiny_batch_arithmetic": [P], "tiny_batch_debug_graph_captures": [P], "tiny_batch_set_storage": [P, C.c_int], "tiny_batch_set_storage_ex": [P, C.c_int, C.c_int],
         "tiny_batch_set_row_kernel": [P, C.c_int],
-        "tiny_batch_set_dispatch": [P, C.c_int], "tiny_batch_set_tile_queue": [P, C.c_int], "tiny_batch_set_dispatch_order_device": [P, P], "tiny_batch_dispatch_applied": [P],
+        "tiny_batch_set_dispatch": [P, C.c_int], "tiny_batch_set_tile_queue": [P, C.c_int], "tiny_batch_set_tile_grouping": [P, C.c_int], "tiny_batch_tile_grouping_applied": [P], "tiny_batch_get_tile_map": [P, I, I], "tiny_batch_set_dispatch_order_device": [P, P], "tiny_batch_dispatch_applied": [P],
         "tiny_batch_set_optional_terms": [P, C.c_int, C.c_int], "tiny_batch_set_input_cost": [P, F],
         "tiny_batch_set_coeff_d2p": [P, F], "tiny_batch_set_uref": [P, F, C.c_int],
         "tiny_batch_group_solve": [C.POINTER(P), C.c_int, I],
@@ -449,6 +449,21 @@
     def set_tile_queue(self, stride: int):
         self._check(self.lib.tiny_batch_set_tile_queue(self._h, stride))
 
+    def set_tile_grouping(self, mode: int):
+        self._check(self.lib.tiny_batch_set_tile_grouping(self._h, mode))
+
+    def tile_grouping_applied(self) -> bool:
+        return bool(self._check(self.lib.tiny_batch_tile_grouping_applied(self._h)))
+
+    def tile_map(self):
+        builds = C.c_int(0)
+        n = self._check(self.lib.tiny_batch_get_tile_map(self._h, None, C.byref(builds)))
+        if n == 0:
+            return None, builds.value
+        m = np.empty(n, np.int32)
+        self._check(self.lib.tiny_batch_get_tile_map(self._h, m.ctypes.data_as(C.POINTER(C.c_int)), None))
+        return m, builds.value
+
     def dispatch_applied(self) -> int:
         return self._check(self.lib.tiny_batch_dispatch_applied(self._h))
 
diff --git a/include/tinympc_batch.h b/include/tinympc_batch.h
--- a/include/tinympc_batch.h
+++ b/include/tinympc_batch.h
@@ -103,6 +103,9 @@
 
     int tiny_batch_set_dispatch(TinyBatch *tb, int mode);
     int tiny_batch_set_tile_queue(TinyBatch *tb, int stride);
+    int tiny_batch_set_tile_grouping(TinyBatch *tb, int mode);
+    int tiny_batch_tile_grouping_applied(TinyBatch *tb);
+    int tiny_batch_get_tile_map(TinyBatch *tb, int *map, int *builds);
     int tiny_batch_dispatch_applied(TinyBatch *tb);
     int tiny_batch_set_dispatch_order_device(TinyBatch *tb, const int *d_order);
 
```

Result: faster. 47.87 million solves/s, median of 6 (+3.7%).
